# HKUST-SING/herald

Hardware: AMD Instinct MI355X
Metric: embedding rows/s (lookup+grad) (higher is better)
Workload: dtype f32

## Files before the change

herald_amd/_build.py:

```python
import os
import shutil
import subprocess
import sys

ROOT = os.path.dirname(os.path.dirname(os.path.abspath(__file__)))
PKG = os.path.join(ROOT, "herald_amd")
CSRC = os.path.join(PKG, "csrc")
OBJ = os.path.join(PKG, "_build")
LIB = os.path.join(PKG, "libherald_amd.so")

HIPCC = os.environ.get("HIPCC", "/opt/rocm/bin/hipcc")
HIP_FLAGS = [
    "--offload-arch=gfx950", "-O3", "-std=c++17", "-fPIC",
    "-ffp-contract=off",
    "-fno-gpu-rdc", "-Wall", "-Wno-unused-function",
    "-I", os.path.join(ROOT, "include"),
]


def _run(cmd, **kw):
    r = subprocess.run(cmd, stdout=subprocess.PIPE, stderr=subprocess.STDOUT, text=True, **kw)
    if r.returncode != 0:
        sys.stderr.write(" ".join(cmd) + "\n" + r.stdout + "\n")
        raise RuntimeError("build step failed: %s" % " ".join(cmd[:3]))
    return r.stdout


def _newer(src_list, target):
    if not os.path.exists(target):
        return True
    t = os.path.getmtime(target)
    return any(os.path.getmtime(s) > t for s in src_list)


def hip_sources():
    return sorted(os.path.join(CSRC, f) for f in os.listdir(CSRC) if f.endswith(".hip"))


def build_lib(force=False, verbose=False):
    os.makedirs(OBJ, exist_ok=True)
    headers = [os.path.join(CSRC, f) for f in os.listdir(CSRC) if f.endswith(".h")]
    headers.append(os.path.join(ROOT, "include", "herald_amd.h"))
    objs = []
    procs = []
    for src in hip_sources():
        obj = os.path.join(OBJ, os.path.basename(src)[:-4] + ".o")
        objs.append(obj)
        if force or _newer([src] + headers, obj):
            cmd = [HIPCC] + HIP_FLAGS + ["-c", src, "-o", obj]
            if verbose:
                print(" ".join(cmd))
            procs.append((cmd, subprocess.Popen(cmd, stdout=subprocess.PIPE,
                                                stderr=subprocess.STDOUT, text=True)))
    for cmd, p in procs:
        out, _ = p.communicate()
        if p.returncode != 0:
            sys.stderr.write(" ".join(cmd) + "\n" + out + "\n")
            raise RuntimeError("hipcc failed on %s" % cmd[-3])
        if verbose and out.strip():
            print(out)
    if force or procs or _newer(objs, LIB):
        _run([HIPCC, "--offload-arch=gfx950", "-shared", "-fPIC", "-fno-gpu-rdc", "-o", LIB] + objs)
    return LIB


PS_LIB = os.path.join(PKG, "libherald_ps.so")


def build_ps_shim(force=False):
    src = os.path.join(CSRC, "libps_shim.cpp")
    deps = [src, os.path.join(ROOT, "include", "herald_ps.h"), os.path.join(ROOT, "include", "herald_amd.h"), LIB]
    if force or _newer(deps, PS_LIB):
        _run(["g++", "-O2", "-std=c++17", "-shared", "-fPIC", "-Wall", src, "-o", PS_LIB, "-L", PKG, "-lherald_amd",
              "-Wl,-rpath,$ORIGIN"])
    return PS_LIB


def build_plugins(force=False):
    import sysconfig
    import pybind11
    out_dir = os.path.join(PKG, "plugins")
    os.makedirs(out_dir, exist_ok=True)
    suffix = sysconfig.get_config_var("EXT_SUFFIX")
    inc = ["-I", pybind11.get_include(), "-I", sysconfig.get_paths()["include"], "-I", "/opt/rocm/include"]
    outs = []
    procs = []
    for name in ("hetu_cache", "laia_cache"):
        src = os.path.join(CSRC, "py_%s.cpp" % name)
        out = os.path.join(out_dir, name + suffix)
        outs.append(out)
        if force or _newer([src, os.path.join(ROOT, "include", "herald_amd.h"), LIB], out):
            cmd = ["g++", "-O2", "-std=c++17", "-shared", "-fPIC", "-w", "-D__HIP_PLATFORM_AMD__"] + inc + \
                  [src, "-o", out, "-L", PKG, "-lherald_amd", "-L", "/opt/rocm/lib", "-lamdhip64",
                   "-Wl,-rpath,$ORIGIN/..", "-Wl,-rpath,/opt/rocm/lib", "-pthread"]
            procs.append((cmd, subprocess.Popen(cmd, stdout=subprocess.PIPE, stderr=subprocess.STDOUT, text=True)))
    for cmd, p in procs:
        o, _ = p.communicate()
        if p.returncode != 0:
            sys.stderr.write(" ".join(cmd) + "\n" + o + "\n")
            raise RuntimeError("plugin build failed")
    return outs


def build_oracle(force=False):
    src = os.path.join(ROOT, "oracle", "oracle.c")
    out_dir = os.path.join(ROOT, "oracle", "_build")
    out = os.path.join(out_dir, "liboracle.so")
    if not os.path.exists(src):
        return None
    os.makedirs(out_dir, exist_ok=True)
    if force or _newer([src], out):
        _run(["gcc", "-O3", "-fopenmp", "-ffp-contract=off", "-fPIC", "-shared", "-std=c11",
              "-Wall", "-o", out, src, "-lm"])
    return out


def build_ref(force=False):
    script = os.path.join(ROOT, "oracle", "build_ref.sh")
    if not (os.path.isdir("/root/reference") and os.path.exists(script)):
        return None
    _run(["bash", script])
    return os.path.join(ROOT, "oracle", "_ref")


def build_all(force=False, verbose=False):
    lib = build_lib(force=force, verbose=verbose)
    build_ps_shim(force=force)
    build_plugins(force=force)
    build_oracle(force=force)
    build_ref(force=force)
    return lib


if __name__ == "__main__":
    build_all(force="--force" in sys.argv, verbose=True)
    print("built", LIB)
```

herald_amd/_lib.py:

```python
import ctypes
import os
import re

_PKG = os.path.dirname(os.path.abspath(__file__))
LIB_PATH = os.path.join(_PKG, "libherald_amd.so")
HEADER_PATH = os.path.join(os.path.dirname(_PKG), "include", "herald_amd.h")

_lib = None


class HeraldAmdError(RuntimeError):
    pass


class DLContext(ctypes.Structure):
    _fields_ = [("device_id", ctypes.c_int), ("device_type", ctypes.c_int)]


class DLArray(ctypes.Structure):
    _fields_ = [("data", ctypes.c_void_p), ("ctx", DLContext), ("ndim", ctypes.c_int),
                ("shape", ctypes.POINTER(ctypes.c_int64)), ("stride", ctypes.POINTER(ctypes.c_int64))]


class DLStream(ctypes.Structure):
    _fields_ = [("device_id", ctypes.c_int), ("handle", ctypes.c_void_p)]


class CacheRemote(ctypes.Structure):
    _fields_ = [("req_keys", ctypes.c_void_p), ("req_versions", ctypes.c_void_p), ("inbox_pull", ctypes.c_void_p),
                ("inbox_idx", ctypes.c_void_p), ("inbox_versions", ctypes.c_void_p), ("inbox_rows", ctypes.c_void_p),
                ("out_keys", ctypes.c_void_p), ("out_updates", ctypes.c_void_p), ("out_rows", ctypes.c_void_p),
                ("out_capacity", ctypes.c_int64), ("max_batch", ctypes.c_int64)]


class PlanView(ctypes.Structure):
    _fields_ = [("n", ctypes.c_int64), ("n_unique", ctypes.c_void_p), ("keys", ctypes.c_void_p),
                ("sorted", ctypes.c_void_p), ("perm", ctypes.c_void_p), ("inverse", ctypes.c_void_p),
                ("uniq", ctypes.c_void_p), ("counts", ctypes.c_void_p), ("seg", ctypes.c_void_p),
                ("upos", ctypes.c_void_p)]


def declared_symbols(header=None):
    text = open(header or HEADER_PATH).read()
    text = re.sub(r"/\*.*?\*/", "", text, flags=re.S)
    text = re.sub(r"\(\s*\*\s*\w+\s*\)\s*\([^;{}]*\)\s*;", ";", text)
    names = re.findall(r"\b([A-Za-z_][A-Za-z0-9_]*)\s*\([^;{}]*\)\s*;", text)
    return sorted(set(n for n in names if n not in ("defined", "int", "void", "float")))


PS_LIB_PATH = os.path.join(_PKG, "libherald_ps.so")
PS_HEADER_PATH = os.path.join(os.path.dirname(_PKG), "include", "herald_ps.h")


def load(build_if_missing=True):
    global _lib
    if _lib is not None:
        return _lib
    try:
        import torch
    except ImportError:
        pass
    if not os.path.exists(LIB_PATH):
        if not build_if_missing:
            raise HeraldAmdError("libherald_amd.so is not built (%s)" % LIB_PATH)
        from . import _build
        _build.build_lib()
    try:
        L = ctypes.CDLL(LIB_PATH, mode=ctypes.RTLD_GLOBAL)
    except OSError as e:
        raise HeraldAmdError("cannot load %s: %s" % (LIB_PATH, e))
    _declare(L)
    _lib = L
    return L


class ShardSlot(ctypes.Structure):
    _fields_ = [("world", ctypes.c_int32), ("rank", ctypes.c_int32), ("rcap", ctypes.c_int64), ("n", ctypes.c_int64),
                ("plan_ws", ctypes.c_void_p), ("keys_fixed", ctypes.c_void_p), ("meta_dev", ctypes.c_void_p),
                ("posmap", ctypes.c_void_p), ("rowmap", ctypes.c_void_p), ("counts_host", ctypes.c_void_p),
                ("owner_plan_ws", ctypes.c_void_p)]


def check(rc, what=""):
    if rc != 0:
        msg = load().ha_last_error().decode("utf-8", "replace")
        raise HeraldAmdError("%s failed: %s" % (what or "herald_amd call", msg))


def _declare(L):
    c = ctypes
    vp, i64, f32, sz = c.c_void_p, c.c_int64, c.c_float, c.c_size_t
    L.ha_version.restype = c.c_char_p
    L.ha_last_error.restype = c.c_char_p
    L.ha_device_count.restype = c.c_int
    L.ha_plan_bytes.restype = sz
    L.ha_plan_bytes.argtypes = [i64]
    L.ha_plan_view_of.argtypes = [vp, i64, c.POINTER(PlanView)]
    L.ha_plan_radix_stamps.argtypes = [vp, i64, vp, vp]
    L.ha_pend_bytes.restype = sz
    L.ha_pend_bytes.argtypes = []
    L.ha_plan_handoff_timeout.restype = vp
    L.ha_plan_handoff_timeout.argtypes = [vp]
    L.ha_step_tab_bytes.restype = sz
    L.ha_step_tab_bytes.argtypes = []
    L.ha_step_max_ids.restype = i64
    L.ha_step_max_ids.argtypes = []
    L.ha_qstep_max_ids.restype = i64
    L.ha_qstep_max_ids.argtypes = []
    L.ha_qstep_init.restype = c.c_int
    L.ha_qstep_init.argtypes = []
    L.ha_event_create.restype = vp
    L.ha_event_create.argtypes = []
    L.ha_host_unmap.restype = c.c_int
    L.ha_host_unmap.argtypes = [vp]
    L.ha_qbig_max_ids.restype = i64
    L.ha_qbig_max_ids.argtypes = []
    L.ha_xchg_create.restype = vp
    L.ha_xchg_create.argtypes = [vp, c.c_int, c.c_int]
    L.ha_qbig_plan_bytes.restype = sz
    L.ha_qbig_plan_bytes.argtypes = [i64]
    L.ha_qbig_buckets.restype = c.c_int
    L.ha_qbig_buckets.argtypes = [i64]
    L.ha_qstep_queue_bytes.restype = sz
    L.ha_qstep_queue_bytes.argtypes = [i64, i64]
    L.ha_qstep_queue_header.restype = vp
    L.ha_qstep_queue_header.argtypes = [vp]
    sigs = {
        "ha_gather_f32ids": [vp, i64, i64, vp, i64, vp, vp],
        "ha_gather_u64ids": [vp, i64, i64, vp, i64, vp, vp],
        "ha_gather_u32keys": [vp, i64, i64, vp, i64, vp, vp],
        "ha_scatter_rows_f32ids": [vp, vp, i64, i64, vp, i64, vp],
        "ha_scale_f32": [vp, i64, f32, vp],
        "ha_plan_build_f32ids": [vp, i64, vp, vp],
        "ha_plan_build_u64ids": [vp, i64, vp, vp],
        "ha_plan_build_u32keys": [vp, i64, vp, c.c_int, vp],
        "ha_plan_sort_f32ids": [vp, i64, vp, vp],
        "ha_plan_sort_u32keys": [vp, i64, vp, c.c_int, vp],
        "ha_plan_sort_u64ids": [vp, i64, vp, vp],
        "ha_plan_finish": [vp, i64, vp],
        "ha_plan_build_f32ids_lim": [vp, i64, vp, c.c_uint64, vp],
        "ha_plan_sort_f32ids_lim": [vp, i64, vp, c.c_uint64, vp],
        "ha_plan_build_u64ids_lim": [vp, i64, vp, c.c_uint64, vp],
        "ha_plan_sort_u64ids_lim": [vp, i64, vp, c.c_uint64, vp],
        "ha_plan_export_f32": [vp, i64, vp, vp, vp],
        "ha_dedup_reduce": [vp, i64, vp, i64, vp, vp],
        "ha_apply_mapped": [vp, i64, i64, vp, i64, vp, f32, vp, vp, vp, vp],
        "ha_apply_mapped2": [vp, i64, vp, i64, vp, i64, vp, f32, vp, vp, vp, vp],
        "ha_shard_bucket": [vp, i64, vp, c.c_int, vp, vp, vp],
        "ha_shard_route_f32ids": [vp, i64, vp, vp, c.c_int, vp, vp, vp],
        "ha_shard_route_u64ids": [vp, i64, vp, vp, c.c_int, vp, vp, vp],
        "ha_shard_route_pack_f32ids": [vp, i64, vp, vp, c.c_int, i64, vp, vp, vp],
        "ha_shard_route_pack_u64ids": [vp, i64, vp, vp, c.c_int, i64, vp, vp, vp],
        "ha_shard_route_unpack": [vp, c.c_int, i64, vp, vp, vp],
        "ha_shard_frames_route_f32ids": [vp, i64, vp, vp, c.c_int, i64, i64, vp, vp, vp, vp],
        "ha_shard_frames_route_u64ids": [vp, i64, vp, vp, c.c_int, i64, i64, vp, vp, vp, vp],
        "ha_shard_frames_pack": [vp, i64, vp, c.c_int, i64, i64, vp, vp, vp, vp],
        "ha_shard_frames_unpack": [vp, c.c_int, i64, i64, vp, vp, vp],
        "ha_set_tolerance_mode": [c.c_int],
        "ha_get_tolerance_mode": [],
        "ha_shard_frames_serve_push": [vp, i64, i64, vp, c.c_int, i64, vp, vp, vp],
        "ha_shard_frames_pack_batch": [vp, vp, c.c_int, vp, c.c_int, i64, i64, vp, vp, vp, vp],
        "ha_shard_frames_unpack_batch": [vp, c.c_int, c.c_int, i64, i64, vp, vp, vp],
        "ha_shard_frames_pack_batch_sized": [vp, vp, c.c_int, vp, c.c_int, c.c_int, i64, i64, vp, vp, vp, vp, vp, vp],
        "ha_shard_frames_unpack_batch_sized": [vp, c.c_int, c.c_int, i64, i64, vp, vp, vp, vp],
        "ha_shard_sized_serve_pull": [vp, i64, i64, vp, c.c_int, c.c_int, i64, vp, vp, vp],
        "ha_gather2_u32map": [vp, i64, vp, i64, i64, vp, i64, vp, vp],
        "ha_shard_sized_serve_push": [vp, i64, i64, vp, c.c_int, c.c_int, i64, vp, i64, vp, vp, vp],
        "ha_push_apply_scaled_finished": [vp, i64, i64, vp, i64, vp, f32, vp],
        "ha_qbig_plan_batch_f32ids": [vp, vp, vp, i64, i64, vp],
        "ha_qbig_plan_batch_u64ids": [vp, vp, vp, i64, i64, vp],
        "ha_qbig_queue_batch": [i64, i64, vp, vp, vp, vp, vp, i64, i64, vp, vp, vp],
        "ha_qbig_apply": [vp, i64, i64, vp, i64, vp, f32, vp, i64, vp, vp, i64, i64, c.c_uint32, vp, vp, vp],
        "ha_event_destroy": [vp],
        "ha_event_record": [vp, vp],
        "ha_stream_wait_event": [vp, vp],
        "ha_qqueue_batch_epochs": [i64, i64, vp, vp, vp, vp, vp, i64, i64, vp, vp, vp],
        "ha_shard_step_pull": [vp, i64, i64, vp, vp, vp, vp, i64, vp, vp],
        "ha_shard_step_push": [vp, i64, i64, vp, vp, vp, i64, vp, vp, f32, vp],
        "ha_shard_step": [vp, i64, i64, vp, vp, vp, vp, i64, vp, i64, vp, vp, vp, f32, vp],
        "ha_shard_steps": [vp, i64, i64, i64, vp, vp, vp, vp, i64, vp, i64, vp, vp, vp, f32, vp],
        "ha_qapply_steps_sync": [vp, i64, i64, f32, i64, i64, vp, vp, vp, vp, vp, vp, vp, vp, vp, vp, vp, vp],
        "ha_qapply_steps_counts": [vp, i64, i64, f32, i64, i64, vp, vp, vp, vp, vp, vp, vp, vp, vp, vp, vp, vp, vp],
        "ha_qapply_sync": [vp, i64, i64, vp, i64, vp, f32, vp, i64, vp, vp, i64, i64, c.c_uint32, vp, vp, vp],
        "ha_xchg_available": [],
        "ha_xchg_unique_id": [vp],
        "ha_xchg_destroy": [vp],
        "ha_xchg_bytes": [vp, vp, vp, vp, vp, vp],
        "ha_xchg_rows": [vp, vp, vp, vp, vp, i64, vp],
        "ha_qbig_plan_view": [vp, i64, vp, vp, vp, vp, vp, vp, vp],
        "ha_plan_build_batch_f32ids_lim": [vp, vp, vp, c.c_int, c.c_uint64, vp],
        "ha_plan_sort_batch_f32ids_lim": [vp, vp, vp, c.c_int, c.c_uint64, vp],
        "ha_plan_sort_batch_u64ids_lim": [vp, vp, vp, c.c_int, c.c_uint64, vp],
        "ha_plan_build_batch_u64ids_lim": [vp, vp, vp, c.c_int, c.c_uint64, vp],
        "ha_shard_frames_serve_pull": [vp, i64, i64, vp, c.c_int, i64, i64, vp, vp, vp, vp],
        "ha_shard_serve_push": [vp, i64, i64, vp, i64, vp, vp, vp],
        "ha_dedup_reduce_scaled": [vp, i64, vp, i64, f32, vp, vp],
        "ha_debug_apply_timeline": [vp, i64, i64, vp, i64, vp, f32, vp, vp],
        "ha_sgd_apply": [vp, i64, i64, vp, i64, vp, f32, vp],
        "ha_sgd_apply_finished": [vp, i64, i64, vp, i64, vp, f32, vp],
        "ha_push_apply": [vp, i64, i64, vp, i64, vp, vp],
        "ha_sgd_sparse_update_f32ids": [vp, i64, i64, vp, i64, vp, f32, vp],
        "ha_lookup_sort_f32ids": [vp, i64, i64, vp, i64, vp, vp, vp],
        "ha_lookup_sort_u64ids": [vp, i64, i64, vp, i64, vp, vp, vp],
        "ha_sgd_apply_finish": [vp, i64, i64, vp, i64, vp, f32, vp],
        "ha_push_apply_finish": [vp, i64, i64, vp, i64, vp, vp],
        "ha_sgd_apply_finish_prefetch_f32ids": [vp, i64, i64, vp, i64, vp, f32, vp, i64, vp],
        "ha_sparse_opt_fused_f32ids": [c.c_int, vp, i64, i64, vp, i64, vp, vp, vp, vp, vp, vp],
        "ha_pend_reset": [vp, vp],
        "ha_lookup_sort_pend_f32ids": [vp, i64, i64, vp, i64, vp, vp, vp, vp],
        "ha_lookup_sort_pend_u64ids": [vp, i64, i64, vp, i64, vp, vp, vp, vp],
        "ha_sgd_push_pull_f32ids": [vp, i64, i64, vp, i64, vp, f32, vp, vp, i64, vp, vp, vp, vp],
        "ha_sgd_push_pull_u64ids": [vp, i64, i64, vp, i64, vp, f32, vp, vp, i64, vp, vp, vp, vp],
        "ha_step_tab_reset": [vp, vp],
        "ha_step_f32ids": [vp, i64, i64, vp, i64, vp, f32, vp, vp, i64, vp, vp, vp, i64, vp, vp, i64, vp, vp, vp],
        "ha_step_u64ids": [vp, i64, i64, vp, i64, vp, f32, vp, vp, i64, vp, vp, vp, i64, vp, vp, i64, vp, vp, vp],
        "ha_qstep_f32ids": [vp, i64, i64, vp, i64, vp, f32, vp, i64, vp, vp, vp, i64, vp, i64, vp, i64, vp, vp],
        "ha_qstep_u64ids": [vp, i64, i64, vp, i64, vp, f32, vp, i64, vp, vp, vp, i64, vp, i64, vp, i64, vp, vp],
        "ha_qprep_f32ids": [i64, i64, vp, i64, vp, vp, i64, vp, i64, vp, i64, vp],
        "ha_qprep_u64ids": [i64, i64, vp, i64, vp, vp, i64, vp, i64, vp, i64, vp],
        "ha_qplan_batch_f32ids": [vp, vp, vp, i64, vp],
        "ha_qplan_batch_u64ids": [vp, vp, vp, i64, vp],
        "ha_qqueue_batch": [i64, i64, vp, vp, vp, vp, vp, i64, i64, vp],
        "ha_stream_gate": [vp, vp],
        "ha_debug_occupy": [i64, i64, i64, i64, vp],
        "ha_qapply": [vp, i64, i64, vp, i64, vp, f32, vp, i64, vp, vp, i64, vp],
        "ha_qapply_sized": [vp, i64, i64, vp, i64, vp, f32, vp, i64, vp, vp, i64, i64, vp],
        "ha_qapply_steps": [vp, i64, i64, f32, i64, i64, vp, vp, vp, vp, vp, vp, vp, vp, vp],
        "ha_qqueue_batch_counts": [i64, i64, vp, vp, vp, vp, vp, i64, i64, vp, vp],
        "ha_debug_qprep_f32ids": [i64, i64, vp, i64, vp, vp, i64, vp, i64, vp, i64, vp, vp],
        "ha_debug_qapply": [vp, i64, i64, vp, i64, vp, f32, vp, i64, vp, vp, i64, vp, vp],
        "ha_debug_step_fwd_timeline": [vp, i64, i64, vp, i64, vp, f32, vp, vp, i64, vp, vp, vp, i64, vp, vp, i64, vp,
                                       vp, vp, vp],
    }
    for name, args in sigs.items():
        fn = getattr(L, name)
        fn.argtypes = args
        fn.restype = c.c_int
    L.ha_cache_create.restype = vp
    L.ha_cache_create.argtypes = [c.c_int, i64, i64, i64, i64]
    L.ha_cache_destroy.restype = None
    L.ha_cache_destroy.argtypes = [vp]
    for name in ("ha_cache_data", "ha_cache_grad"):
        getattr(L, name).restype = vp
        getattr(L, name).argtypes = [vp]
    for name in ("ha_cache_limit", "ha_cache_width", "ha_cache_fused_updates"):
        getattr(L, name).restype = i64
        getattr(L, name).argtypes = [vp]
    cache_sigs = {
        "ha_cache_set_bounds": [vp, i64, i64],
        "ha_cache_set_bypass": [vp, c.c_int],
        "ha_cache_bind_store": [vp, vp, vp, i64, i64],
        "ha_cache_lookup": [vp, vp, c.c_int, i64, vp, vp],
        "ha_cache_sort_ahead": [vp, vp, c.c_int, i64, vp],
        "ha_cache_lookup_presorted": [vp, vp, c.c_int, i64, vp, vp],
        "ha_cache_sort_ahead_batch": [vp, vp, c.c_int, vp, c.c_int, vp],
        "ha_cache_plan_block": [vp, vp, c.c_int, vp, c.c_int, vp, vp],
        "ha_cache_plan_block_push_keys": [vp, vp, c.c_int, vp, vp, c.c_int, vp, c.c_int, vp, vp],
        "ha_cache_lookup_planned": [vp, i64, vp, vp],
        "ha_cache_update_planned": [vp, i64, vp, vp],
        "ha_cache_plan_pending": [vp],
        "ha_cache_run_planned_pairs": [vp, c.c_int, vp, vp, vp, vp],
        "ha_cache_plan_block_push_pull": [vp, vp, c.c_int, vp, c.c_int, vp, vp],
        "ha_cache_push_pull_planned": [vp, i64, vp, i64, vp, vp],
        "ha_cache_run_planned_push_pulls": [vp, c.c_int, vp, vp, vp, vp, vp],
        "ha_cache_update": [vp, vp, c.c_int, i64, vp, vp],
        "ha_cache_update_same_keys": [vp, i64, vp, vp],
        "ha_cache_update_with_push_keys": [vp, vp, c.c_int, i64, vp, c.c_int, i64, vp, vp],
        "ha_cache_push_pull": [vp, vp, c.c_int, i64, vp, vp, c.c_int, i64, vp, vp],
        "ha_cache_perf": [vp, vp, vp],
        "ha_cache_state": [vp, vp, vp],
        "ha_cache_phase_times": [vp, vp, vp],
        "ha_cache_set_timing": [vp, c.c_int],
        "ha_cache_stage_times": [vp, vp],
        "ha_cache_snapshot": [vp, i64, vp, vp, vp, vp, vp, vp, vp],
        "ha_cache_set_line": [vp, i64, i64, vp, vp],
        "ha_cache_set_remote": [vp],
        "ha_cache_remote_buffers": [vp, vp],
        "ha_cache_lookup_begin": [vp, vp, c.c_int, i64, vp, vp],
        "ha_cache_lookup_finish": [vp, i64, vp, vp],
        "ha_cache_outbox_count": [vp, vp, vp],
        "ha_cache_outbox_pad": [vp, i64],
        "ha_store_count_valid": [vp, i64, i64, vp, vp],
        "ha_cache_push_pull_begin": [vp, vp, c.c_int, i64, vp, c.c_int, i64, vp, vp, vp],
        "ha_cache_push_pull_finish": [vp, vp, vp],
        "ha_store_serve_sync": [vp, vp, i64, i64, vp, vp, i64, i64, vp, vp, vp, vp, vp, vp, vp],
        "ha_store_add_versions": [vp, i64, vp, vp, i64, vp],
        "ha_store_push_distinct": [vp, vp, i64, i64, vp, vp, vp, i64, vp],
    }
    for name, args in cache_sigs.items():
        fn = getattr(L, name)
        fn.argtypes = args
        fn.restype = c.c_int
    L.ha_laia_create.restype = vp
    L.ha_laia_create.argtypes = [vp, i64, i64, i64, i64, i64, i64]
    L.ha_laia_destroy.restype = None
    L.ha_laia_destroy.argtypes = [vp]
    L.ha_laia_next.restype = c.c_int
    L.ha_laia_next.argtypes = [vp, i64, i64, vp, vp, i64, vp]
    L.ha_laia_hint_next.restype = c.c_int
    L.ha_laia_hint_next.argtypes = [vp, i64]
    L.ha_laia_next_for_rank.restype = c.c_int
    L.ha_laia_next_for_rank.argtypes = [vp, i64, i64, i64, vp, vp, i64, vp]
    L.ha_laia_snapshot_keys.restype = i64
    L.ha_laia_snapshot_keys.argtypes = [vp, i64, vp, i64]
    L.ha_laia_next_topk.restype = c.c_int
    L.ha_laia_next_topk.argtypes = [vp, i64, i64, vp, i64, i64, vp, vp, i64, vp]
    L.ha_laia_counters.restype = c.c_int
    L.ha_laia_counters.argtypes = [vp, vp]
    L.ha_laia_timing.restype = c.c_int
    L.ha_laia_timing.argtypes = [vp, vp]
    L.ha_laia_timing_device.restype = c.c_int
    L.ha_laia_timing_device.argtypes = [vp, vp]
    L.ha_laia_on_device.restype = c.c_int
    L.ha_laia_on_device.argtypes = [vp]
    L.ha_shm_ring_open.restype = vp
    L.ha_shm_ring_open.argtypes = [c.c_char_p, c.c_int, i64]
    L.ha_shm_ring_close.restype = None
    L.ha_shm_ring_close.argtypes = [vp]
    L.ha_shm_ring_send.restype = c.c_int
    L.ha_shm_ring_send.argtypes = [vp, vp, i64]
    L.ha_shm_ring_recv.restype = i64
    L.ha_shm_ring_recv.argtypes = [vp, vp, i64, vp]
    L.ha_shm_ring_pending_words.restype = i64
    L.ha_shm_ring_pending_words.argtypes = [vp]
    A, S = c.POINTER(DLArray), c.POINTER(DLStream)
    dl = {
        "DLGpuEmbeddingLookUp": [A, A, A, S],
        "DLGpuEmbeddingLookUp_Gradient": [A, A, A, S],
        "IndexedSlicesOneSideAdd": [A, A, A, S],
        "DeduplicateIndexedSlices": [A, A, A, S],
        "IndexedSlices2Dense": [A, A, A, S],
        "SGDOptimizerSparseUpdate": [A, A, A, f32, S],
        "AdaGradOptimizerSparseUpdate": [A, A, A, A, f32, f32, S],
        "AdamOptimizerSparseUpdate": [A, A, A, A, A, f32, f32, f32, f32, f32, f32, S],
        "AdamWOptimizerSparseUpdate": [A, A, A, A, A, f32, f32, f32, f32, f32, f32, f32, S],
        "AddL2RegularizationSparse": [A, A, A, f32, S],
# ... 10 lines not shown
```

herald_amd/csrc/qstep.hip:

```cpp
#include <hip/hip_ext.h>

#include "plan_dev.h"
#include "gather_dev.h"

namespace ha {

constexpr int kQMax = 7168;
#ifndef QV_GOLD
#define QV_GOLD 1
#endif
#ifndef QV_WG
#define QV_WG (QV_GOLD ? 1024 : 256)
#endif
#ifndef QV_COOPSLOTS
#define QV_COOPSLOTS (QV_GOLD ? 64 : 256)
#endif
constexpr int kQWg = QV_WG;
constexpr int kQWpw = kQWg / 64;
constexpr int kQCoopSlots = QV_COOPSLOTS;
constexpr int kQWorkerMax = 448 * 16 / kQWpw;
constexpr int kQSmallC = 3, kQSmallM = 16, kQMediumC = 15, kQLongC = 64;
enum QKind { kQS = 0, kQM = 1, kQL = 2, kQZ = 3, kQG = 4, kQNone = 15 };

struct QHeader {
    uint32_t n_wave, n_coop;
    uint32_t n_long, n_medium, n_small;
    uint32_t n_copy, n_copy_medium, n_copy_small;
    uint32_t overflow_wave, overflow_copy;
    uint32_t epoch_wave, epoch_copy, done;
    uint32_t verdict;
    uint32_t reserved[50];
};
static_assert(sizeof(QHeader) == 256, "queue header is one 256-byte line");
struct QEntry {
    uint32_t w[8];
};
constexpr uint32_t kQOccMask = 0x1FFFFFu;
__host__ __device__ __forceinline__ uint2 q_occ_pack(uint32_t o0, uint32_t o1, uint32_t o2) {
    const unsigned long long v = static_cast<unsigned long long>(o0 & kQOccMask) |
                                 (static_cast<unsigned long long>(o1 & kQOccMask) << 21) |
                                 (static_cast<unsigned long long>(o2 & kQOccMask) << 42);
    return uint2{static_cast<uint32_t>(v), static_cast<uint32_t>(v >> 32)};
}
static_assert(sizeof(QEntry) == 32, "queue items are 32 bytes");

struct QLayout {
    QHeader *hdr;
    QEntry *coop, *wave, *copy;
    float *part;
    uint32_t *pcnt;
    uint32_t cap_coop, cap_wave, cap_copy;
    size_t bytes;
};
constexpr uint32_t kQChunk = 256;
__host__ __device__ __forceinline__ uint32_t q_nchunk(uint32_t c) {
    return (QV_GOLD && c > kQChunk) ? (c + kQChunk - 1u) / kQChunk : 1u;
}
static inline int ceil_div(int64_t a, int64_t b) { return static_cast<int>((a + b - 1) / b); }
static inline QLayout queue_layout(void *ws, int64_t n_cap, int64_t width) {
    QLayout q;
    char *b = static_cast<char *>(ws);
    q.cap_coop = static_cast<uint32_t>(ceil_div(width, 32) * (ceil_div(n_cap, kQLongC) + 1));
    q.cap_wave = static_cast<uint32_t>(ceil_div(width, 512) * 2 * n_cap + 64);
    q.cap_copy = static_cast<uint32_t>(ceil_div(width, 512) * n_cap + 64);
    q.hdr = reinterpret_cast<QHeader *>(b);
    q.coop = reinterpret_cast<QEntry *>(b ? b + sizeof(QHeader) : nullptr);
    q.wave = q.coop ? q.coop + q.cap_coop : nullptr;
    q.copy = q.wave ? q.wave + q.cap_wave : nullptr;
    const size_t items = sizeof(QHeader) + (static_cast<size_t>(q.cap_coop) + q.cap_wave + q.cap_copy) * sizeof(QEntry);
    q.part = reinterpret_cast<float *>(b ? b + items : nullptr);
    q.pcnt = reinterpret_cast<uint32_t *>(b ? b + items + static_cast<size_t>(q.cap_coop) * 256 : nullptr);
    q.bytes = items + static_cast<size_t>(q.cap_coop) * (256 + 4);
    return q;
}

struct QPlan {
    PlanHeader *hdr;
    uint32_t *keys, *sorted, *uniq;
    int32_t *perm, *inverse, *counts, *seg, *upos;
    uint32_t *occ;
    int n;
};
static inline QPlan qplan(void *ws, int64_t n) {
    QPlan q;
    memset(&q, 0, sizeof(q));
    if (ws == nullptr || n <= 0)
        return q;
    PlanPtrs p = plan_layout(ws, n);
    q.hdr = p.hdr; q.keys = p.keys; q.sorted = p.sorted; q.uniq = p.uniq;
    q.perm = p.perm; q.inverse = p.inverse; q.counts = p.counts; q.seg = p.seg; q.upos = p.upos;
    q.occ = p.keys_alt;
    q.n = static_cast<int>(n);
    return q;
}

struct QArgs {
    float *table;
    uint64_t rows;
    int width;
    const QHeader *qh;
    const QEntry *qcoop, *qwave, *qcopy;
    float *qpart;
    uint32_t *qpcnt;
    uint32_t cap_coop, cap_wave, cap_copy;
    const int32_t *perm_a;
    int n_a;
    const float *grads;
    float lr;
    const int32_t *perm_g;
    int n_g;
    float *out;
    int ncoop, nworker;
    uint32_t epoch;
    uint32_t *err;
    unsigned long long *dbg;
};

__device__ __forceinline__ void q_phase(unsigned long long *ph, int k) {
    if (ph != nullptr && threadIdx.x == 0)
        ph[k] = __builtin_amdgcn_s_memrealtime();
}

template <int NW>
__device__ __forceinline__ uint32_t qscan_n(uint32_t v, uint32_t *s_w, uint32_t *total, int w) {
    const int lane = lane_id();
    uint32_t x = v;
#pragma unroll
    for (int o = 1; o < 64; o <<= 1) {
        const uint32_t y = __shfl_up(x, o, 64);
        if (lane >= o)
            x += y;
    }
    __syncthreads();
    if (lane == 63)
        s_w[w] = x;
    __syncthreads();
    const uint32_t mine = s_w[lane & (NW - 1)];
    uint32_t woff = 0, tot = 0;
#pragma unroll
    for (int k = 0; k < NW; ++k) {
        const uint32_t t = static_cast<uint32_t>(__builtin_amdgcn_readlane(static_cast<int>(mine), k));
        woff += k < w ? t : 0u;
        tot += t;
    }
    *total = tot;
    return woff + x - v;
}

constexpr int kQTabBits = 13, kQTabSize = 1 << kQTabBits;
constexpr uint32_t kQTabEmpty = 0xFFFFFFFFu;
constexpr int kGroupedFlagWord = 12;
constexpr int kOrderFlagWord = 13;
__device__ __forceinline__ uint32_t q_hash(uint32_t key, int bits = kQTabBits) {
    return (key * 0x9E3779B1u) >> (32 - bits);
}
static inline size_t qsort_lds_bytes(int n) {
    const size_t npad = (static_cast<size_t>(n) + 1023) & ~static_cast<size_t>(1023);
    return kQTabSize * 4 + 3 * npad * 2 + 8 + 32 * 4;
}
constexpr int kQSubThreads = 256, kQSubTabBits = 12, kQSubMax = 7 * kQSubThreads;
constexpr size_t kQSubPlanLds = (size_t(1) << kQSubTabBits) * 4 + 3 * size_t(kQSubMax) * 2 + 8 + 32 * 4 + 120;
static_assert(kQSubPlanLds % 128 == 0, "the groups' LDS regions stay aligned");

template <typename IdT, bool RANK_ATOMIC, bool BUCKET = false, int NT = 1024, int TBITS = kQTabBits>
__device__ __forceinline__ void qsort_finish_body(const IdT *__restrict__ ids, const QPlan &p, uint32_t *lds,
                                                  unsigned long long *ph = nullptr,
                                                  const uint32_t *__restrict__ pos_map = nullptr) {
    constexpr int TS = 1 << TBITS, SPT = TS / NT;
    const int n = p.n;
    const int tid = static_cast<int>(threadIdx.x) & (NT - 1), lane = lane_id(), w = tid >> 6;
    const int npad = (n + NT - 1) & ~(NT - 1);
    const int P = npad / NT;
    uint32_t *s_tab = lds;
    uint16_t *s_lab = reinterpret_cast<uint16_t *>(lds + TS);
    uint16_t *s_cnt = s_lab + npad;
    uint16_t *s_rank = s_cnt + npad + 4;
    uint32_t *s_w = reinterpret_cast<uint32_t *>(s_rank + npad);
    q_phase(ph, 0);
    uint32_t key[7];
#pragma unroll
    for (int k = 0; k < 7; ++k)
        key[k] = to_key<IdT>(ids[max(min(tid + k * NT, n - 1), 0)]);
    for (int i = tid; i < TS; i += NT)
        s_tab[i] = kQTabEmpty;
    for (int i = tid; i < npad / 2 + 2; i += NT)
        reinterpret_cast<uint32_t *>(s_cnt)[i] = 0;
    __syncthreads();
    q_phase(ph, 1);
    {
        uint32_t h[7], seen[7];
#pragma unroll
        for (int k = 0; k < 7; ++k) {
            h[k] = q_hash(key[k], TBITS);
            seen[k] = key[k];
            if (k < P && tid + k * NT < n) {
                if (BUCKET && k > 0 && s_tab[h[k]] == key[k])
                    continue;
                seen[k] = kQTabEmpty;
                if (__hip_atomic_compare_exchange_strong(s_tab + h[k], &seen[k], key[k], __ATOMIC_RELAXED,
                                                         __ATOMIC_RELAXED, __HIP_MEMORY_SCOPE_WORKGROUP))
                    seen[k] = key[k];
            }
        }
#pragma unroll
        for (int k = 0; k < 7; ++k) {
            const int i = tid + k * NT;
            if (k < P && i < n) {
                while (seen[k] != key[k]) {
                    h[k] = (h[k] + 1) & (TS - 1);
                    seen[k] = kQTabEmpty;
                    if (__hip_atomic_compare_exchange_strong(s_tab + h[k], &seen[k], key[k], __ATOMIC_RELAXED,
                                                             __ATOMIC_RELAXED, __HIP_MEMORY_SCOPE_WORKGROUP))
                        seen[k] = key[k];
                }
                s_lab[i] = static_cast<uint16_t>(h[k]);
            }
        }
    }
    __syncthreads();
    q_phase(ph, 2);
    uint32_t U;
    {
        uint32_t kk[SPT], occ = 0;
#pragma unroll
        for (int j = 0; j < SPT; ++j) {
            kk[j] = s_tab[tid * SPT + j];
            occ += kk[j] != kQTabEmpty;
        }
        uint32_t g = qscan_n<NT / 64>(occ, s_w, &U, w);
#pragma unroll
        for (int j = 0; j < SPT; ++j) {
            if (kk[j] != kQTabEmpty) {
                p.uniq[g] = kk[j];
                s_tab[tid * SPT + j] = g;
                ++g;
            }
        }
    }
    __syncthreads();
    q_phase(ph, 3);
    uint32_t lab[7];
#pragma unroll
    for (int k = 0; k < 7; ++k) {
        const int i = tid + k * NT;
        lab[k] = 0;
        if (k < P && i < n) {
            lab[k] = s_tab[s_lab[i]];
            s_lab[i] = static_cast<uint16_t>(lab[k]);
        }
    }
    __syncthreads();
    q_phase(ph, 4);
    if (w == 0) {
        uint32_t *cnt32 = reinterpret_cast<uint32_t *>(s_cnt);
        const uint32_t spare = static_cast<uint32_t>(npad);
        uint32_t nx[8];
#pragma unroll
        for (int r = 0; r < 8; ++r)
            nx[r] = s_lab[min(r * 64 + lane, npad - 1)];
        for (int r0 = 0; r0 < npad; r0 += 8 * 64) {
            uint32_t lb[8], rk[8];
#pragma unroll
            for (int r = 0; r < 8; ++r) {
                const int i = r0 + r * 64 + lane;
                lb[r] = i < n ? nx[r] : spare;
            }
// ... 77 lines not shown
        }
    }
    if (tid == 0) {
        p.hdr->n_unique = U;
        p.hdr->reserved[kGroupedFlagWord] = 1;
        p.hdr->reserved[kOrderFlagWord] = 0;
        p.seg[U] = n;
    }
    __syncthreads();
    q_phase(ph, 6);
    {
        uint32_t q[7];
#pragma unroll
        for (int k = 0; k < 7; ++k) {
            const int i = tid + k * NT;
            q[k] = (k < P && i < n) ? static_cast<uint32_t>(s_cnt[lab[k]]) + s_rank[i] : 0u;
        }
        __syncthreads();
        uint16_t *s_perm = s_lab, *s_gq = s_rank;
        uint32_t *s_key = s_tab;
#pragma unroll
        for (int k = 0; k < 7; ++k) {
            const int i = tid + k * NT;
            if (k < P && i < n) {
                s_perm[q[k]] = static_cast<uint16_t>(i);
                s_gq[q[k]] = static_cast<uint16_t>(lab[k]);
                s_key[i] = key[k];
            }
        }
        __syncthreads();
        bool disorder = false;
        for (int qq = tid; qq < n; qq += NT) {
            const uint32_t i = s_perm[qq];
            if (BUCKET) {
                p.perm[qq] = static_cast<int32_t>(pos_map[i]);
            } else {
                p.perm[qq] = static_cast<int32_t>(i);
                p.sorted[qq] = s_key[i];
                p.upos[qq] = static_cast<int32_t>(s_gq[qq]);
            }
            disorder |= qq > 0 && s_gq[qq] == s_gq[qq - 1] && i <= s_perm[qq - 1];
        }
        if (disorder)
            p.hdr->reserved[kOrderFlagWord] = 1;
        for (uint32_t g = tid; g < U; g += NT) {
            const int st = s_cnt[g];
            uint32_t o0 = s_perm[min(st, n - 1)], o1 = s_perm[min(st + 1, n - 1)], o2 = s_perm[min(st + 2, n - 1)];
            if (BUCKET) {
                o0 = pos_map[o0];
                o1 = pos_map[o1];
                o2 = pos_map[o2];
            }
            reinterpret_cast<uint2 *>(p.occ)[g] = q_occ_pack(o0, o1, o2);
        }
    }
    q_phase(ph, 7);
}

static inline size_t qjoin_lds_bytes(int n_a, int n_g) {
    return kQTabSize * 4 + static_cast<size_t>(n_a > n_g ? n_a : n_g) * 4 + 32 * 4;
}
static inline size_t qjoin_lds_resident_bytes(int n_g) {
    return kQTabSize * 4 + static_cast<size_t>(n_g) * 8 + 32 * 4;
}

__device__ __forceinline__ int q_kind(uint32_t c, uint32_t m, bool in_table) {
    if (!in_table)
        return m > 0 ? kQZ : kQNone;
    if (c >= static_cast<uint32_t>(kQLongC))
        return kQG;
    if (c > static_cast<uint32_t>(kQMediumC))
        return kQL;
    if (c > static_cast<uint32_t>(kQSmallC) || m > static_cast<uint32_t>(kQSmallM))
        return kQM;
    return kQS;
}
__device__ __forceinline__ int q_slice(int kind) {
    return kind == kQL ? 32 : kind == kQG ? (QV_GOLD ? 64 : 32) : kind == kQM ? 128 : 512;
}

__device__ __forceinline__ void q_st_item(QEntry *dst, uint4 lo, uint4 hi) {
    float4v a, b;
    __builtin_memcpy(&a, &lo, 16);
    __builtin_memcpy(&b, &hi, 16);
    st4_sc1(reinterpret_cast<float *>(dst), a);
    st4_sc1(reinterpret_cast<float *>(dst) + 4, b);
}
__device__ __forceinline__ void q_emit_words(QEntry *dst, int kind, uint32_t key, uint32_t c, uint32_t st, uint32_t m,
                                             uint32_t fs, int width, uint32_t o01, uint32_t o23, uint32_t *pcnt = nullptr) {
    const int slice = q_slice(kind);
    if (kind == kQZ)
        c = 0;
    int j = 0;
    const uint32_t nch = kind == kQG ? q_nchunk(c) : 1u;
    if (nch > 1u) {
        for (int col0 = 0; col0 < width; col0 += slice) {
            __hip_atomic_store(pcnt + j, 0u, __ATOMIC_RELAXED, __HIP_MEMORY_SCOPE_AGENT);
            for (uint32_t ch = 0; ch < nch; ++ch, ++j) {
                uint4 lo, hi;
                lo.x = static_cast<uint32_t>(kind) | (static_cast<uint32_t>(col0 / 4) << 4);
                lo.y = key;
                lo.z = c;
                lo.w = st;
                hi.x = m;
                hi.y = fs;
                hi.z = ch | (nch << 16);
                hi.w = 0;
                q_st_item(dst + j, lo, hi);
            }
        }
        return;
    }
    if (kind == kQG)
        o01 = 0;
    for (int col0 = 0; col0 < width; col0 += slice, ++j) {
        const int cols = min(slice, width - col0);
        uint4 lo, hi;
        lo.x = static_cast<uint32_t>(kind) | (static_cast<uint32_t>(col0 / 4) << 4);
        lo.y = key;
        lo.z = c;
        (void)cols;
        lo.w = st;
        hi.x = m;
        hi.y = fs;
        hi.z = o01;
        hi.w = o23;
        q_st_item(dst + j, lo, hi);
    }
}
struct QCount {
    uint32_t g, l, m, s;
};
__device__ __forceinline__ QCount q_count(QCount t, int kind, uint32_t per512, uint32_t per128, uint32_t per32, uint32_t c) {
    t.g += kind == kQG ? (QV_GOLD ? (per32 + 1u) / 2u : per32) * q_nchunk(c) : 0u;
    t.l += kind == kQL ? per32 : 0u;
    t.m += kind == kQM ? per128 : 0u;
    t.s += (kind == kQS || kind == kQZ) ? per512 : 0u;
    return t;
}

struct QJoin {
    QPlan pa, pg;
    uint64_t rows;
    int width, Ua, Ug, Ub;
    bool cs_res;
    uint32_t *s_tab, *s_bk, *s_cs, *s_w;
    QHeader *bqh;
    QEntry *bcoop, *bwave, *bcopy;
    uint32_t *bpcnt;
    uint32_t bcap_coop, bcap_wave, bcap_copy, per512, per128, per32;
    uint32_t st_base, fs_base;
    uint32_t tid, nt;
    int tbits;
};

__device__ __forceinline__ uint32_t qjoin_probe(const QJoin &j, uint32_t key) {
    uint32_t h = q_hash(key, j.tbits);
    const uint32_t mask = (1u << j.tbits) - 1u;
    for (;;) {
        const uint32_t e = j.s_tab[h];
        if (e == kQTabEmpty || j.s_bk[e] == key)
            return e;
        h = (h + 1) & mask;
    }
}
__device__ __forceinline__ uint32_t qjoin_dest(const QJoin &j, uint32_t e) {
    if (e == kQTabEmpty)
        return 0u;
    return j.cs_res ? j.s_cs[e] : (static_cast<uint32_t>(j.pg.counts[e]) | (static_cast<uint32_t>(j.pg.seg[e]) << 16));
}
__device__ __forceinline__ QCount qjoin_emit_one(const QJoin &j, QCount b, QEntry *wave, uint32_t cap_wave, uint32_t key,
                                                 uint32_t c, uint32_t st, uint32_t m, uint32_t fs, uint32_t o01, uint32_t o2) {
    const int kind = q_kind(c, m, key < j.rows);
    if (kind == kQNone)
        return b;
    const uint32_t at = kind == kQG ? b.g : kind == kQL ? b.l : kind == kQM ? b.m : b.s;
    const QCount nb = q_count(b, kind, j.per512, j.per128, j.per32, c);
    const uint32_t cnt = (nb.g - b.g) + (nb.l - b.l) + (nb.m - b.m) + (nb.s - b.s);
    if (at + cnt <= (kind == kQG ? j.bcap_coop : cap_wave))
        q_emit_words((kind == kQG ? j.bcoop : wave) + at, kind, key, c, st + j.st_base, m, fs + j.fs_base, j.width, o01, o2,
                     kind == kQG ? j.bpcnt + at : nullptr);
    return nb;
}

template <int R0, int R1>
__device__ __forceinline__ QCount qjoin_count_groups(const QJoin &j, QCount t) {
    const uint32_t tid = j.tid, last = static_cast<uint32_t>(max(j.Ua, 1) - 1);
    uint32_t ka[R1 - R0], c[R1 - R0];
#pragma unroll
    for (int r = R0; r < R1; ++r) {
        const uint32_t x = min(static_cast<uint32_t>(r) * j.nt + tid, last);
        ka[r - R0] = j.pa.uniq[x];
        c[r - R0] = static_cast<uint32_t>(j.pa.counts[x]);
    }
#pragma unroll
    for (int r = R0; r < R1; ++r) {
        if (static_cast<int>(static_cast<uint32_t>(r) * j.nt + tid) < j.Ua) {
            const uint32_t mf = qjoin_dest(j, qjoin_probe(j, ka[r - R0]));
            t = q_count(t, q_kind(c[r - R0], mf & 0xFFFFu, ka[r - R0] < j.rows), j.per512, j.per128, j.per32, c[r - R0]);
        }
    }
    return t;
}
template <int R0, int R1>
__device__ __forceinline__ QCount qjoin_emit_groups(const QJoin &j, QCount b) {
    const uint32_t tid = j.tid, last = static_cast<uint32_t>(max(j.Ua, 1) - 1);
    uint32_t ka[R1 - R0], cst[R1 - R0], o01[R1 - R0], o2[R1 - R0];
#pragma unroll
    for (int r = R0; r < R1; ++r) {
        const uint32_t x = min(static_cast<uint32_t>(r) * j.nt + tid, last);
        const uint2 oc = reinterpret_cast<const uint2 *>(j.pa.occ)[x];
        ka[r - R0] = j.pa.uniq[x];
        cst[r - R0] = static_cast<uint32_t>(j.pa.counts[x]) | (static_cast<uint32_t>(j.pa.seg[x]) << 16);
        o01[r - R0] = oc.x;
        o2[r - R0] = oc.y;
    }
#pragma unroll
    for (int r = R0; r < R1; ++r) {
        if (static_cast<int>(static_cast<uint32_t>(r) * j.nt + tid) < j.Ua) {
            const uint32_t mf = qjoin_dest(j, qjoin_probe(j, ka[r - R0]));
            b = qjoin_emit_one(j, b, j.bwave, j.bcap_wave, ka[r - R0], cst[r - R0] & 0xFFFFu, cst[r - R0] >> 16,
                               mf & 0xFFFFu, mf >> 16, o01[r - R0], o2[r - R0]);
        }
    }
    return b;
}

template <int R0, int R1>
__device__ __forceinline__ QCount qjoin_count_copies(const QJoin &j, QCount t) {
    const uint32_t tid = j.tid, last = static_cast<uint32_t>(max(j.Ug, 1) - 1);
    uint32_t kg[R1 - R0], m[R1 - R0];
#pragma unroll
    for (int r = R0; r < R1; ++r) {
        const uint32_t y = min(static_cast<uint32_t>(r) * j.nt + tid, last);
        kg[r - R0] = j.pg.uniq[y];
        m[r - R0] = static_cast<uint32_t>(j.pg.counts[y]);
    }
#pragma unroll
    for (int r = R0; r < R1; ++r)
        if (static_cast<int>(static_cast<uint32_t>(r) * j.nt + tid) < j.Ug && qjoin_probe(j, kg[r - R0]) == kQTabEmpty)
            t = q_count(t, q_kind(0u, m[r - R0], kg[r - R0] < j.rows), j.per512, j.per128, j.per32, 0u);
    return t;
}
template <int R0, int R1>
__device__ __forceinline__ QCount qjoin_emit_copies(const QJoin &j, QCount b) {
    const uint32_t tid = j.tid, last = static_cast<uint32_t>(max(j.Ug, 1) - 1);
    uint32_t kg[R1 - R0], mfs[R1 - R0];
#pragma unroll
    for (int r = R0; r < R1; ++r) {
        const uint32_t y = min(static_cast<uint32_t>(r) * j.nt + tid, last);
        kg[r - R0] = j.pg.uniq[y];
        mfs[r - R0] = static_cast<uint32_t>(j.pg.counts[y]) | (static_cast<uint32_t>(j.pg.seg[y]) << 16);
    }
#pragma unroll
    for (int r = R0; r < R1; ++r)
        if (static_cast<int>(static_cast<uint32_t>(r) * j.nt + tid) < j.Ug && qjoin_probe(j, kg[r - R0]) == kQTabEmpty)
            b = qjoin_emit_one(j, b, j.bcopy, j.bcap_copy, kg[r - R0], 0u, 0u, mfs[r - R0] & 0xFFFFu, mfs[r - R0] >> 16,
                               0u, 0u);
    return b;
}

template <bool WIDE = false, int NT = 1024, int TBITS = kQTabBits>
__device__ __forceinline__ void qjoin_body(const QPlan pa, const QPlan pg, const uint64_t rows, const int width,
                                           QHeader *bqh, QEntry *bcoop, QEntry *bwave, QEntry *bcopy,
                                           const uint32_t bcap_coop, const uint32_t bcap_wave, const uint32_t bcap_copy,
                                           uint32_t *lds, uint32_t lds_bytes, const int part,
                                           unsigned long long *ph = nullptr, uint32_t *mirror = nullptr,
                                           const uint32_t st_base = 0, const uint32_t fs_base = 0,
                                           const uint32_t epoch = 0, const uint32_t wide_parts = 0, const bool signal = true) {
    constexpr int TS = 1 << TBITS;
    const int tid = static_cast<int>(threadIdx.x) & (NT - 1), w = tid >> 6;
    q_phase(ph, 0);
    QJoin j;
    j.tid = static_cast<uint32_t>(tid);
    j.nt = NT;
    j.tbits = TBITS;
    j.pa = pa;
    j.pg = pg;
    j.st_base = st_base;
    j.fs_base = fs_base;
    j.rows = rows;
    j.width = width;
    j.Ua = uniform(pa.n > 0 ? static_cast<int>(pa.hdr->n_unique) : 0);
    j.Ug = uniform(pg.n > 0 ? static_cast<int>(pg.hdr->n_unique) : 0);
    j.Ub = part == 0 ? j.Ug : j.Ua;
    j.cs_res = part == 0 && static_cast<uint32_t>(TS * 4 + j.Ug * 8 + 32 * 4) <= lds_bytes;
    j.s_tab = lds;
    j.s_bk = lds + TS;
    j.s_cs = j.s_bk + j.Ub;
    j.s_w = j.s_bk + (j.cs_res ? 2 * j.Ub : j.Ub);
    j.bqh = bqh;
    j.bcoop = bcoop;
    j.bwave = bwave;
    j.bcopy = bcopy;
    j.bcap_coop = bcap_coop;
    j.bpcnt = reinterpret_cast<uint32_t *>(reinterpret_cast<char *>(bcoop + (static_cast<size_t>(bcap_coop) + bcap_wave + bcap_copy)) +
                                           static_cast<size_t>(bcap_coop) * 256);
    j.bcap_wave = bcap_wave;
    j.bcap_copy = bcap_copy;
    j.per512 = (width + 511) / 512;
    j.per128 = (width + 127) / 128;
    j.per32 = (width + 31) / 32;
    const uint32_t *bkeys = part == 0 ? pg.uniq : pa.uniq;
    for (int i = tid; i < TS; i += NT)
        j.s_tab[i] = kQTabEmpty;
    for (int y = tid; y < j.Ub; y += NT) {
        j.s_bk[y] = bkeys[y];
        if (j.cs_res)
            j.s_cs[y] = static_cast<uint32_t>(pg.counts[y]) | (static_cast<uint32_t>(pg.seg[y]) << 16);
    }
    __syncthreads();
    q_phase(ph, 1);
    for (int y = tid; y < j.Ub; y += NT) {
        uint32_t h = q_hash(j.s_bk[y], TBITS);
        for (;;) {
            uint32_t seen = kQTabEmpty;
            if (__hip_atomic_compare_exchange_strong(j.s_tab + h, &seen, static_cast<uint32_t>(y), __ATOMIC_RELAXED,
                                                     __ATOMIC_RELAXED, __HIP_MEMORY_SCOPE_WORKGROUP))
                break;
            h = (h + 1) & (TS - 1);
        }
    }
    __syncthreads();
    q_phase(ph, 2);
    QCount t{0u, 0u, 0u, 0u};
    if (part == 0) {
        if (j.Ua > 0)
            t = qjoin_count_groups<0, 4>(j, t);
        if (j.Ua > 4 * NT)
            t = qjoin_count_groups<4, 8>(j, t);
        q_phase(ph, 3);
        uint32_t nL, nM, nS, nG;
        QCount b;
        b.l = qscan_n<NT / 64>(t.l, j.s_w, &nL, w);
        b.m = qscan_n<NT / 64>(t.m, j.s_w, &nM, w) + nL;
        b.s = qscan_n<NT / 64>(t.s, j.s_w, &nS, w) + nL + nM;
        b.g = qscan_n<NT / 64>(t.g, j.s_w, &nG, w);
        if (WIDE) {
            __syncthreads();
            if (tid == 0) {
                const uint32_t tot = nL + nM + nS;
                const uint32_t bw = tot ? atomicAdd(&bqh->n_wave, tot) : 0u;
                const uint32_t bc = nG ? atomicAdd(&bqh->n_coop, nG) : 0u;
                if (nL) atomicAdd(&bqh->n_long, nL);
                if (nM) atomicAdd(&bqh->n_medium, nM);
                if (nS) atomicAdd(&bqh->n_small, nS);
                uint32_t over = (bw + tot > bcap_wave || bc + nG > bcap_coop) ? 1u : 0u;
                if ((pa.n > 0 && pa.hdr->reserved[kOrderFlagWord] != 0) || (pg.n > 0 && pg.hdr->reserved[kOrderFlagWord] != 0))
                    over |= 2u;
                if (over) {
                    atomicOr(&bqh->overflow_wave, over);
                    if (mirror)
                        mirror[3] = over;
                }
                j.s_w[20] = bw;
                j.s_w[21] = bc;
            }
            __syncthreads();
            const uint32_t bw = j.s_w[20], bc = j.s_w[21];
            b.l += bw;
            b.m += bw;
            b.s += bw;
            b.g += bc;
        }
        if (!WIDE && tid == 0) {
            bqh->n_wave = min(nL + nM + nS, bcap_wave);
            bqh->n_coop = min(nG, bcap_coop);
            bqh->n_long = nL;
            bqh->n_medium = nM;
            bqh->n_small = nS;
            uint32_t over = (nL + nM + nS > bcap_wave || nG > bcap_coop) ? 1u : 0u;
            if ((pa.n > 0 && pa.hdr->reserved[kOrderFlagWord] != 0) || (pg.n > 0 && pg.hdr->reserved[kOrderFlagWord] != 0))
                over |= 2u;
            bqh->overflow_wave = over;
            if (mirror) {
                mirror[0] = min(nL + nM + nS, bcap_wave) + 1u;
                mirror[1] = min(nG, bcap_coop) + 1u;
                if (over)
                    mirror[3] = over;
            }
        }
        q_phase(ph, 4);
        if (j.Ua > 0)
            b = qjoin_emit_groups<0, 3>(j, b);
        if (j.Ua > 3 * NT)
            b = qjoin_emit_groups<3, 5>(j, b);
        if (j.Ua > 5 * NT)
            b = qjoin_emit_groups<5, 8>(j, b);
    } else {
        if (j.Ug > 0)
            t = qjoin_count_copies<0, 4>(j, t);
        if (j.Ug > 4 * NT)
            t = qjoin_count_copies<4, 8>(j, t);
        q_phase(ph, 3);
        uint32_t nM, nS;
        QCount b{0u, 0u, 0u, 0u};
        b.m = qscan_n<NT / 64>(t.m, j.s_w, &nM, w);
        b.s = qscan_n<NT / 64>(t.s, j.s_w, &nS, w) + nM;
        if (WIDE) {
            __syncthreads();
            if (tid == 0) {
                const uint32_t tot = nM + nS;
                const uint32_t bw = tot ? atomicAdd(&bqh->n_copy, tot) : 0u;
                if (nM) atomicAdd(&bqh->n_copy_medium, nM);
                if (nS) atomicAdd(&bqh->n_copy_small, nS);
                if (bw + tot > bcap_copy) {
                    atomicOr(&bqh->overflow_copy, 1u);
                    if (mirror)
                        mirror[3] = 1u;
                }
                j.s_w[20] = bw;
            }
            __syncthreads();
            const uint32_t bw = j.s_w[20];
            b.m += bw;
            b.s += bw;
        }
        if (!WIDE && tid == 0) {
            bqh->n_copy = min(nM + nS, bcap_copy);
            bqh->n_copy_medium = nM;
            bqh->n_copy_small = nS;
            bqh->overflow_copy = nM + nS > bcap_copy ? 1u : 0u;
            if (mirror) {
                mirror[2] = min(nM + nS, bcap_copy) + 1u;
                if (nM + nS > bcap_copy)
                    mirror[3] = 1u;
            }
        }
        q_phase(ph, 4);
        if (j.Ug > 0)
            b = qjoin_emit_copies<0, 4>(j, b);
        if (j.Ug > 4 * NT)
            b = qjoin_emit_copies<4, 8>(j, b);
    }
    q_phase(ph, 5);
    asm volatile("s_waitcnt vmcnt(0) lgkmcnt(0)" ::: "memory");
    __syncthreads();
    if (tid == 0) {
        if (!WIDE) {
            if (part == 0) {
                __hip_atomic_store(&bqh->n_wave, bqh->n_wave, __ATOMIC_RELAXED, __HIP_MEMORY_SCOPE_AGENT);
                __hip_atomic_store(&bqh->n_coop, bqh->n_coop, __ATOMIC_RELAXED, __HIP_MEMORY_SCOPE_AGENT);
            } else {
                __hip_atomic_store(&bqh->n_copy, bqh->n_copy, __ATOMIC_RELAXED, __HIP_MEMORY_SCOPE_AGENT);
            }
            asm volatile("s_waitcnt vmcnt(0) lgkmcnt(0)" ::: "memory");
            __hip_atomic_store(part == 0 ? &bqh->epoch_wave : &bqh->epoch_copy, epoch, __ATOMIC_RELAXED, __HIP_MEMORY_SCOPE_AGENT);
        } else if (signal &&
                   __hip_atomic_fetch_add(&bqh->done, 1u, __ATOMIC_RELAXED, __HIP_MEMORY_SCOPE_AGENT) + 1u == wide_parts) {
            __hip_atomic_store(&bqh->epoch_wave, epoch, __ATOMIC_RELAXED, __HIP_MEMORY_SCOPE_AGENT);
            __hip_atomic_store(&bqh->epoch_copy, epoch, __ATOMIC_RELAXED, __HIP_MEMORY_SCOPE_AGENT);
            if (mirror) {
                const uint32_t nw = __hip_atomic_load(&bqh->n_wave, __ATOMIC_RELAXED, __HIP_MEMORY_SCOPE_AGENT);
                const uint32_t nc = __hip_atomic_load(&bqh->n_coop, __ATOMIC_RELAXED, __HIP_MEMORY_SCOPE_AGENT);
                const uint32_t np = __hip_atomic_load(&bqh->n_copy, __ATOMIC_RELAXED, __HIP_MEMORY_SCOPE_AGENT);
                mirror[1] = min(nc, bcap_coop) + 1u;
                mirror[2] = min(np, bcap_copy) + 1u;
                __threadfence_system();
                mirror[0] = min(nw, bcap_wave) + 1u;
            }
        }
    }
}

typedef float float2v_ __attribute__((ext_vector_type(2)));

__device__ __forceinline__ float4v sgd4(float4v acc, float4v g, float lr) {
    float4v r;
#pragma unroll
    for (int k = 0; k < 4; ++k)
        r[k] = __fsub_rn(acc[k], __fmul_rn(lr, g[k]));
    return r;
}
__device__ __forceinline__ float4v acc4(float4v p, float4v g, float lr) {
    float4v r;
#pragma unroll
    for (int k = 0; k < 4; ++k)
        r[k] = __fadd_rn(p[k], __fmul_rn(lr, g[k]));
    return r;
}
__device__ __forceinline__ float4v add4(float4v x, float4v y) {
    float4v r;
#pragma unroll
    for (int k = 0; k < 4; ++k)
        r[k] = __fadd_rn(x[k], y[k]);
    return r;
}
__device__ __forceinline__ float4v sub4(float4v x, float4v y) {
    float4v r;
#pragma unroll
    for (int k = 0; k < 4; ++k)
        r[k] = __fsub_rn(x[k], y[k]);
    return r;
}
__device__ __forceinline__ float4v shfl_xor4(float4v v, int mask) {
    float4v r;
#pragma unroll
    for (int k = 0; k < 4; ++k)
        r[k] = __shfl_xor(v[k], mask, 64);
    return r;
}

#ifndef QV_ROW_NT
#define QV_ROW_NT 1
#endif
#ifndef QV_OUT_NT
#define QV_OUT_NT 1
#endif
#ifndef QV_GRAD_NT
#define QV_GRAD_NT 0
#endif
#ifndef QV_INTERLEAVE
#define QV_INTERLEAVE 1
#endif
#ifndef QV_ROWLD_NT
#define QV_ROWLD_NT 0
#endif
template <typename V>
__device__ __forceinline__ V q_ld_row(const float *p) {
#if QV_ROWLD_NT
    return __builtin_nontemporal_load(reinterpret_cast<const V *>(p));
#else
    return *reinterpret_cast<const V *>(p);
#endif
}
template <typename V>
__device__ __forceinline__ void q_st_row(float *p, V v) {
#if QV_ROW_NT
    __builtin_nontemporal_store(v, reinterpret_cast<V *>(p));
#else
    *reinterpret_cast<V *>(p) = v;
#endif
}
template <typename V>
__device__ __forceinline__ void q_st_out(float *p, V v) {
#if QV_OUT_NT
    __builtin_nontemporal_store(v, reinterpret_cast<V *>(p));
#else
    *reinterpret_cast<V *>(p) = v;
#endif
}
template <typename V>
__device__ __forceinline__ V q_ld_grad(const float *p) {
#if QV_GRAD_NT
    return __builtin_nontemporal_load(reinterpret_cast<const V *>(p));
#else
    return *reinterpret_cast<const V *>(p);
#endif
}

struct QItem {
    int kind, col0, cols;
    uint32_t key, c, st, m, fs, o01, o23;
};
__device__ __forceinline__ QItem q_load(const QEntry *e, int width) {
    const uint4 lo = reinterpret_cast<const uint4 *>(e)[0], hi = reinterpret_cast<const uint4 *>(e)[1];
    QItem it;
    it.kind = static_cast<int>(uniform(lo.x & 15u));
    it.col0 = static_cast<int>(uniform(lo.x >> 4)) * 4;
    it.key = uniform(lo.y);
    it.c = uniform(lo.z);
    it.cols = min(q_slice(it.kind), width - it.col0);
    it.st = uniform(lo.w);
    it.m = uniform(hi.x);
    it.fs = uniform(hi.y);
    it.o01 = uniform(hi.z);
    it.o23 = uniform(hi.w);
    return it;
}

__device__ __forceinline__ void q_small(const QArgs &a, const QItem &it) {
    const int lane = lane_id();
    const int width = a.width;
    const int ca = it.col0 + 4 * lane, cb = ca + 256;
    const bool a0 = 4 * lane < it.cols, a1 = 256 + 4 * lane < it.cols;
    const int la = a0 ? ca : it.col0, lb = a1 ? cb : it.col0;
    float *row = a.table + static_cast<uint64_t>(it.kind == kQZ ? 0u : it.key) * static_cast<uint64_t>(width);
    float4v r0{0.f, 0.f, 0.f, 0.f}, r1{0.f, 0.f, 0.f, 0.f};
    if (it.kind != kQZ) {
        r0 = q_ld_row<float4v>(row + la);
        r1 = q_ld_row<float4v>(row + lb);
    }
    int dv = 0;
    if (it.m > 0)
        dv = a.perm_g[it.fs + min(static_cast<uint32_t>(lane), it.m - 1u)];
    float4v g0[kQSmallC], g1[kQSmallC];
#pragma unroll
    for (int t = 0; t < kQSmallC; ++t) {
        if (static_cast<uint32_t>(t) < it.c) {
            const uint32_t o = t == 0 ? (it.o01 & kQOccMask)
                                      : t == 1 ? (((it.o01 >> 21) | (it.o23 << 11)) & kQOccMask) : ((it.o23 >> 10) & kQOccMask);
            const float *src = a.grads + static_cast<uint64_t>(o) * static_cast<uint64_t>(width);
            g0[t] = q_ld_grad<float4v>(src + la);
            g1[t] = q_ld_grad<float4v>(src + lb);
        }
    }
#pragma unroll
// ... 164 lines not shown
    float4v cur = q_ld_row<float4v>(row + col);
    int dv = 0;
    if (it.m > 0)
        dv = a.perm_g[it.fs + min(static_cast<uint32_t>(64 * (lane >> 2) + 4 * w + (lane & 3)), it.m - 1u)];
    float4v p{0.f, 0.f, 0.f, 0.f};
    for (uint32_t base = c_lo; base < c_hi; base += 256) {
        const uint32_t mine = base + 16u * static_cast<uint32_t>(w);
        if (mine >= c_hi)
            break;
        const int pidx = a.perm_a[it.st + min(mine + static_cast<uint32_t>(lane & 15), c_hi - 1u)];
        float4v g[4];
#pragma unroll
        for (int t = 0; t < 4; ++t) {
            const uint32_t o = static_cast<uint32_t>(__shfl(pidx, 4 * t + r, 64));
            g[t] = q_ld_grad<float4v>(a.grads + static_cast<uint64_t>(o) * static_cast<uint64_t>(width) + col);
        }
#pragma unroll
        for (int t = 0; t < 4; ++t) {
            const float4v q = acc4(p, g[t], a.lr);
            const bool valid = mine + static_cast<uint32_t>(4 * t + r) < c_hi;
            p = valid ? q : p;
        }
    }
    p = add4(p, shfl_xor4(p, 16));
    p = add4(p, shfl_xor4(p, 32));
    if (lane < 16)
        *reinterpret_cast<float4v *>(s_part + w * 64 + 4 * c4) = p;
    __syncthreads();
    const float *sp = s_part + (4 * r) * 64 + 4 * c4;
    float4v total = add4(add4(*reinterpret_cast<const float4v *>(sp), *reinterpret_cast<const float4v *>(sp + 64)),
                         add4(*reinterpret_cast<const float4v *>(sp + 128), *reinterpret_cast<const float4v *>(sp + 192)));
    total = add4(total, shfl_xor4(total, 16));
    total = add4(total, shfl_xor4(total, 32));
    if (nch > 1u) {
        const uint32_t first = e - ch;
        if (w == 0 && r == 0)
            st4_sc1(a.qpart + static_cast<size_t>(e) * 64 + 4 * c4, total);
        asm volatile("s_waitcnt vmcnt(0) lgkmcnt(0)" ::: "memory");
        __syncthreads();
        uint32_t *s_flag = reinterpret_cast<uint32_t *>(s_part);
        if (threadIdx.x == 0)
            *s_flag = __hip_atomic_fetch_add(a.qpcnt + first, 1u, __ATOMIC_RELAXED, __HIP_MEMORY_SCOPE_AGENT);
        __syncthreads();
        const bool last = *s_flag + 1u == nch;
        __syncthreads();
        if (!last)
            return;
        const float *pp = a.qpart + static_cast<size_t>(first) * 64 + 4 * c4;
        float4v tot{0.f, 0.f, 0.f, 0.f};
        for (uint32_t j0 = 0; j0 < nch; j0 += 4) {
            float4v q0 = ld4_sc1_async(pp + static_cast<size_t>(min(j0, nch - 1u)) * 64);
            float4v q1 = ld4_sc1_async(pp + static_cast<size_t>(min(j0 + 1u, nch - 1u)) * 64);
            float4v q2 = ld4_sc1_async(pp + static_cast<size_t>(min(j0 + 2u, nch - 1u)) * 64);
            float4v q3 = ld4_sc1_async(pp + static_cast<size_t>(min(j0 + 3u, nch - 1u)) * 64);
            wait_loads(q0, q1, q2, q3);
            tot = j0 == 0 ? q0 : add4(tot, q0);
            if (j0 + 1u < nch) tot = add4(tot, q1);
            if (j0 + 2u < nch) tot = add4(tot, q2);
            if (j0 + 3u < nch) tot = add4(tot, q3);
        }
        total = tot;
    }
    const float4v nv = sub4(cur, total);
    if (w == 0 && r == 0 && act)
        q_st_row(row + col, nv);
    for (uint32_t k0 = 0; k0 * 64u < it.m; k0 += 16) {
        if (k0 > 0)
            dv = a.perm_g[it.fs + min(64u * (k0 + static_cast<uint32_t>(lane >> 2)) + static_cast<uint32_t>(4 * w + (lane & 3)),
                                      it.m - 1u)];
        const uint32_t rounds = min(16u, (it.m - 64u * k0 + 63u) / 64u);
        for (uint32_t k = 0; k < rounds; ++k) {
            const uint32_t j = 64u * (k0 + k) + static_cast<uint32_t>(4 * w + r);
            const uint32_t d = static_cast<uint32_t>(__shfl(dv, static_cast<int>(4 * k) + r, 64));
            if (j < it.m && act)
                q_st_out(a.out + static_cast<uint64_t>(d) * static_cast<uint64_t>(width) + col, nv);
        }
    }
    __syncthreads();
}

#endif

__device__ __forceinline__ void q_coop(const QArgs &a, const QItem &it, float *s_part) {
    const int lane = lane_id(), w = uniform(static_cast<int>(threadIdx.x >> 6));
    const int width = a.width;
    const int r = lane >> 3, c4 = lane & 7;
    const bool act = 4 * c4 < it.cols;
    const int col = it.col0 + (act ? 4 * c4 : 0);
    float *row = a.table + static_cast<uint64_t>(it.key) * static_cast<uint64_t>(width);
    const float4v cur = q_ld_row<float4v>(row + col);
    constexpr uint32_t kDW = 8u * kQWpw, kBlk = 64u * kQWpw;
    int dv = 0;
    if (it.m > 0)
        dv = a.perm_g[it.fs + min(kDW * static_cast<uint32_t>(lane >> 3) + static_cast<uint32_t>(8 * w + (lane & 7)), it.m - 1u)];
    float4v p{0.f, 0.f, 0.f, 0.f};
    for (uint32_t base = 0; base < it.c; base += kBlk) {
        const uint32_t mine = base + 64u * static_cast<uint32_t>(w);
        if (mine >= it.c)
            break;
        const int pidx = a.perm_a[it.st + min(mine + static_cast<uint32_t>(lane), it.c - 1u)];
        float4v g[8];
#pragma unroll
        for (int t = 0; t < 8; ++t) {
            const uint32_t o = static_cast<uint32_t>(__shfl(pidx, 8 * t + r, 64));
            g[t] = q_ld_grad<float4v>(a.grads + static_cast<uint64_t>(o) * static_cast<uint64_t>(width) + col);
        }
#pragma unroll
        for (int t = 0; t < 8; ++t) {
            const float4v q = acc4(p, g[t], a.lr);
            const bool valid = mine + static_cast<uint32_t>(8 * t + r) < it.c;
            p = valid ? q : p;
        }
    }
    p = add4(p, shfl_xor4(p, 8));
    p = add4(p, shfl_xor4(p, 16));
    p = add4(p, shfl_xor4(p, 32));
    if (lane < 8)
        *reinterpret_cast<float4v *>(s_part + w * 32 + 4 * c4) = p;
    __syncthreads();
    const float *sp = s_part + 4 * c4;
    float4v total = add4(add4(*reinterpret_cast<const float4v *>(sp), *reinterpret_cast<const float4v *>(sp + 32)),
                         add4(*reinterpret_cast<const float4v *>(sp + 64), *reinterpret_cast<const float4v *>(sp + 96)));
#pragma unroll
    for (int q = 1; q < kQWpw / 4; ++q)
        total = add4(total, add4(add4(*reinterpret_cast<const float4v *>(sp + 128 * q), *reinterpret_cast<const float4v *>(sp + 128 * q + 32)),
                                 add4(*reinterpret_cast<const float4v *>(sp + 128 * q + 64), *reinterpret_cast<const float4v *>(sp + 128 * q + 96))));
    const float4v nv = sub4(cur, total);
    if (w == 0 && r == 0 && act)
        q_st_row(row + col, nv);
    for (uint32_t k0 = 0; k0 * kDW < it.m; k0 += 8) {
        if (k0 > 0)
            dv = a.perm_g[it.fs + min(kDW * (k0 + static_cast<uint32_t>(lane >> 3)) + static_cast<uint32_t>(8 * w + (lane & 7)),
                                      it.m - 1u)];
        const uint32_t rounds = min(8u, (it.m - kDW * k0 + kDW - 1u) / kDW);
        for (uint32_t k = 0; k < rounds; ++k) {
            const uint32_t j = kDW * (k0 + k) + static_cast<uint32_t>(8 * w + r);
            const uint32_t d = static_cast<uint32_t>(__shfl(dv, static_cast<int>(8 * k) + r, 64));
            if (j < it.m && act)
                q_st_out(a.out + static_cast<uint64_t>(d) * static_cast<uint64_t>(width) + col, nv);
        }
    }
    __syncthreads();
}

static_assert(kQWg == 256 || kQWg == 512 || kQWg == 1024, "workgroups of 4, 8 or 16 waves");
static_assert(!QV_GOLD || kQWg == 1024, "the sixteen-wave G item needs 1024-thread workgroups");
__global__ __launch_bounds__(kQWg, 8) void qapply_kernel(const QArgs a) {
    extern __shared__ __attribute__((aligned(16))) uint32_t s_dyn[];
    const unsigned long long t0 = a.dbg ? __builtin_amdgcn_s_memrealtime() : 0ull;
    int role, kind = -1;
    int b = blockIdx.x;
    if (a.epoch != 0u) {
        const uint32_t fail = ~a.epoch;
        bool ready = a.qh->epoch_wave == a.epoch && a.qh->epoch_copy == a.epoch &&
                     a.qh->verdict != fail;
        if (blockIdx.x == 0) {
            const unsigned long long t_poll = __builtin_amdgcn_s_memrealtime();
            for (int spin = 0; !ready && spin < (1 << 22); ++spin) {
                const uint32_t e0 = __hip_atomic_load(&a.qh->epoch_wave, __ATOMIC_ACQUIRE, __HIP_MEMORY_SCOPE_AGENT);
                const uint32_t e1 = __hip_atomic_load(&a.qh->epoch_copy, __ATOMIC_ACQUIRE, __HIP_MEMORY_SCOPE_AGENT);
                ready = uniform(static_cast<uint32_t>(e0 == a.epoch && e1 == a.epoch)) != 0u;
                if (ready || __builtin_amdgcn_s_memrealtime() - t_poll > 200000000ull)
                    break;
                __builtin_amdgcn_s_sleep(64);
            }
            if (threadIdx.x == 0) {
                __hip_atomic_store(const_cast<uint32_t *>(&a.qh->verdict), ready ? a.epoch : fail, __ATOMIC_RELAXED,
                                   __HIP_MEMORY_SCOPE_AGENT);
                if (!ready && a.err != nullptr)
                    __hip_atomic_store(a.err, 8u, __ATOMIC_RELAXED, __HIP_MEMORY_SCOPE_SYSTEM);
            }
        } else if (!ready) {
            const unsigned long long t_poll = __builtin_amdgcn_s_memrealtime();
            uint32_t vd = 0u;
            for (int spin = 0; spin < (1 << 23); ++spin) {
                vd = uniform(__hip_atomic_load(&a.qh->verdict, __ATOMIC_ACQUIRE, __HIP_MEMORY_SCOPE_AGENT));
                if (vd == a.epoch || vd == fail || __builtin_amdgcn_s_memrealtime() - t_poll > 400000000ull)
                    break;
                __builtin_amdgcn_s_sleep(64);
            }
            ready = vd == a.epoch;
            if (!ready && vd != fail && a.err != nullptr && threadIdx.x == 0)
                __hip_atomic_store(a.err, 8u, __ATOMIC_RELAXED, __HIP_MEMORY_SCOPE_SYSTEM);
        }
        if (!ready)
            return;
    }
    const bool coop = b < a.ncoop;
    if (coop) {
        role = 0;
        const uint32_t n = min(a.qh->n_coop, a.cap_coop);
        for (uint32_t e = static_cast<uint32_t>(b); e < n; e += static_cast<uint32_t>(a.ncoop)) {
            const QItem it = q_load(a.qcoop + e, a.width);
#if QV_GOLD
            q_coop_r3(a, it, reinterpret_cast<float *>(s_dyn), e);
#else
            q_coop(a, it, reinterpret_cast<float *>(s_dyn));
#endif
            kind = it.kind;
        }
    } else {
        b -= a.ncoop;
        role = 3;
        const uint32_t n0 = min(a.qh->n_wave, a.cap_wave), n = n0 + min(a.qh->n_copy, a.cap_copy);
        const uint32_t stride = static_cast<uint32_t>(a.nworker) * static_cast<uint32_t>(kQWpw);
        const uint32_t wv = uniform(static_cast<uint32_t>(threadIdx.x >> 6));
        if (a.width <= 128) {
            const uint32_t n1 = n - n0, both = 2u * (n0 < n1 ? n0 : n1), npair = (n + 1u) / 2u;
            for (uint32_t pe = static_cast<uint32_t>(b) * static_cast<uint32_t>(kQWpw) + wv; pe < npair; pe += stride) {
                const QEntry *src[2];
#pragma unroll
                for (int h = 0; h < 2; ++h) {
                    const uint32_t e = 2u * pe + static_cast<uint32_t>(h);
                    src[h] = e >= n ? nullptr
                                    : e < both ? ((e & 1u) ? a.qcopy + (e >> 1) : a.qwave + (e >> 1))
                                               : (n0 > n1 ? a.qwave + (e - n1) : a.qcopy + (e - n0));
                }
                const uint32_t ka = uniform(src[0]->w[0] & 15u), kb = src[1] ? uniform(src[1]->w[0] & 15u) : 15u;
                const bool sa = ka == static_cast<uint32_t>(kQS), sb = kb == static_cast<uint32_t>(kQS);
                if (sa && sb) {
                    q_small_pair(a, src[0], src[1]);
                    kind = kQS;
                    continue;
                }
#pragma unroll
                for (int h = 0; h < 2; ++h) {
                    if (src[h] == nullptr)
                        continue;
                    const QItem it = q_load(src[h], a.width);
                    kind = it.kind;
                    if (it.kind == kQL)
                        q_long(a, it);
                    else if (it.kind == kQM)
                        q_medium(a, it);
                    else
                        q_small(a, it);
                }
            }
        } else
        for (uint32_t e = static_cast<uint32_t>(b) * static_cast<uint32_t>(kQWpw) + wv; e < n; e += stride) {
#if QV_INTERLEAVE
            const uint32_t n1 = n - n0, both = 2u * (n0 < n1 ? n0 : n1);
            const QEntry *src;
            if (e < both)
                src = (e & 1u) ? a.qcopy + (e >> 1) : a.qwave + (e >> 1);
            else
                src = n0 > n1 ? a.qwave + (e - n1) : a.qcopy + (e - n0);
            const QItem it = q_load(src, a.width);
#else
            const QItem it = q_load(e < n0 ? a.qwave + e : a.qcopy + (e - n0), a.width);
#endif
            kind = it.kind;
            if (it.kind == kQL)
                q_long(a, it);
            else if (it.kind == kQM)
                q_medium(a, it);
            else
                q_small(a, it);
        }
    }
    if (a.dbg) {
        __builtin_amdgcn_s_waitcnt(0);
        const unsigned long long t1 = __builtin_amdgcn_s_memrealtime();
        if (lane_id() == 0) {
            unsigned xcc;
            asm volatile("s_getreg_b32 %0, hwreg(HW_REG_XCC_ID)" : "=s"(xcc));
            unsigned long long *d = a.dbg + (static_cast<size_t>(blockIdx.x) * kQWpw + (threadIdx.x >> 6)) * 4;
            d[0] = t0;
            d[1] = t1;
            d[2] = static_cast<unsigned long long>(role) | (static_cast<unsigned long long>(xcc & 0xF) << 8);
            unsigned long long rec = static_cast<unsigned long long>(static_cast<unsigned>(kind)) & 0xFFull;
            if (kind >= 0) {
                const QEntry *src = nullptr;
                if (role == 0) {
                    src = a.qcoop + blockIdx.x;
                } else if (a.width > 128) {
                    const uint32_t n0 = min(a.qh->n_wave, a.cap_wave), n = n0 + min(a.qh->n_copy, a.cap_copy);
                    const uint32_t e = static_cast<uint32_t>(b) * static_cast<uint32_t>(kQWpw) + static_cast<uint32_t>(threadIdx.x >> 6);
                    const uint32_t n1 = n - n0, both = 2u * (n0 < n1 ? n0 : n1);
                    if (e < n)
                        src = e < both ? ((e & 1u) ? a.qcopy + (e >> 1) : a.qwave + (e >> 1))
                                       : (n0 > n1 ? a.qwave + (e - n1) : a.qcopy + (e - n0));
                }
                if (src != nullptr)
                    rec = (src->w[0] & 15u) | (static_cast<unsigned long long>(src->w[2] & 0xFFFFFu) << 8) |
                          (static_cast<unsigned long long>(src->w[4] & 0xFFFFFu) << 28) |
                          (static_cast<unsigned long long>((src->w[0] >> 4) & 0xFFFFu) << 48);
            }
            d[3] = rec;
        }
    }
}

constexpr int kQBatch = 16;
struct QPlanBatch {
    int count;
    const void *ids[kQBatch];
    QPlan plan[kQBatch];
    unsigned long long *ph;
};
template <typename IdT, bool RANK_ATOMIC>
__global__ __launch_bounds__(1024, 4) void qplan_kernel(const QPlanBatch b) {
    extern __shared__ __attribute__((aligned(16))) uint32_t s_dyn[];
    const int i = blockIdx.x;
    qsort_finish_body<IdT, RANK_ATOMIC>(static_cast<const IdT *>(b.ids[i]), b.plan[i], s_dyn, i == 0 ? b.ph : nullptr);
}

constexpr int kQJoinBatch = 8;
struct QJoinBatch {
    int count, width;
    uint64_t rows;
    uint32_t lds_bytes, cap_coop, cap_wave, cap_copy;
    QPlan pa[kQJoinBatch], pg[kQJoinBatch];
    QHeader *qh[kQJoinBatch];
    QEntry *coop[kQJoinBatch], *wave[kQJoinBatch], *copy[kQJoinBatch];
    uint32_t *mirror[kQJoinBatch];
    uint32_t epoch[kQJoinBatch];
    unsigned long long *ph;
};
__global__ __launch_bounds__(1024, 4) void qqueue_kernel(const QJoinBatch b) {
    extern __shared__ __attribute__((aligned(16))) uint32_t s_dyn[];
    const int i = blockIdx.x >> 1, part = blockIdx.x & 1;
    qjoin_body(b.pa[i], b.pg[i], b.rows, b.width, b.qh[i], b.coop[i], b.wave[i], b.copy[i], b.cap_coop, b.cap_wave,
               b.cap_copy, s_dyn, b.lds_bytes, part, (i == 0 && b.ph) ? b.ph + 8 * part : nullptr, b.mirror[i], 0u, 0u,
               b.epoch[i]);
}

__global__ __launch_bounds__(1024) void q_lds_order_check_kernel(uint32_t *bad) {
    __shared__ uint32_t cnt[16][256];
    __shared__ uint32_t ref[16][512];
    const int w = threadIdx.x >> 6, lane = lane_id();
    for (int i = threadIdx.x; i < 16 * 256; i += 1024)
        (&cnt[0][0])[i] = 0;
    for (int i = threadIdx.x; i < 16 * 512; i += 1024)
        (&ref[0][0])[i] = 0;
    __syncthreads();
    uint32_t s = 12345u + 977u * threadIdx.x, wrong = 0;
    for (int r = 0; r < 7; ++r) {
        s = s * 1664525u + 1013904223u;
        const uint32_t x = s >> 16;
        const int mode = w & 3;
        const uint32_t d = mode == 0 ? 7u : mode == 1 ? (x & 1u) * 255u + 3u : mode == 2 ? (x & 15u) * 3u : (x & 511u);
        const uint32_t sh = (d & 1u) * 16u;
        const uint32_t old = (__hip_atomic_fetch_add(&cnt[w][d >> 1], 1u << sh, __ATOMIC_RELAXED,
                                                     __HIP_MEMORY_SCOPE_WORKGROUP) >> sh) & 0xFFFFu;
        uint32_t want = 0;
        for (int l = 0; l < 64; ++l) {
            if (lane == l) {
                want = ref[w][d];
                ref[w][d] = want + 1;
            }
        }
        wrong += old != want;
    }
    if (wrong)
        atomicAdd(bad, wrong);
}

static int lds_atomics_lane_ordered() {
    static std::atomic<int> state[256];
    int d = 0;
    if (hipGetDevice(&d) != hipSuccess || d < 0 || d >= 256)
        return 0;
    int st = state[d].load(std::memory_order_acquire);
    if (st == 0) {
        st = 2;
        const char *env = getenv("HA_QSTEP_BALLOT");
        uint32_t *bad = nullptr, host = 1;
        if (!(env && env[0] == '1') && hipMalloc(reinterpret_cast<void **>(&bad), 4) == hipSuccess) {
            if (hipMemset(bad, 0, 4) == hipSuccess) {
                hipLaunchKernelGGL(q_lds_order_check_kernel, dim3(8), dim3(1024), 0, nullptr, bad);
                if (hipGetLastError() == hipSuccess &&
                    hipMemcpy(&host, bad, 4, hipMemcpyDeviceToHost) == hipSuccess && host == 0)
                    st = 1;
            }
            (void)hipFree(bad);
        }
        state[d].store(st, std::memory_order_release);
    }
    return st == 1;
}

template <typename IdT>
static int qplan_batch(const IdT *const *ids, const int64_t *n, void *const *plans, int64_t count, hipStream_t stream,
                       unsigned long long *ph = nullptr) {
    HA_REQUIRE(count >= 0 && (count == 0 || (ids && n && plans)), "ha_qplan_batch: null pointer");
    static DeviceOnce lds_allowed;
    if (lds_allowed.run([]() -> int {
            HA_ALLOW_LDS((qplan_kernel<IdT, true>), 160 * 1024);
            HA_ALLOW_LDS((qplan_kernel<IdT, false>), 160 * 1024);
            return 0;
        }))
        return -1;
    const bool ordered = lds_atomics_lane_ordered() != 0;
    for (int64_t k0 = 0; k0 < count; k0 += kQBatch) {
        QPlanBatch b;
        memset(&b, 0, sizeof(b));
        b.ph = k0 == 0 ? ph : nullptr;
        size_t lds = 0;
        for (int64_t k = k0; k < count && b.count < kQBatch; ++k) {
            HA_REQUIRE(n[k] >= 0 && n[k] <= kQMax, "ha_qplan_batch: at most %d ids per batch", kQMax);
            if (n[k] == 0)
                continue;
            HA_REQUIRE(ids[k] && plans[k], "ha_qplan_batch: null pointer (batch %lld)", (long long)k);
            b.ids[b.count] = ids[k];
            b.plan[b.count] = qplan(plans[k], n[k]);
            lds = lds > qsort_lds_bytes(static_cast<int>(n[k])) ? lds : qsort_lds_bytes(static_cast<int>(n[k]));
            ++b.count;
        }
        if (b.count == 0)
            continue;
        if (ordered)
            hipLaunchKernelGGL((qplan_kernel<IdT, true>), dim3(b.count), dim3(1024), lds, stream, b);
        else
            hipLaunchKernelGGL((qplan_kernel<IdT, false>), dim3(b.count), dim3(1024), lds, stream, b);
        HA_LAUNCH_CHECK();
    }
    return 0;
}

static int qqueue_batch(int64_t rows, int64_t width, void *const *plans_a, const int64_t *n_a, void *const *plans_g,
                        const int64_t *n_g, void *const *queues, int64_t queue_n_cap, int64_t count,
                        hipStream_t stream, unsigned long long *ph = nullptr, uint32_t *const *counts_host = nullptr,
                        const uint32_t *epochs = nullptr) {
    HA_REQUIRE(rows >= 0 && rows <= 0xFFFFFFFEll && width >= 4 && width % 4 == 0 && width <= (1 << 20),
               "ha_qqueue_batch: rows of a multiple of 4 floats");
    HA_REQUIRE(count >= 0 && (count == 0 || (plans_a && n_a && plans_g && n_g && queues)), "ha_qqueue_batch: null pointer");
    HA_REQUIRE(count == 0 || (queue_n_cap >= 1 && queue_n_cap <= kQMax), "ha_qqueue_batch: bad queue capacity");
    static DeviceOnce lds_allowed;
    if (lds_allowed.run([]() -> int {
            HA_ALLOW_LDS(qqueue_kernel, 160 * 1024);
            return 0;
        }))
        return -1;
    for (int64_t k0 = 0; k0 < count; k0 += kQJoinBatch) {
        QJoinBatch b;
        memset(&b, 0, sizeof(b));
        b.rows = static_cast<uint64_t>(rows);
        b.width = static_cast<int>(width);
        b.ph = k0 == 0 ? ph : nullptr;
        size_t lds = 0;
        for (int64_t k = k0; k < count && b.count < kQJoinBatch; ++k) {
            HA_REQUIRE(n_a[k] >= 0 && n_g[k] >= 0 && n_a[k] <= queue_n_cap && n_g[k] <= queue_n_cap,
                       "ha_qqueue_batch: a batch is larger than the queues were sized for");
            if (n_a[k] == 0 && n_g[k] == 0)
                continue;
            HA_REQUIRE(queues[k] && (n_a[k] == 0 || plans_a[k]) && (n_g[k] == 0 || plans_g[k]),
                       "ha_qqueue_batch: null pointer (step %lld)", (long long)k);
            const int i = b.count++;
            b.pa[i] = qplan(plans_a[k], n_a[k]);
            b.pg[i] = qplan(plans_g[k], n_g[k]);
            const QLayout q = queue_layout(queues[k], queue_n_cap, width);
            b.qh[i] = q.hdr;
            b.mirror[i] = counts_host ? counts_host[k] : nullptr;
            b.epoch[i] = epochs ? epochs[k] : 0u;
            b.coop[i] = q.coop;
            b.wave[i] = q.wave;
            b.copy[i] = q.copy;
            b.cap_coop = q.cap_coop;
            b.cap_wave = q.cap_wave;
            b.cap_copy = q.cap_copy;
            const size_t need = qjoin_lds_bytes(b.pa[i].n, b.pg[i].n), res = qjoin_lds_resident_bytes(b.pg[i].n);
            lds = lds > need ? lds : need;
            lds = lds > res ? lds : res;
        }
        if (b.count == 0)
            continue;
        b.lds_bytes = static_cast<uint32_t>(lds);
        hipLaunchKernelGGL(qqueue_kernel, dim3(2 * b.count), dim3(1024), lds, stream, b);
        HA_LAUNCH_CHECK();
    }
    return 0;
}

static int qapply_lists(float *table, int64_t rows, int64_t width, const int32_t *perm_cur, int64_t n_cur, const float *grads,
                        float lr, const int32_t *perm_next, int64_t n_next, float *next_out, const void *queue_cur,
                        int64_t queue_n_cap, int64_t n_max, hipStream_t stream, unsigned long long *dbg = nullptr,
                        int64_t wave_items = -1, uint32_t epoch = 0, uint32_t *err = nullptr, hipEvent_t done = nullptr,
                        int64_t coop_items = -1);

static int qapply(float *table, int64_t rows, int64_t width, void *plan_cur, int64_t n_cur, const float *grads, float lr,
                  void *plan_next, int64_t n_next, float *next_out, const void *queue_cur, int64_t queue_n_cap,
                  hipStream_t stream, unsigned long long *dbg = nullptr, int64_t wave_items = -1, uint32_t epoch = 0,
                  uint32_t *err = nullptr, hipEvent_t done = nullptr) {
    HA_REQUIRE(n_cur >= 0 && n_next >= 0 && (n_cur == 0 || plan_cur) && (n_next == 0 || plan_next),
               "ha_qapply: a batch needs its plan");
    return qapply_lists(table, rows, width, n_cur > 0 ? plan_layout(plan_cur, n_cur).perm : nullptr, n_cur, grads, lr,
                        n_next > 0 ? plan_layout(plan_next, n_next).perm : nullptr, n_next, next_out, queue_cur, queue_n_cap,
                        kQMax, stream, dbg, wave_items, epoch, err, done);
}

static int qapply_lists(float *table, int64_t rows, int64_t width, const int32_t *perm_cur, int64_t n_cur, const float *grads,
                        float lr, const int32_t *perm_next, int64_t n_next, float *next_out, const void *queue_cur,
                        int64_t queue_n_cap, int64_t n_max, hipStream_t stream, unsigned long long *dbg,
                        int64_t wave_items, uint32_t epoch, uint32_t *err, hipEvent_t done, int64_t coop_items) {
    HA_REQUIRE(table != nullptr && rows >= 0 && rows <= 0xFFFFFFFEll && width >= 4 && width % 4 == 0 &&
                   width <= (1 << 20) && reinterpret_cast<uintptr_t>(table) % 16 == 0,
               "ha_qapply: the table must be 16-byte aligned with rows of a multiple of 4 floats");
    HA_REQUIRE(n_cur >= 0 && n_next >= 0 && n_cur <= n_max && n_next <= n_max && queue_n_cap >= 1 &&
                   queue_n_cap <= n_max && n_cur <= queue_n_cap && n_next <= queue_n_cap,
               "ha_qapply: at most %lld ids per batch and no more than the queue was sized for", (long long)n_max);
    HA_REQUIRE(n_cur == 0 || (perm_cur && grads && reinterpret_cast<uintptr_t>(grads) % 16 == 0),
               "ha_qapply: current batch needs its plan and 16-byte aligned gradients");
    HA_REQUIRE(n_next == 0 || (perm_next && next_out && reinterpret_cast<uintptr_t>(next_out) % 16 == 0),
               "ha_qapply: next batch needs its plan and a 16-byte aligned output");
    if (n_cur == 0 && n_next == 0) {
        if (done != nullptr)
            HA_CHECK_HIP(hipEventRecord(done, stream));
        return 0;
    }
    HA_REQUIRE(queue_cur != nullptr, "ha_qapply: the queue of this step is missing");
    QArgs a;
    memset(&a, 0, sizeof(a));
    a.epoch = epoch;
    a.err = err;
    a.table = table;
    a.rows = static_cast<uint64_t>(rows);
    a.width = static_cast<int>(width);
    a.lr = lr;
    a.dbg = dbg;
    const QLayout q = queue_layout(const_cast<void *>(queue_cur), queue_n_cap, width);
    a.qh = q.hdr;
    a.qcoop = q.coop;
    a.qwave = q.wave;
    a.qcopy = q.copy;
    a.qpart = q.part;
    a.qpcnt = q.pcnt;
    a.cap_coop = q.cap_coop;
    a.cap_wave = q.cap_wave;
    a.cap_copy = q.cap_copy;
    a.perm_a = perm_cur;
    a.n_a = static_cast<int>(n_cur);
    a.grads = grads;
    a.perm_g = perm_next;
    a.n_g = static_cast<int>(n_next);
    a.out = next_out;
    a.ncoop = n_cur >= kQLongC ? kQCoopSlots : 0;
    if (coop_items >= 0) {
        const int64_t most = 4096 / kQWpw;
        a.ncoop = static_cast<int>(coop_items < most ? coop_items : most);
    }
    const int64_t bound = static_cast<int64_t>(ceil_div(width, 512)) * (n_cur + n_next);
    a.nworker = static_cast<int>(bound / kQWpw + 1 < kQWorkerMax ? bound / kQWpw + 1 : kQWorkerMax);
    if (wave_items >= 0 && wave_items / kQWpw + 1 < a.nworker)
        a.nworker = static_cast<int>(wave_items / kQWpw + 1);
    if (done != nullptr)
        hipExtLaunchKernelGGL(qapply_kernel, dim3(static_cast<unsigned>(a.ncoop + a.nworker)), dim3(kQWg), kQWpw * 64 * 4, stream,
                              nullptr, done, 0, a);
    else
        hipLaunchKernelGGL(qapply_kernel, dim3(static_cast<unsigned>(a.ncoop + a.nworker)), dim3(kQWg), kQWpw * 64 * 4, stream, a);
    HA_LAUNCH_CHECK();
    return 0;
}


constexpr int kQBigTile = 4096;
constexpr int kQBigBucketsMax = 128;
constexpr int64_t kQBigMax = 1 << 17;
constexpr int kQBigTilesMax = static_cast<int>(kQBigMax / kQBigTile);

static inline int qbig_buckets(int64_t n_cap) {
    int p = 4;
    while (p < kQBigBucketsMax && static_cast<int64_t>(p) * 1024 < n_cap)
        p *= 2;
    return p;
}
__device__ __forceinline__ uint32_t qbig_bucket(uint32_t key, int logp) {
    return (key * 0x85EBCA6Bu) >> (32 - logp);
}

struct QBigRef {
    const void *ids;
    int n;
    uint32_t *meta;
    uint32_t *boff;
    uint32_t *thist;
    uint32_t *bkeys, *bpos;
    int32_t *gperm;
    uint32_t *uniq;
    int32_t *counts;
    int32_t *seg;
    uint32_t *occ;
    PlanHeader *bhdr;
    PlanHeader *dummy;
};
static inline size_t qbig_layout(void *ws, int64_t n_cap, QBigRef *r) {
    char *b = static_cast<char *>(ws);
    size_t off = 0;
    auto take = [&](size_t bytes) {
        char *q = b ? b + off : nullptr;
        off += align_up(bytes, 256);
        return q;
    };
    const int P = qbig_buckets(n_cap);
    const size_t n4 = static_cast<size_t>(n_cap) * 4;
    QBigRef t;
    memset(&t, 0, sizeof(t));
    t.meta = reinterpret_cast<uint32_t *>(take(256));
    t.boff = reinterpret_cast<uint32_t *>(take((P + 1) * 4));
    t.thist = reinterpret_cast<uint32_t *>(take(static_cast<size_t>(kQBigTilesMax) * P * 4));
    t.bkeys = reinterpret_cast<uint32_t *>(take(n4));
    t.bpos = reinterpret_cast<uint32_t *>(take(n4));
    t.gperm = reinterpret_cast<int32_t *>(take(n4));
    t.uniq = reinterpret_cast<uint32_t *>(take(n4));
    t.counts = reinterpret_cast<int32_t *>(take(n4));
    t.seg = reinterpret_cast<int32_t *>(take(n4 + (P + 1) * 4));
    t.occ = reinterpret_cast<uint32_t *>(take(2 * n4));
    t.bhdr = reinterpret_cast<PlanHeader *>(take(static_cast<size_t>(P) * sizeof(PlanHeader)));
    t.dummy = reinterpret_cast<PlanHeader *>(take(2 * sizeof(PlanHeader)));
    if (r)
        *r = t;
    return off;
}

struct QBigBatch {
    int count, P, logp;
    QBigRef r[kQBatch];
};

template <typename IdT>
__global__ __launch_bounds__(1024) void qbpart_hist_kernel(const QBigBatch b) {
    __shared__ uint32_t s_h[kQBigBucketsMax];
    const QBigRef &r = b.r[blockIdx.y];
    const int n = r.n, base = static_cast<int>(blockIdx.x) * kQBigTile;
    if (base >= n)
        return;
    if (threadIdx.x < kQBigBucketsMax)
        s_h[threadIdx.x] = 0;
    __syncthreads();
    const IdT *ids = static_cast<const IdT *>(r.ids);
#pragma unroll
    for (int k = 0; k < kQBigTile / 1024; ++k) {
        const int i = base + k * 1024 + static_cast<int>(threadIdx.x);
        if (i < n)
            atomicAdd(&s_h[qbig_bucket(to_key<IdT>(ids[i]), b.logp)], 1u);
    }
    __syncthreads();
    if (static_cast<int>(threadIdx.x) < b.P)
        r.thist[blockIdx.x * b.P + threadIdx.x] = s_h[threadIdx.x];
}

template <typename IdT>
__global__ __launch_bounds__(1024) void qbpart_scatter_kernel(const QBigBatch b) {
    __shared__ uint32_t s_base[kQBigBucketsMax], s_tot[kQBigBucketsMax];
    __shared__ uint32_t s_cnt[(kQBigTile / 64) * kQBigBucketsMax];
    const QBigRef &r = b.r[blockIdx.y];
    const int n = r.n, P = b.P, t = static_cast<int>(blockIdx.x), tid = static_cast<int>(threadIdx.x);
    const int T = (n + kQBigTile - 1) / kQBigTile;
    if (n == 0) {
        if (t == 0 && tid <= P) {
            r.boff[tid] = 0;
            if (tid == 0)
                r.meta[0] = 0;
        }
        return;
    }
    if (t >= T)
        return;
    uint32_t before = 0;
    if (tid < P) {
        uint32_t tot = 0;
        for (int q = 0; q < T; ++q) {
            const uint32_t v = r.thist[q * P + tid];
            tot += v;
            before += q < t ? v : 0u;
        }
        s_tot[tid] = tot;
// ... 269 lines not shown
            if (n_a[k] > 0)
                qbig_layout(ws_a[k], n_cap, &b.a[i]);
            if (n_g[k] > 0)
                qbig_layout(ws_g[k], n_cap, &b.g[i]);
            b.a[i].n = static_cast<int>(n_a[k]);
            b.g[i].n = static_cast<int>(n_g[k]);
            const QLayout q = queue_layout(queues[k], n_cap, width);
            b.qh[i] = q.hdr;
            z.qh[z.count++] = q.hdr;
            b.mirror[i] = counts_host ? counts_host[k] : nullptr;
            b.epoch[i] = epochs ? epochs[k] : 0u;
            b.coop[i] = q.coop;
            b.wave[i] = q.wave;
            b.copy[i] = q.copy;
            b.cap_coop = q.cap_coop;
            b.cap_wave = q.cap_wave;
            b.cap_copy = q.cap_copy;
        }
        if (b.count == 0)
            continue;
        const size_t need = qjoin_lds_bytes(kQMax, kQMax), res = qjoin_lds_resident_bytes(kQMax);
        const size_t lds1 = need > res ? need : res;
        b.lds_bytes = static_cast<uint32_t>(lds1);
        hipLaunchKernelGGL(qbzero_kernel, dim3(z.count), dim3(64), 0, stream, z);
        HA_LAUNCH_CHECK();
        hipLaunchKernelGGL(qbqueue_kernel<true>, dim3(2 * (P / 4), b.count), dim3(1024), 4 * kQSubJoinLds, stream, b);
        hipLaunchKernelGGL(qbqueue_kernel<false>, dim3(2 * (P / 4), b.count), dim3(1024), lds1, stream, b);
        HA_LAUNCH_CHECK();
    }
    return 0;
}

}

using namespace ha;

extern "C" int64_t ha_qstep_max_ids(void) { return kQMax; }

extern "C" int ha_qstep_init(void) {
    const float *ids = nullptr;
    const uint64_t *ids64 = nullptr;
    if (qplan_batch<float>(&ids, nullptr, nullptr, 0, nullptr) || qplan_batch<uint64_t>(&ids64, nullptr, nullptr, 0, nullptr) ||
        qqueue_batch(0, 4, nullptr, nullptr, nullptr, nullptr, nullptr, 1, 0, nullptr))
        return -1;
    return lds_atomics_lane_ordered();
}

extern "C" size_t ha_qstep_queue_bytes(int64_t n_cap, int64_t width) {
    if (n_cap < 1 || width < 4)
        return 0;
    return queue_layout(nullptr, n_cap, width).bytes;
}

extern "C" int ha_qplan_batch_f32ids(const float *const *ids, const int64_t *n, void *const *plans, int64_t count,
                                     ha_stream_t stream) {
    return qplan_batch<float>(ids, n, plans, count, as_stream(stream));
}
extern "C" int ha_qplan_batch_u64ids(const uint64_t *const *ids, const int64_t *n, void *const *plans, int64_t count,
                                     ha_stream_t stream) {
    return qplan_batch<uint64_t>(ids, n, plans, count, as_stream(stream));
}
extern "C" int ha_qqueue_batch(int64_t rows, int64_t width, void *const *plans_a, const int64_t *n_a,
                               void *const *plans_g, const int64_t *n_g, void *const *queues, int64_t queue_n_cap,
                               int64_t count, ha_stream_t stream) {
    return qqueue_batch(rows, width, plans_a, n_a, plans_g, n_g, queues, queue_n_cap, count, as_stream(stream));
}
extern "C" int ha_qapply(float *table, int64_t rows, int64_t width, void *plan_cur, int64_t n_cur, const float *grads,
                         float lr, void *plan_next, int64_t n_next, float *next_out, const void *queue_cur,
                         int64_t queue_n_cap, ha_stream_t stream) {
    return qapply(table, rows, width, plan_cur, n_cur, grads, lr, plan_next, n_next, next_out, queue_cur, queue_n_cap,
                  as_stream(stream));
}
extern "C" int ha_qapply_sized(float *table, int64_t rows, int64_t width, void *plan_cur, int64_t n_cur, const float *grads,
                               float lr, void *plan_next, int64_t n_next, float *next_out, const void *queue_cur,
                               int64_t queue_n_cap, int64_t wave_items, ha_stream_t stream) {
    return qapply(table, rows, width, plan_cur, n_cur, grads, lr, plan_next, n_next, next_out, queue_cur, queue_n_cap,
                  as_stream(stream), nullptr, wave_items);
}
extern "C" int ha_qapply_steps(float *table, int64_t rows, int64_t width, float lr, int64_t queue_n_cap, int64_t count,
                               void *const *plan_cur, const int64_t *n_cur, const float *const *grads,
                               void *const *plan_next, const int64_t *n_next, float *const *next_out,
                               const void *const *queue_cur, const int64_t *wave_items, ha_stream_t stream) {
    HA_REQUIRE(count >= 0 && (count == 0 || (plan_cur && n_cur && grads && plan_next && n_next && next_out && queue_cur)),
               "ha_qapply_steps: null pointer");
    for (int64_t k = 0; k < count; ++k)
        if (qapply(table, rows, width, plan_cur[k], n_cur[k], grads[k], lr, plan_next[k], n_next[k], next_out[k],
                   queue_cur[k], queue_n_cap, as_stream(stream), nullptr, wave_items ? wave_items[k] : -1))
            return -1;
    return 0;
}

extern "C" void *ha_event_create(void) {
    hipEvent_t e = nullptr;
    if (hipEventCreateWithFlags(&e, hipEventDisableTiming) != hipSuccess)
        return nullptr;
    return e;
}
extern "C" int ha_event_destroy(void *event) {
    if (event)
        HA_CHECK_HIP(hipEventDestroy(static_cast<hipEvent_t>(event)));
    return 0;
}
extern "C" int ha_event_record(void *event, ha_stream_t stream) {
    HA_REQUIRE(event != nullptr, "ha_event_record: null event");
    HA_CHECK_HIP(hipEventRecord(static_cast<hipEvent_t>(event), as_stream(stream)));
    return 0;
}
extern "C" int ha_stream_wait_event(ha_stream_t stream, void *event) {
    HA_REQUIRE(event != nullptr, "ha_stream_wait_event: null event");
    HA_CHECK_HIP(hipStreamWaitEvent(as_stream(stream), static_cast<hipEvent_t>(event), 0));
    return 0;
}
extern "C" int ha_qqueue_batch_epochs(int64_t rows, int64_t width, void *const *plans_a, const int64_t *n_a,
                                      void *const *plans_g, const int64_t *n_g, void *const *queues, int64_t queue_n_cap,
                                      int64_t count, uint32_t *const *counts_host, const uint32_t *epochs,
                                      ha_stream_t stream) {
    return qqueue_batch(rows, width, plans_a, n_a, plans_g, n_g, queues, queue_n_cap, count, as_stream(stream), nullptr,
                        counts_host, epochs);
}
extern "C" int ha_qapply_steps_sync(float *table, int64_t rows, int64_t width, float lr, int64_t queue_n_cap, int64_t count,
                                    void *const *plan_cur, const int64_t *n_cur, const float *const *grads,
                                    void *const *plan_next, const int64_t *n_next, float *const *next_out,
                                    const void *const *queue_cur, const int64_t *wave_items, const uint32_t *epochs,
                                    uint32_t *err, void *done_event, ha_stream_t stream) {
    HA_REQUIRE(count >= 0 && (count == 0 || (plan_cur && n_cur && grads && plan_next && n_next && next_out && queue_cur)),
               "ha_qapply_steps_sync: null pointer");
    for (int64_t k = 0; k < count; ++k)
        if (qapply(table, rows, width, plan_cur[k], n_cur[k], grads[k], lr, plan_next[k], n_next[k], next_out[k],
                   queue_cur[k], queue_n_cap, as_stream(stream), nullptr, wave_items ? wave_items[k] : -1,
                   epochs ? epochs[k] : 0u, err, k + 1 == count ? static_cast<hipEvent_t>(done_event) : nullptr))
            return -1;
    if (count == 0 && done_event)
        HA_CHECK_HIP(hipEventRecord(static_cast<hipEvent_t>(done_event), as_stream(stream)));
    return 0;
}
extern "C" int ha_qapply_steps_counts(float *table, int64_t rows, int64_t width, float lr, int64_t queue_n_cap, int64_t count,
                                      void *const *plan_cur, const int64_t *n_cur, const float *const *grads,
                                      void *const *plan_next, const int64_t *n_next, float *const *next_out,
                                      const void *const *queue_cur, const int64_t *wave_items,
                                      const uint32_t *const *counts_host, const uint32_t *epochs, uint32_t *err,
                                      void *done_event, ha_stream_t stream) {
    (void)counts_host;
    return ha_qapply_steps_sync(table, rows, width, lr, queue_n_cap, count, plan_cur, n_cur, grads, plan_next, n_next, next_out,
                                queue_cur, wave_items, epochs, err, done_event, stream);
}
extern "C" int ha_qapply_sync(float *table, int64_t rows, int64_t width, void *plan_cur, int64_t n_cur, const float *grads,
                              float lr, void *plan_next, int64_t n_next, float *next_out, const void *queue_cur,
                              int64_t queue_n_cap, int64_t wave_items, uint32_t epoch, uint32_t *err, void *done_event,
                              ha_stream_t stream) {
    return qapply(table, rows, width, plan_cur, n_cur, grads, lr, plan_next, n_next, next_out, queue_cur, queue_n_cap,
                  as_stream(stream), nullptr, wave_items, epoch, err, static_cast<hipEvent_t>(done_event));
}

extern "C" int ha_qqueue_batch_counts(int64_t rows, int64_t width, void *const *plans_a, const int64_t *n_a,
                                      void *const *plans_g, const int64_t *n_g, void *const *queues, int64_t queue_n_cap,
                                      int64_t count, uint32_t *const *counts_host, ha_stream_t stream) {
    return qqueue_batch(rows, width, plans_a, n_a, plans_g, n_g, queues, queue_n_cap, count, as_stream(stream), nullptr,
                        counts_host);
}

template <typename IdT>
static int qprep_one(int64_t rows, int64_t width, const IdT *ahead_ids, int64_t n_ahead, void *plan_ahead, void *plan_a,
                     int64_t n_a, void *plan_g, int64_t n_g, void *queue_build, int64_t queue_n_cap, hipStream_t s) {
    if (n_ahead > 0 && qplan_batch<IdT>(&ahead_ids, &n_ahead, &plan_ahead, 1, s))
        return -1;
    if (n_a > 0 || n_g > 0)
        return qqueue_batch(rows, width, &plan_a, &n_a, &plan_g, &n_g, &queue_build, queue_n_cap, 1, s);
    return 0;
}
extern "C" int ha_qprep_f32ids(int64_t rows, int64_t width, const float *ahead_ids, int64_t n_ahead, void *plan_ahead,
                               void *plan_a, int64_t n_a, void *plan_g, int64_t n_g, void *queue_build,
                               int64_t queue_n_cap, ha_stream_t stream) {
    return qprep_one<float>(rows, width, ahead_ids, n_ahead, plan_ahead, plan_a, n_a, plan_g, n_g, queue_build,
                            queue_n_cap, as_stream(stream));
}
extern "C" int ha_qprep_u64ids(int64_t rows, int64_t width, const uint64_t *ahead_ids, int64_t n_ahead, void *plan_ahead,
                               void *plan_a, int64_t n_a, void *plan_g, int64_t n_g, void *queue_build,
                               int64_t queue_n_cap, ha_stream_t stream) {
    return qprep_one<uint64_t>(rows, width, ahead_ids, n_ahead, plan_ahead, plan_a, n_a, plan_g, n_g, queue_build,
                               queue_n_cap, as_stream(stream));
}
extern "C" int ha_qstep_f32ids(float *table, int64_t rows, int64_t width, void *plan_cur, int64_t n_cur,
                               const float *grads, float lr, void *plan_next, int64_t n_next, float *next_out,
                               const void *queue_cur, void *plan_b1, int64_t n_b1, void *queue_build,
                               int64_t queue_n_cap, const float *ahead_ids, int64_t n_ahead, void *plan_ahead,
                               ha_stream_t stream) {
    if (qprep_one<float>(rows, width, ahead_ids, n_ahead, plan_ahead, plan_next, n_next, plan_b1, n_b1, queue_build,
                         queue_n_cap, as_stream(stream)))
        return -1;
    return qapply(table, rows, width, plan_cur, n_cur, grads, lr, plan_next, n_next, next_out, queue_cur, queue_n_cap,
                  as_stream(stream));
}
extern "C" int ha_qstep_u64ids(float *table, int64_t rows, int64_t width, void *plan_cur, int64_t n_cur,
                               const float *grads, float lr, void *plan_next, int64_t n_next, float *next_out,
                               const void *queue_cur, void *plan_b1, int64_t n_b1, void *queue_build,
                               int64_t queue_n_cap, const uint64_t *ahead_ids, int64_t n_ahead, void *plan_ahead,
                               ha_stream_t stream) {
    if (qprep_one<uint64_t>(rows, width, ahead_ids, n_ahead, plan_ahead, plan_next, n_next, plan_b1, n_b1, queue_build,
                            queue_n_cap, as_stream(stream)))
        return -1;
    return qapply(table, rows, width, plan_cur, n_cur, grads, lr, plan_next, n_next, next_out, queue_cur, queue_n_cap,
                  as_stream(stream));
}

extern "C" int64_t ha_qbig_max_ids(void) { return kQBigMax; }
extern "C" size_t ha_qbig_plan_bytes(int64_t n_cap) {
    if (n_cap < 1 || n_cap > kQBigMax)
        return 0;
    return qbig_layout(nullptr, n_cap, nullptr);
}
extern "C" int ha_qbig_buckets(int64_t n_cap) { return n_cap >= 1 && n_cap <= kQBigMax ? qbig_buckets(n_cap) : 0; }
extern "C" int ha_qbig_plan_batch_f32ids(const float *const *ids, const int64_t *n, void *const *ws, int64_t n_cap,
                                         int64_t count, ha_stream_t stream) {
    return qbig_plan_batch<float>(ids, n, ws, n_cap, count, as_stream(stream));
}
extern "C" int ha_qbig_plan_batch_u64ids(const uint64_t *const *ids, const int64_t *n, void *const *ws, int64_t n_cap,
                                         int64_t count, ha_stream_t stream) {
    return qbig_plan_batch<uint64_t>(ids, n, ws, n_cap, count, as_stream(stream));
}
extern "C" int ha_qbig_queue_batch(int64_t rows, int64_t width, void *const *ws_a, const int64_t *n_a, void *const *ws_g,
                                   const int64_t *n_g, void *const *queues, int64_t n_cap, int64_t count,
                                   uint32_t *const *counts_host, const uint32_t *epochs, ha_stream_t stream) {
    return qbig_queue_batch(rows, width, ws_a, n_a, ws_g, n_g, queues, n_cap, count, counts_host, epochs, as_stream(stream));
}
extern "C" int ha_qbig_apply(float *table, int64_t rows, int64_t width, void *ws_cur, int64_t n_cur, const float *grads,
                             float lr, void *ws_next, int64_t n_next, float *next_out, const void *queue_cur, int64_t n_cap,
                             int64_t coop_items, uint32_t epoch, uint32_t *err, void *done_event, ha_stream_t stream) {
    HA_REQUIRE(n_cap >= 1 && n_cap <= kQBigMax && (n_cur == 0 || ws_cur) && (n_next == 0 || ws_next), "ha_qbig_apply: bad arguments");
    QBigRef a, g;
    memset(&a, 0, sizeof(a));
    memset(&g, 0, sizeof(g));
    if (n_cur > 0)
        qbig_layout(ws_cur, n_cap, &a);
    if (n_next > 0)
        qbig_layout(ws_next, n_cap, &g);
    return qapply_lists(table, rows, width, a.gperm, n_cur, grads, lr, g.gperm, n_next, next_out, queue_cur, n_cap, kQBigMax,
                        as_stream(stream), nullptr, -1, epoch, err, static_cast<hipEvent_t>(done_event), coop_items);
}
extern "C" int ha_qbig_plan_view(void *ws, int64_t n_cap, void **boff, void **bhdr, void **uniq, void **counts, void **seg,
                                 void **gperm, void **meta) {
    HA_REQUIRE(ws && n_cap >= 1 && n_cap <= kQBigMax, "ha_qbig_plan_view: bad arguments");
    QBigRef r;
    qbig_layout(ws, n_cap, &r);
    if (boff) *boff = r.boff;
    if (bhdr) *bhdr = r.bhdr;
    if (uniq) *uniq = r.uniq;
    if (counts) *counts = r.counts;
    if (seg) *seg = r.seg;
    if (gperm) *gperm = r.gperm;
    if (meta) *meta = r.meta;
    return 0;
}

extern "C" int ha_debug_qapply(float *table, int64_t rows, int64_t width, void *plan_cur, int64_t n_cur,
                               const float *grads, float lr, void *plan_next, int64_t n_next, float *next_out,
                               const void *queue_cur, int64_t queue_n_cap, unsigned long long *dbg, ha_stream_t stream) {
    HA_REQUIRE(dbg != nullptr, "qapply timeline: null debug buffer");
    return qapply(table, rows, width, plan_cur, n_cur, grads, lr, plan_next, n_next, next_out, queue_cur, queue_n_cap,
                  as_stream(stream), dbg);
}
extern "C" int ha_debug_qprep_f32ids(int64_t rows, int64_t width, const float *ahead_ids, int64_t n_ahead,
                                     void *plan_ahead, void *plan_a, int64_t n_a, void *plan_g, int64_t n_g,
                                     void *queue_build, int64_t queue_n_cap, unsigned long long *ph, ha_stream_t stream) {
    HA_REQUIRE(ph != nullptr, "qprep phases: null debug buffer");
    if (n_ahead > 0 && qplan_batch<float>(&ahead_ids, &n_ahead, &plan_ahead, 1, as_stream(stream), ph))
        return -1;
    if (n_a > 0 || n_g > 0)
        return qqueue_batch(rows, width, &plan_a, &n_a, &plan_g, &n_g, &queue_build, queue_n_cap, 1, as_stream(stream),
                            ph + 16);
    return 0;
}

extern "C" const uint32_t *ha_qstep_queue_header(const void *queue) {
    return reinterpret_cast<const uint32_t *>(queue);
}
```

herald_amd/ops.py:

```python
import ctypes
import os

import numpy as np

import torch

from . import _lib
from ._lib import DLArray, DLContext, DLStream, PlanView, check


def _stream_ptr(stream=None):
    if stream is None:
        return ctypes.c_void_p(torch._C._cuda_getCurrentRawStream(torch.cuda.current_device()))
    if isinstance(stream, int):
        return ctypes.c_void_p(stream)
    return ctypes.c_void_p(stream.cuda_stream)


def _ptr(t):
    return ctypes.c_void_p(t.data_ptr())


def _raw_stream(stream=None):
    p = _stream_ptr(stream).value
# ... 523 lines not shown
        L = _lib.load()
        ptr = [ctypes.c_void_p() for _ in range(7)]
        check(L.ha_qbig_plan_view(_ptr(self.ws), self.capacity, *[ctypes.byref(p) for p in ptr]), "ha_qbig_plan_view")
        torch.cuda.synchronize(self.device)
        base = self.ws.data_ptr()

        def arr(p, count, dtype):
            off = p.value - base
            return self.ws[off:off + count * dtype.itemsize].view(dtype).cpu().numpy()
        P, n = self.buckets, self.n
        boff = arr(ptr[0], P + 1, torch.int32).astype(np.int64)
        hdr = arr(ptr[1], P * 32, torch.int64).reshape(P, 32)
        uniq = arr(ptr[2], max(n, 1), torch.int32).astype(np.int64) & 0xFFFFFFFF
        counts = arr(ptr[3], max(n, 1), torch.int32).astype(np.int64)
        gperm = arr(ptr[5], max(n, 1), torch.int32).astype(np.int64)
        meta = arr(ptr[6], 1, torch.int32)
        keys, cnts, lists = [], [], []
        for p in range(P):
            U = int(hdr[p, 0])
            o = int(boff[p])
            keys.append(uniq[o:o + U])
            cnts.append(counts[o:o + U])
            lists.append(gperm[o:int(boff[p + 1])])
        return {"overflow": int(meta[0]), "bucket_sizes": np.diff(boff), "uniq": np.concatenate(keys) if keys else uniq[:0],
                "counts": np.concatenate(cnts) if cnts else counts[:0], "perm": np.concatenate(lists) if lists else gperm[:0]}


def qstep_max_ids():
    return int(_lib.load().ha_qstep_max_ids())


class SortAheadPipeline:

    NBLOCKS = 3

    def __init__(self, table, max_ids, lr, block=8, key_limit=None, device=None, finish_ahead=None):
        _require(table, torch.float32, "table")
        self.table, self.lr, self.block = table, float(lr), int(block)
        self.device = table.device if device is None else torch.device(device)
        self.key_limit = int(table.shape[0]) if key_limit is None else int(key_limit)
        self.finish_ahead = bool(finish_ahead)
        self.plans = [[IndexPlan(max_ids, self.device) for _ in range(self.block)] for _ in range(self.NBLOCKS)]
        self.side = torch.cuda.Stream(device=self.device)
        self._sorted = [torch.cuda.Event() for _ in range(self.NBLOCKS)]
        self._freed = [None] * self.NBLOCKS
        self._first = [0] * self.NBLOCKS
        self._count = [0] * self.NBLOCKS
        self._next_block = 0
        self._waited = -1

    def prepare_block(self, ids_list):
        if not 0 < len(ids_list) <= self.block:
            raise ValueError("a block holds 1..%d batches" % self.block)
        b = self._next_block
        slot = b % self.NBLOCKS
        self.side.wait_stream(torch.cuda.current_stream(self.device))
        with torch.cuda.stream(self.side):
            if self._freed[slot] is not None:
                self.side.wait_event(self._freed[slot])
            for i, ids in enumerate(ids_list):
                if self.finish_ahead:
                    self.plans[slot][i].build(ids, stream=self.side, key_limit=self.key_limit)
                else:
                    self.plans[slot][i].sort(ids, stream=self.side, key_limit=self.key_limit)
            self._sorted[slot].record(self.side)
        self._first[slot] = (self._first[(b - 1) % self.NBLOCKS] + self._count[(b - 1) % self.NBLOCKS]) if b else 0
        self._count[slot] = len(ids_list)
        self._next_block = b + 1
        return b

    def _plan(self, k, stream):
        for b in range(max(self._next_block - self.NBLOCKS, 0), self._next_block):
            slot = b % self.NBLOCKS
            if self._first[slot] <= k < self._first[slot] + self._count[slot]:
                if b > self._waited:
                    (stream or torch.cuda.current_stream(self.device)).wait_event(self._sorted[slot])
                    self._waited = b
                return slot, k - self._first[slot]
        raise ValueError("step %d is not in a prepared block" % k)

    def lookup(self, k, ids, out=None, stream=None):
        self._plan(k, stream)
        return embedding_lookup(self.table, ids, out=out, stream=stream)

    def apply(self, k, grads, stream=None):
        slot, i = self._plan(k, stream)
        if self.finish_ahead:
            sgd_apply(self.table, self.plans[slot][i], grads, self.lr, stream=stream, finished=True)
            self.plans[slot][i].produced_on(self.side)
        else:
            sgd_apply_finish(self.table, self.plans[slot][i], grads, self.lr, stream=stream)
        if i == self._count[slot] - 1:
            ev = torch.cuda.Event()
            ev.record(stream or torch.cuda.current_stream(self.device))
            self._freed[slot] = ev
        return self.plans[slot][i]


class QueueStepPipeline:

    def __init__(self, table, capacity, lr, device=None, block=8, overlap=True, sync="events", min_flags_block=8):
        L = _lib.load()
        _require(table, torch.float32, "table")
        self.table, self.lr = table, float(lr)
        self.device = table.device if device is None else torch.device(device)
        self.wide = capacity > qstep_max_ids()
        if capacity > qbig_max_ids():
            raise ValueError("ha_qstep_* takes at most %d ids per batch (got capacity %d): use SortAheadPipeline / "
                             "lookup_sort + sgd_apply_finish" % (qbig_max_ids(), capacity))
        if table.shape[1] % 4 != 0:
            raise ValueError("ha_qstep_* needs rows of a multiple of 4 floats")
        with torch.cuda.device(self.device):
            if L.ha_qstep_init() < 0:
                check(-1, "ha_qstep_init")
        self.capacity = max(int(capacity), 1)
        self.overlap = bool(overlap)
        if sync not in ("events", "flags"):
            raise ValueError("sync must be 'events' or 'flags'")
        self.sync = sync if self.overlap else "events"
        if self.sync == "flags" and int(block) < int(min_flags_block):
            self.sync = "events"
        self._done_ev, self._cev_pool = {}, []
        self._cev_busy = []
        self.block = int(block) if self.overlap else 1
        if not 1 <= self.block <= 64:
            raise ValueError("block must be 1..64")
        self.LOOKAHEAD = 3 * self.block
        self.NPLAN, self.NQUEUE = 4 * self.block, 2 * self.block
        self.ROTATION = 4 * self.block
        self.plans = [(WidePlan if self.wide else IndexPlan)(self.capacity, self.device) for _ in range(self.NPLAN)]
        self.queue_bytes = int(L.ha_qstep_queue_bytes(self.capacity, table.shape[1]))
        self.queues = torch.zeros(self.NQUEUE * self.queue_bytes, dtype=torch.uint8, device=self.device)
        torch.cuda.current_stream(self.device).synchronize()
        side_prio = 0
        if os.environ.get("HA_QSIDE_PRIO") in ("low", "high"):
            try:
                lo_hi = torch.cuda.Stream.priority_range()
                side_prio = max(lo_hi) if os.environ["HA_QSIDE_PRIO"] == "low" else min(lo_hi)
            except Exception:
                side_prio = 0
        self.side = torch.cuda.Stream(device=self.device, priority=side_prio) if self.overlap else None
        self.COUNTS = 8192
        self.counts = torch.zeros((self.COUNTS, 4), dtype=torch.int32).pin_memory()
        self._counts_np = self.counts.numpy()
        self._counts_c = (ctypes.c_int32 * (self.COUNTS * 4)).from_address(self.counts.data_ptr())
        self._counts_base = self.counts.data_ptr()
        self._L = L
        self._plan_ptr = [p.ws.data_ptr() for p in self.plans]
        self._queue_ptr = [self.queues.data_ptr() + q * self.queue_bytes for q in range(self.NQUEUE)]
        self._ev_pool = []
        self._last_items = 0
        self.fallbacks, self._fb_plan, self._wide_ids = 0, None, {}
        self._enq_last = None
        self.reset()

    def close(self):
        for ev in list(self._done_ev.values()) + self._cev_pool + [e for e, _ in self._cev_busy]:
            self._L.ha_event_destroy(ev)
        self._done_ev, self._cev_pool, self._cev_busy = {}, [], []

    def __del__(self):
        try:
            self.close()
        except Exception:
            pass

    def reset(self, stream=None):
        if self._done_ev:
            if self.side is not None:
                marker = self._event() if hasattr(self, "_ev_pool") else torch.cuda.Event()
                marker.record(self.side)
                self._cev_busy.extend((e, marker) for e in self._done_ev.values())
            else:
                self._cev_pool.extend(self._done_ev.values())
        self._done_ev = {}
        self.c, self.n, self.shape, self.ids = None, {}, {}, {}
        self._enq_last, self._covered = None, -(1 << 60)
        self._ev_side = {}
        self._held = {}
        return self

    def plan_of(self, b):
        return self.plans[b % self.NPLAN]

    def _queue(self, c):
        return self.queues.data_ptr() + (c % self.NQUEUE) * self.queue_bytes

    def queue_header(self, c):
        off = (c % self.NQUEUE) * self.queue_bytes
        torch.cuda.synchronize(self.device)
        h = self.queues[off:off + 40].view(torch.int32).cpu().tolist()
        d = dict(zip(("wave_items", "workgroup_items", "long", "medium", "small", "copy_items"), h))
        d["overflow"] = int(h[8] != 0 or h[9] != 0)
        return d

    def overflowed(self):
        return bool((self._counts_np[:, 3] & ~4).any())

    def _raise_if_failed(self, steps):
        cc, ring = self._counts_c, self.COUNTS
        for j in steps:
            f = cc[4 * (j % ring) + 3]
            if f & ~4:
                raise RuntimeError("QueueStepPipeline: step %d failed on the device (flags %d: 1 = queue overflow, 2 = an "
                                   "occurrence list out of position order, 8 = an apply launch gave up waiting -- its queue was "
                                   "never completed, or an item it depends on never finished; the table is partly updated)"
                                   % (j, f))

    def prepare_block(self, b, ids_of, stream=None, ph=None):
        L = self._L
        rows, width = self.table.shape
        main = stream if stream is not None else torch.cuda.current_stream(self.device)
        B = self.block
        s = self.side if self.overlap else main
        sp = _stream_ptr(s)
        vp, i64 = ctypes.c_void_p, ctypes.c_int64
        flags = self.sync == "flags"
        self._raise_if_failed(range(max((b - 2) * B, 0), max((b - 1) * B, 0)))
        if self.overlap and flags:
            cev = self._done_ev.pop(b - 1, None)
            if cev is not None:
                check(L.ha_stream_wait_event(sp, cev), "ha_stream_wait_event")
                marker = self._event()
                marker.record(s)
                self._cev_busy.append((cev, marker))
                self._covered = b * B - 1
            elif self._enq_last is not None and self._enq_last > self._covered:
                ev = self._event()
                ev.record(main)
                s.wait_event(ev)
                self._ev_pool.append(ev)
                self._covered = self._enq_last
        elif self.overlap:
            ev = self._event()
            ev.record(main)
            s.wait_event(ev)
        sel = {"f32ids": [], "u64ids": []}
        held = []
        for j in range((b + 2) * B, (b + 3) * B):
            t = ids_of(j)
            if t is None:
                continue
            m = t.numel()
            if m == 0:
                continue
            if m > self.capacity:
                raise ValueError("plan capacity %d < %d ids" % (self.capacity, m))
            if not t.is_cuda or not t.is_contiguous():
                raise ValueError("ids must be contiguous device tensors")
            sel[_ids_kind(t)].append((j, t, m))
            held.append(t)
            self.n[j] = m
            if self.wide:
                self._wide_ids[j] = t
                self._wide_ids.pop(j - 5 * B, None)
        for kind, lst in sel.items():
            if not lst:
                continue
            cnt = len(lst)
            ids_arr = (vp * cnt)(*[t.data_ptr() for _, t, _ in lst])
            n_arr = (i64 * cnt)(*[m for _, _, m in lst])
            pl_arr = (vp * cnt)(*[self._plan_ptr[j % self.NPLAN] for j, _, _ in lst])
            if ph is not None and kind == "f32ids":
                j0, t0, m0 = lst[0]
                check(L.ha_debug_qprep_f32ids(rows, width, _ptr(t0), m0, _ptr(self.plan_of(j0).ws), None, 0,
                                              None, 0, None, self.capacity, _ptr(ph), sp), "ha_debug_qprep")
            if self.wide:
                check(getattr(L, "ha_qbig_plan_batch_" + kind)(ids_arr, n_arr, pl_arr, self.capacity, cnt, sp),
                      "ha_qbig_plan_batch")
            else:
                check(getattr(L, "ha_qplan_batch_" + kind)(ids_arr, n_arr, pl_arr, cnt, sp), "ha_qplan_batch")
            for j, _, m in lst:
                pl = self.plans[j % self.NPLAN]
                pl.n = m
                pl._view = None
                pl._produced_on = sp.value if sp.value is not None else 0
        self._held[b] = held
        self._held.pop(b - 2, None)
        nget = self.n.get
        steps = [j for j in range((b + 1) * B, (b + 2) * B) if nget(j, 0) or nget(j + 1, 0)]
        if steps:
            cnt = len(steps)
            pp, NP, NQ = self._plan_ptr, self.NPLAN, self.NQUEUE
            pa = (vp * cnt)(*[pp[j % NP] if nget(j, 0) else None for j in steps])
            na = (i64 * cnt)(*[nget(j, 0) for j in steps])
            pg = (vp * cnt)(*[pp[(j + 1) % NP] if nget(j + 1, 0) else None for j in steps])
            ng = (i64 * cnt)(*[nget(j + 1, 0) for j in steps])
            qs = (vp * cnt)(*[self._queue_ptr[j % NQ] for j in steps])
            if ph is not None:
                check(L.ha_debug_qprep_f32ids(rows, width, None, 0, None, pa[0], na[0], pg[0], ng[0], qs[0], self.capacity,
                                              _ptr(ph), sp), "ha_debug_qprep")
            base, ring, cc = self._counts_base, self.COUNTS, self._counts_c
            for j in steps:
                at = 4 * (j % ring)
                cc[at] = 0
                cc[at + 2] = 0
                cc[at + 3] &= ~4
            cs = (vp * cnt)(*[base + 16 * (j % ring) for j in steps])
            eps = (ctypes.c_uint32 * cnt)(*[self._epoch(j) for j in steps])
            if self.wide:
                check(L.ha_qbig_queue_batch(rows, width, pa, na, pg, ng, qs, self.capacity, cnt, cs, eps, sp),
                      "ha_qbig_queue_batch")
            else:
                check(L.ha_qqueue_batch_epochs(rows, width, pa, na, pg, ng, qs, self.capacity, cnt, cs, eps, sp),
                      "ha_qqueue_batch")
        if self.overlap and not flags:
            ev = self._event()
            ev.record(s)
            self._ev_side[b] = ev
            ready = self._ev_side.pop(b - 1, None)
            if ready is not None:
                main.wait_event(ready)
                self._ev_pool.append(ready)

    def _event(self):
        return self._ev_pool.pop() if self._ev_pool else torch.cuda.Event()

    @staticmethod
    def _epoch(j):
        return (j + (1 << 24)) & 0xFFFFFFFF

    def _block_done_event(self, c):
        if self.sync != "flags" or (c + 1) % self.block != 0:
            return None
        if not self._cev_pool and self._cev_busy and self._cev_busy[0][1].query():
            old_ev, marker = self._cev_busy.pop(0)
            self._ev_pool.append(marker)
            self._cev_pool.append(old_ev)
        ev = self._cev_pool.pop() if self._cev_pool else ctypes.c_void_p(self._L.ha_event_create())
        if not ev:
            raise RuntimeError("ha_event_create failed")
        old = self._done_ev.pop(c // self.block, None)
        if old is not None:
            self._cev_pool.append(old)
        self._done_ev[c // self.block] = ev
        return ev

    def _err_ptr(self, c):
        return ctypes.c_void_p(self._counts_base + 16 * (c % self.COUNTS) + 12)

    def wave_items(self, c):
        at = 4 * (c % self.COUNTS)
        if self._counts_c[at + 3]:
            raise RuntimeError("ha_qqueue_batch: the work queue of step %d is unusable (flags %d: 1 = overflow, 2 = an "
                               "occurrence list out of position order, 4 = a hash bucket of a wide batch holds more than "
                               "%d ids)" % (c, self._counts_c[at + 3], qstep_max_ids()))
        if os.environ.get("HA_QHINT") == "0":
            return -1
        w, cp = self._counts_c[at], self._counts_c[at + 2]
        return w + cp - 2 if w > 0 and cp > 0 else -1

    def apply(self, c, grads, out, stream=None, dbg=None, n_cur=None, n_next=None):
        L = self._L
        t = self.table
        rows, width = t.shape
        n_cur = self.n.get(c, 0) if n_cur is None else int(n_cur)
        n_next = self.n.get(c + 1, 0) if n_next is None else int(n_next)
        if n_cur:
            _require(grads, torch.float32, "grads")
            if grads.numel() != n_cur * width:
                raise ValueError("grads must hold %d x %d values" % (n_cur, width))
        if n_next:
            _require(out, torch.float32, "out")
            if out.numel() != n_next * width:
                raise ValueError("out must hold %d x %d values" % (n_next, width))
        flags = self.sync == "flags" and dbg is None
        capturing = flags and torch.cuda.is_current_stream_capturing()
        if capturing:
            raise RuntimeError("QueueStepPipeline(sync='flags'): steps cannot be captured into a hipGraph (use sync='events')")
        done = self._block_done_event(c) if flags else None
        self._enq_last = c if self._enq_last is None else max(self._enq_last, c)
        if not (n_cur or n_next):
            if done is not None:
                check(L.ha_event_record(done, _stream_ptr(stream)), "ha_event_record")
            return
        args = [_ptr(t), rows, width, _ptr(self.plan_of(c).ws) if n_cur else None, n_cur,
                _ptr(grads) if n_cur else None, ctypes.c_float(self.lr),
                _ptr(self.plan_of(c + 1).ws) if n_next else None, n_next, _ptr(out) if n_next else None,
                self._queue(c), self.capacity]
        if self.wide:
            flag, coop = self._wide_built(c)
            if flag & 4:
                self._wide_fallback(c, grads, out, stream, n_cur, n_next, done)
                return
            if flag:
                self.wave_items(c)
            check(L.ha_qbig_apply(*args, coop, self._epoch(c) if flags else 0, self._err_ptr(c) if flags else None, done,
                                  _stream_ptr(stream)), "ha_qbig_apply")
        elif flags:
            check(L.ha_qapply_sync(*args, self.wave_items(c), self._epoch(c), self._err_ptr(c), done, _stream_ptr(stream)),
                  "ha_qapply_sync")
        elif dbg is None:
            check(L.ha_qapply_sized(*args, self.wave_items(c), _stream_ptr(stream)), "ha_qapply")
        else:
            check(L.ha_debug_qapply(*args, _ptr(dbg), _stream_ptr(stream)), "ha_debug_qapply")

    def _wide_built(self, c, timeout=20.0):
        import time
        at = 4 * (c % self.COUNTS)
        cc = self._counts_c
        if cc[at] == 0:
            t0 = time.perf_counter()
            while cc[at] == 0:
                if time.perf_counter() - t0 > timeout:
                    raise RuntimeError("QueueStepPipeline: the queue of step %d was not built within %.0f s (was its block "
                                       "prepared?)" % (c, timeout))
        return cc[at + 3], max(cc[at + 1] - 1, 0)

    def _wide_fallback(self, c, grads, out, stream, n_cur, n_next, done):
        self.fallbacks += 1
        if n_cur:
            if self._fb_plan is None:
                self._fb_plan = IndexPlan(self.capacity, self.device)
            self._fb_plan.build(self._wide_ids[c], stream=stream)
            sgd_apply(self.table, self._fb_plan, grads.reshape(n_cur, -1), self.lr, stream=stream, finished=True)
        if n_next:
            embedding_lookup(self.table, self._wide_ids[c + 1].reshape(-1), out=out.reshape(n_next, -1), stream=stream)
        if done is not None:
            check(self._L.ha_event_record(done, _stream_ptr(stream)), "ha_event_record")

    def apply_call(self, c, grads, out, stream, n_cur, n_next, sized=True):
        if self.sync == "flags":
            raise RuntimeError("apply_call: use apply / apply_steps_call with sync='flags'")
        L = self._L
        t = self.table
        rows, width = t.shape
        hint = ctypes.c_int64(-1)
        args = (ctypes.c_void_p(t.data_ptr()), ctypes.c_int64(rows), ctypes.c_int64(width),
                ctypes.c_void_p(self.plan_of(c).ws.data_ptr() if n_cur else None), ctypes.c_int64(n_cur),
                ctypes.c_void_p(grads.data_ptr() if n_cur else None), ctypes.c_float(self.lr),
                ctypes.c_void_p(self.plan_of(c + 1).ws.data_ptr() if n_next else None), ctypes.c_int64(n_next),
                ctypes.c_void_p(out.data_ptr() if n_next else None), ctypes.c_void_p(self._queue(c)),
                ctypes.c_int64(self.capacity), hint, _stream_ptr(stream))
        fn = L.ha_qapply_sized

        def call(k):
            self._enq_last = k if self._enq_last is None else max(self._enq_last, k)
            if sized:
                hint.value = self.wave_items(k)
            if fn(*args) != 0:
                check(-1, "ha_qapply")
        return call

    def apply_steps_call(self, c0, grads_list, out_list, stream, n, sized=True):
        L = self._L
        t = self.table
        rows, width = t.shape
        cnt = len(grads_list)
        vp, i64 = ctypes.c_void_p, ctypes.c_int64
        pc = (vp * cnt)(*[self.plan_of(c0 + i).ws.data_ptr() for i in range(cnt)])
        pn = (vp * cnt)(*[self.plan_of(c0 + i + 1).ws.data_ptr() for i in range(cnt)])
        ns = (i64 * cnt)(*[n] * cnt)
        gs = (vp * cnt)(*[g.data_ptr() for g in grads_list])
        os_ = (vp * cnt)(*[o.data_ptr() for o in out_list])
        qs = (vp * cnt)(*[self._queue(c0 + i) for i in range(cnt)])
        hints = (i64 * cnt)(*[-1] * cnt)
        head = (vp(t.data_ptr()), i64(rows), i64(width), ctypes.c_float(self.lr), i64(self.capacity), i64(cnt))
        sp = _stream_ptr(stream)
        fn = L.ha_qapply_steps
        counts, ring = self._counts_c, self.COUNTS
        flags = self.sync == "flags"
        eps = (ctypes.c_uint32 * cnt)()
        fn_sync, epoch, last_err = L.ha_qapply_steps_counts, self._epoch, self._err_ptr
        B = self.block
        cs = (vp * cnt)()
        base = self._counts_base
        use_counts = os.environ.get("HA_QCOUNTS", "0") != "0"

        def call(k0):
            if flags and k0 // B != (k0 + cnt - 1) // B:
                raise RuntimeError("apply_steps_call(sync='flags'): steps %d..%d cross a block boundary (block = %d)"
                                   % (k0, k0 + cnt - 1, B))
            self._enq_last = k0 + cnt - 1 if self._enq_last is None else max(self._enq_last, k0 + cnt - 1)
            if sized:
                for i in range(cnt):
                    at = 4 * ((k0 + i) % ring)
                    w, cp = counts[at], counts[at + 2]
                    if counts[at + 3]:
                        raise RuntimeError("ha_qqueue_batch: the work queue of step %d is unusable (flags %d: 1 = overflow, "
                                           "2 = an occurrence list out of position order)" % (k0 + i, counts[at + 3]))
                    if w > 0 and cp > 0:
                        self._last_items = w + cp - 2
                    hints[i] = w + cp - 2 if w > 0 and cp > 0 else (self._last_items * 17) // 16 if self._last_items > 0 else -1
                    cs[i] = base + 4 * at if use_counts else None
            if flags:
                for i in range(cnt):
                    eps[i] = epoch(k0 + i)
                done = self._block_done_event(k0 + cnt - 1)
                if fn_sync(*head, pc, ns, gs, pn, ns, os_, qs, hints, cs if sized else None, eps, last_err(k0 + cnt - 1), done,
                           sp) != 0:
                    check(-1, "ha_qapply_steps_counts")
            elif fn(*head, pc, ns, gs, pn, ns, os_, qs, hints, sp) != 0:
                check(-1, "ha_qapply_steps")
        return call

    def _call(self, c, grads, ahead_ids, out, stream):
        if c % self.block == 0:
            self.prepare_block(c // self.block, lambda j: self.ids.get(j), stream)
            for j in [j for j in self.ids if j < c + 3 * self.block]:
                del self.ids[j]
        if ahead_ids is not None and ahead_ids.numel():
            self.ids[c + self.LOOKAHEAD] = ahead_ids
            self.shape[c + self.LOOKAHEAD] = tuple(ahead_ids.shape)
        n_next = self.n.get(c + 1, 0)
        if n_next and out is None:
            out = torch.empty(tuple(self.shape[c + 1]) + (self.table.shape[1],), dtype=torch.float32,
                              device=self.table.device)
        self.apply(c, grads, out, stream)
        for d in (self.n, self.shape):
            d.pop(c - 1, None)
        self.c = c + 1
        return out if n_next else None

    def start(self, ids, out=None, stream=None):
        ids = list(ids)
        if len(ids) > self.LOOKAHEAD:
            raise ValueError("start takes the first %d batches" % self.LOOKAHEAD)
        ids = ids + [None] * (self.LOOKAHEAD - len(ids))
        self.reset()
        res = None
        for k, b in enumerate(ids):
            c = k - self.LOOKAHEAD
            res = self._call(c, None, b, out if c == -1 else None, stream)
        return res

    def step(self, grads, ahead_ids=None, out=None, stream=None):
        if self.c is None:
            raise RuntimeError("QueueStepPipeline.step before start")
        return self._call(self.c, grads, ahead_ids, out, stream)


def push_apply_finish(table, plan, grads, stream=None):
    _require(table, torch.float32, "table")
    _require(grads, torch.float32, "grads")
    check(_lib.load().ha_push_apply_finish(_ptr(table), table.shape[0], table.shape[1], _ptr(plan.ws),
                                           plan.n, _ptr(grads), _stream_ptr(stream)),
          "ha_push_apply_finish")
    plan.produced_on(stream)
    return table


def dl_call(name, arrays, scalars=(), stream=None):
    L = _lib.load()
    holders = [DLHolder(a) for a in arrays]
    sh = DLStreamHolder(stream)
    args = [h.handle for h in holders] + list(scalars) + [sh.handle]
    check(getattr(L, name)(*args), name)


class IndexedSlices:

    def __init__(self, indices=None, values=None, dense_shape=None, push_indices=None):
        self.indices = indices
        self.values = values
        self.dense_shape = dense_shape
        self.push_indices = push_indices
        self.deduplicated = False

    def get_dense_shape(self):
        assert self.dense_shape is not None
        return self.dense_shape

    def get_sparse_shape(self):
        return tuple(self.values.shape)

    def update(self, indices, values, dense_shape, push_indices=None):
        self.indices = indices
        self.push_indices = push_indices
        self.values = values
        if self.dense_shape is not None:
            assert tuple(self.dense_shape) == tuple(dense_shape)
        else:
            self.dense_shape = dense_shape
        self.deduplicated = False

    def deduplicate(self, stream=None):
        ids = self.indices.reshape(-1)
        n = ids.numel()
        width = self.values.shape[-1]
        plan = IndexPlan(max(n, 1), device=ids.device).build(ids, stream)
        reduced = dedup_reduce(plan, self.values.reshape(n, width), stream=stream)
        uniq_f32, _ = plan.export_f32(stream)
        u = uniq_f32.numel()
        self.indices = uniq_f32
        self.values = reduced[:u]
        if self.push_indices is not None:
            pids = self.push_indices.reshape(-1)
            pplan = IndexPlan(max(pids.numel(), 1), device=pids.device).build(pids, stream)
            self.push_indices, _ = pplan.export_f32(stream)
        self.deduplicated = True
        return self

    def to_dense(self, stream=None):
        dense = torch.zeros(tuple(self.get_dense_shape()), dtype=torch.float32, device=self.values.device)
        dl_call("IndexedSlices2Dense", [self.values.contiguous(), self.indices.contiguous(), dense],
                stream=stream)
        return dense
```

herald_amd/streams.py:

```python
import os

import torch

_PICKED = {}


def _probe(main, side, buf, small, blocks=6, per=12):
    import ctypes
    from . import _lib
    L = _lib.load()
    booked = [torch.cuda.Event() for _ in range(blocks)]
    done = [torch.cuda.Event() for _ in range(blocks)]
    e0, e1 = torch.cuda.Event(enable_timing=True), torch.cuda.Event(enable_timing=True)
    for b in range(blocks):
        with torch.cuda.stream(side):
            if b >= 2:
                side.wait_event(done[b - 2])
            L.ha_debug_occupy(16, 1024, 96 * 1024, 2500, ctypes.c_void_p(side.cuda_stream))
            L.ha_debug_occupy(32, 256, 64, 5000, ctypes.c_void_p(side.cuda_stream))
            small.add_(1)
            booked[b].record(side)
        with torch.cuda.stream(main):
            if b == 2:
                e0.record(main)
            main.wait_event(booked[b])
            for i in range(per):
                buf.fill_(float(i))
            done[b].record(main)
    with torch.cuda.stream(main):
        e1.record(main)
    e1.synchronize()
    side.synchronize()
    return e0.elapsed_time(e1) / ((blocks - 2) * per)


def pick_side_stream(main, priority=0, candidates=4):
    if main is None:
        main = torch.cuda.current_stream()
    dev = main.device
    key = (dev.index, main.cuda_stream, priority)
    if key in _PICKED:
        return _PICKED[key]
    first = torch.cuda.Stream(device=dev, priority=priority)
    if os.environ.get("HA_STREAM_CALIBRATE", "1") == "0" or candidates <= 1:
        _PICKED[key] = first
        return first
    buf = torch.empty(8 << 20, dtype=torch.float32, device=dev)
    small = torch.zeros(1 << 16, device=dev)
    torch.cuda.synchronize(dev)
    cands, times = [first], []
    for i in range(candidates):
        if i:
            cands.append(torch.cuda.Stream(device=dev, priority=priority))
        times.append(_probe(main, cands[i], buf, small))
        if i and times[i] < 1.5 * min(times) and times[0] < 1.5 * min(times):
            break
    best = min(range(len(times)), key=lambda i: times[i])
    pick = cands[0] if times[0] < 1.5 * times[best] else cands[best]
    torch.cuda.synchronize(dev)
    del buf, small
    _PICKED[key] = pick
    return pick
```

include/herald_amd.h:

```cpp
#ifndef HERALD_AMD_H_
#define HERALD_AMD_H_

#include <stddef.h>
#include <stdint.h>

#ifdef __cplusplus
extern "C" {
#endif

typedef enum { kCPU = 1, kGPU = 2 } DLDeviceType;
typedef struct {
    int device_id;
    DLDeviceType device_type;
} DLContext;
typedef struct {
    void *data;
    DLContext ctx;
    int ndim;
    int64_t *shape;
    int64_t *stride;
} DLArray;
typedef struct {
    int device_id;
    void *handle;
// ... 123 lines not shown
                        ha_stream_t stream);
int ha_plan_sort_u64ids(const uint64_t *ids, int64_t n, void *ws,
                        ha_stream_t stream);
int ha_plan_build_batch_f32ids_lim(const float *const *ids, const int64_t *n, void *const *ws, int count,
                                   uint64_t key_limit, ha_stream_t stream);
int ha_plan_build_batch_u64ids_lim(const uint64_t *const *ids, const int64_t *n, void *const *ws, int count,
                                   uint64_t key_limit, ha_stream_t stream);
int ha_plan_sort_batch_f32ids_lim(const float *const *ids, const int64_t *n, void *const *ws, int count,
                                  uint64_t key_limit, ha_stream_t stream);
int ha_plan_sort_batch_u64ids_lim(const uint64_t *const *ids, const int64_t *n, void *const *ws, int count,
                                  uint64_t key_limit, ha_stream_t stream);
int ha_plan_build_f32ids_lim(const float *ids, int64_t n, void *ws, uint64_t key_limit, ha_stream_t stream);
int ha_plan_sort_f32ids_lim(const float *ids, int64_t n, void *ws, uint64_t key_limit, ha_stream_t stream);
int ha_plan_build_u64ids_lim(const uint64_t *ids, int64_t n, void *ws, uint64_t key_limit, ha_stream_t stream);
int ha_plan_sort_u64ids_lim(const uint64_t *ids, int64_t n, void *ws, uint64_t key_limit, ha_stream_t stream);
int ha_plan_finish(void *ws, int64_t n, ha_stream_t stream);
int ha_plan_build_u32keys(const uint32_t *keys, int64_t n, void *ws,
                          int key_bits, ha_stream_t stream);
int ha_plan_export_f32(const void *ws, int64_t n, float *uniq_f32,
                       float *inverse_f32, ha_stream_t stream);

int ha_dedup_reduce(const void *plan_ws, int64_t n, const float *grads,
                    int64_t width, float *reduced, ha_stream_t stream);

int ha_dedup_reduce_scaled(const void *plan_ws, int64_t n, const float *grads,
                           int64_t width, float scale, float *reduced,
                           ha_stream_t stream);

int ha_sgd_apply(float *table, int64_t rows, int64_t width,
                 const void *plan_ws, int64_t n, const float *grads, float lr,
                 ha_stream_t stream);
int ha_sgd_apply_finished(float *table, int64_t rows, int64_t width, void *plan_ws, int64_t n, const float *grads,
                          float lr, ha_stream_t stream);

int ha_push_apply(float *table, int64_t rows, int64_t width,
                  const void *plan_ws, int64_t n, const float *grads,
                  ha_stream_t stream);

int ha_apply_mapped(float *dst, int64_t dst_rows, int64_t width,
                    const void *plan_ws, int64_t n, const float *src, float lr,
                    const int32_t *rowmap, const int32_t *valmap,
                    const uint8_t *dst_init, ha_stream_t stream);
int ha_apply_mapped2(float *dst, int64_t dst_rows, float *dst2, int64_t width,
                     const void *plan_ws, int64_t n, const float *src, float lr,
                     const int32_t *rowmap, const int32_t *rowmap2,
                     const uint8_t *dst_init, ha_stream_t stream);

int ha_sparse_opt_fused_f32ids(int kind, float *param, int64_t rows, int64_t width, const float *ids,
                               int64_t n, const float *grads, float *state1, float *state2,
                               const float *hyper_host, void *plan_ws, ha_stream_t stream);

int ha_lookup_sort_f32ids(const float *table, int64_t rows, int64_t width,
                          const float *ids, int64_t n, float *out,
                          void *plan_ws, ha_stream_t stream);
int ha_lookup_sort_u64ids(const float *table, int64_t rows, int64_t width,
                          const uint64_t *ids, int64_t n, float *out,
                          void *plan_ws, ha_stream_t stream);
int ha_sgd_apply_finish(float *table, int64_t rows, int64_t width,
                        void *plan_ws, int64_t n, const float *grads, float lr,
                        ha_stream_t stream);
int ha_push_apply_finish(float *table, int64_t rows, int64_t width,
                         void *plan_ws, int64_t n, const float *grads,
                         ha_stream_t stream);

size_t ha_pend_bytes(void);
int ha_pend_reset(void *pend, ha_stream_t stream);
int ha_lookup_sort_pend_f32ids(const float *table, int64_t rows, int64_t width,
                               const float *ids, int64_t n, float *out,
                               void *plan_ws, void *pend, ha_stream_t stream);
int ha_lookup_sort_pend_u64ids(const float *table, int64_t rows, int64_t width,
                               const uint64_t *ids, int64_t n, float *out,
                               void *plan_ws, void *pend, ha_stream_t stream);
int ha_sgd_push_pull_f32ids(float *table, int64_t rows, int64_t width,
                            void *plan_cur, int64_t n_cur, const float *grads, float lr,
                            void *pend_cur, const float *next_ids, int64_t n_next,
                            float *next_out, void *plan_next, void *pend_next,
                            ha_stream_t stream);
int ha_sgd_push_pull_u64ids(float *table, int64_t rows, int64_t width,
                            void *plan_cur, int64_t n_cur, const float *grads, float lr,
                            void *pend_cur, const uint64_t *next_ids, int64_t n_next,
                            float *next_out, void *plan_next, void *pend_next,
                            ha_stream_t stream);
int ha_debug_step_timeline(float *table, int64_t rows, int64_t width,
                           void *plan_cur, int64_t n_cur, const float *grads, float lr,
                           void *pend_cur, const float *next_ids, int64_t n_next,
                           float *next_out, void *plan_next, void *pend_next,
                           unsigned long long *dbg, ha_stream_t stream);
int64_t *ha_plan_handoff_timeout(void *plan_ws);

size_t ha_step_tab_bytes(void);
int64_t ha_step_max_ids(void);
int ha_step_tab_reset(void *tab, ha_stream_t stream);
int ha_step_f32ids(float *table, int64_t rows, int64_t width,
                   void *plan_cur, int64_t n_cur, const float *grads, float lr, const void *tab_cur,
                   void *plan_next, int64_t n_next, float *next_out, const void *tab_next,
                   void *plan_fin, int64_t n_fin, void *tab_fin,
                   const float *ahead_ids, int64_t n_ahead, void *plan_ahead,
                   void *tab_clear, ha_stream_t stream);
int ha_step_u64ids(float *table, int64_t rows, int64_t width,
                   void *plan_cur, int64_t n_cur, const float *grads, float lr, const void *tab_cur,
                   void *plan_next, int64_t n_next, float *next_out, const void *tab_next,
                   void *plan_fin, int64_t n_fin, void *tab_fin,
                   const uint64_t *ahead_ids, int64_t n_ahead, void *plan_ahead,
                   void *tab_clear, ha_stream_t stream);
int ha_debug_step_fwd_timeline(float *table, int64_t rows, int64_t width,
                               void *plan_cur, int64_t n_cur, const float *grads, float lr, const void *tab_cur,
                               void *plan_next, int64_t n_next, float *next_out, const void *tab_next,
                               void *plan_fin, int64_t n_fin, void *tab_fin,
                               const float *ahead_ids, int64_t n_ahead, void *plan_ahead,
                               void *tab_clear, unsigned long long *dbg, ha_stream_t stream);

int ha_qstep_init(void);
int64_t ha_qstep_max_ids(void);
size_t ha_qstep_queue_bytes(int64_t n_cap, int64_t width);
int ha_qplan_batch_f32ids(const float *const *ids, const int64_t *n, void *const *plans, int64_t count,
                          ha_stream_t stream);
int ha_qplan_batch_u64ids(const uint64_t *const *ids, const int64_t *n, void *const *plans, int64_t count,
                          ha_stream_t stream);
int ha_qqueue_batch(int64_t rows, int64_t width, void *const *plans_a, const int64_t *n_a, void *const *plans_g,
                    const int64_t *n_g, void *const *queues, int64_t queue_n_cap, int64_t count, ha_stream_t stream);
int ha_qapply(float *table, int64_t rows, int64_t width, void *plan_cur, int64_t n_cur, const float *grads, float lr,
              void *plan_next, int64_t n_next, float *next_out, const void *queue_cur, int64_t queue_n_cap,
              ha_stream_t stream);
int ha_qapply_sized(float *table, int64_t rows, int64_t width, void *plan_cur, int64_t n_cur, const float *grads,
                    float lr, void *plan_next, int64_t n_next, float *next_out, const void *queue_cur,
                    int64_t queue_n_cap, int64_t wave_items, ha_stream_t stream);
int ha_qapply_steps(float *table, int64_t rows, int64_t width, float lr, int64_t queue_n_cap, int64_t count,
                    void *const *plan_cur, const int64_t *n_cur, const float *const *grads, void *const *plan_next,
                    const int64_t *n_next, float *const *next_out, const void *const *queue_cur,
                    const int64_t *wave_items, ha_stream_t stream);
int ha_qqueue_batch_counts(int64_t rows, int64_t width, void *const *plans_a, const int64_t *n_a, void *const *plans_g,
                           const int64_t *n_g, void *const *queues, int64_t queue_n_cap, int64_t count,
                           uint32_t *const *counts_host, ha_stream_t stream);
void *ha_event_create(void);
int ha_event_destroy(void *event);
int ha_event_record(void *event, ha_stream_t stream);
int ha_stream_wait_event(ha_stream_t stream, void *event);
int ha_qqueue_batch_epochs(int64_t rows, int64_t width, void *const *plans_a, const int64_t *n_a, void *const *plans_g,
                           const int64_t *n_g, void *const *queues, int64_t queue_n_cap, int64_t count,
                           uint32_t *const *counts_host, const uint32_t *epochs, ha_stream_t stream);
int ha_qapply_steps_sync(float *table, int64_t rows, int64_t width, float lr, int64_t queue_n_cap, int64_t count,
                         void *const *plan_cur, const int64_t *n_cur, const float *const *grads, void *const *plan_next,
                         const int64_t *n_next, float *const *next_out, const void *const *queue_cur,
                         const int64_t *wave_items, const uint32_t *epochs, uint32_t *err, void *done_event,
                         ha_stream_t stream);
int ha_qapply_sync(float *table, int64_t rows, int64_t width, void *plan_cur, int64_t n_cur, const float *grads, float lr,
                   void *plan_next, int64_t n_next, float *next_out, const void *queue_cur, int64_t queue_n_cap,
                   int64_t wave_items, uint32_t epoch, uint32_t *err, void *done_event, ha_stream_t stream);
int ha_qapply_steps_counts(float *table, int64_t rows, int64_t width, float lr, int64_t queue_n_cap, int64_t count,
                           void *const *plan_cur, const int64_t *n_cur, const float *const *grads, void *const *plan_next,
                           const int64_t *n_next, float *const *next_out, const void *const *queue_cur,
                           const int64_t *wave_items, const uint32_t *const *counts_host, const uint32_t *epochs, uint32_t *err,
                           void *done_event, ha_stream_t stream);

int ha_xchg_available(void);
int ha_xchg_unique_id(void *id128);
void *ha_xchg_create(const void *id128, int world, int rank);
int ha_xchg_destroy(void *xchg);
int ha_xchg_bytes(void *xchg, const void *send, const int64_t *send_bytes, void *recv, const int64_t *recv_bytes,
                  ha_stream_t stream);
int ha_xchg_rows(void *xchg, const float *send, const int64_t *send_rows, float *recv, const int64_t *recv_rows, int64_t width,
                 ha_stream_t stream);

int64_t ha_qbig_max_ids(void);
size_t ha_qbig_plan_bytes(int64_t n_cap);
int ha_qbig_buckets(int64_t n_cap);
int ha_qbig_plan_batch_f32ids(const float *const *ids, const int64_t *n, void *const *ws, int64_t n_cap, int64_t count,
                              ha_stream_t stream);
int ha_qbig_plan_batch_u64ids(const uint64_t *const *ids, const int64_t *n, void *const *ws, int64_t n_cap, int64_t count,
                              ha_stream_t stream);
int ha_qbig_queue_batch(int64_t rows, int64_t width, void *const *ws_a, const int64_t *n_a, void *const *ws_g,
                        const int64_t *n_g, void *const *queues, int64_t n_cap, int64_t count, uint32_t *const *counts_host,
                        const uint32_t *epochs, ha_stream_t stream);
int ha_qbig_apply(float *table, int64_t rows, int64_t width, void *ws_cur, int64_t n_cur, const float *grads, float lr,
                  void *ws_next, int64_t n_next, float *next_out, const void *queue_cur, int64_t n_cap, int64_t coop_items,
                  uint32_t epoch, uint32_t *err, void *done_event, ha_stream_t stream);
int ha_qbig_plan_view(void *ws, int64_t n_cap, void **boff, void **bhdr, void **uniq, void **counts, void **seg, void **gperm,
                      void **meta);

int ha_qprep_f32ids(int64_t rows, int64_t width, const float *ahead_ids, int64_t n_ahead, void *plan_ahead,
                    void *plan_a, int64_t n_a, void *plan_g, int64_t n_g, void *queue_build, int64_t queue_n_cap,
                    ha_stream_t stream);
int ha_qprep_u64ids(int64_t rows, int64_t width, const uint64_t *ahead_ids, int64_t n_ahead, void *plan_ahead,
                    void *plan_a, int64_t n_a, void *plan_g, int64_t n_g, void *queue_build, int64_t queue_n_cap,
                    ha_stream_t stream);
int ha_qstep_f32ids(float *table, int64_t rows, int64_t width,
                    void *plan_cur, int64_t n_cur, const float *grads, float lr,
                    void *plan_next, int64_t n_next, float *next_out, const void *queue_cur,
                    void *plan_b1, int64_t n_b1, void *queue_build, int64_t queue_n_cap,
                    const float *ahead_ids, int64_t n_ahead, void *plan_ahead, ha_stream_t stream);
int ha_qstep_u64ids(float *table, int64_t rows, int64_t width,
                    void *plan_cur, int64_t n_cur, const float *grads, float lr,
                    void *plan_next, int64_t n_next, float *next_out, const void *queue_cur,
                    void *plan_b1, int64_t n_b1, void *queue_build, int64_t queue_n_cap,
                    const uint64_t *ahead_ids, int64_t n_ahead, void *plan_ahead, ha_stream_t stream);
const uint32_t *ha_qstep_queue_header(const void *queue);
int ha_debug_qapply(float *table, int64_t rows, int64_t width, void *plan_cur, int64_t n_cur, const float *grads,
                    float lr, void *plan_next, int64_t n_next, float *next_out, const void *queue_cur,
                    int64_t queue_n_cap, unsigned long long *dbg, ha_stream_t stream);
int ha_debug_qprep_f32ids(int64_t rows, int64_t width, const float *ahead_ids, int64_t n_ahead, void *plan_ahead,
                          void *plan_a, int64_t n_a, void *plan_g, int64_t n_g, void *queue_build, int64_t queue_n_cap,
                          unsigned long long *ph, ha_stream_t stream);

int ha_stream_gate(const uint32_t *flag, ha_stream_t stream);
int ha_debug_occupy(int64_t wgs, int64_t threads, int64_t lds_bytes, int64_t ticks, ha_stream_t stream);

int ha_sgd_apply_finish_prefetch_f32ids(float *table, int64_t rows, int64_t width,
                                        void *plan_ws, int64_t n, const float *grads, float lr,
                                        const float *next_ids, int64_t next_n, ha_stream_t stream);

int ha_shard_bucket(const void *plan_ws, int64_t n, const int64_t *starts_host,
                    int nshard, int32_t *offsets, uint32_t *local_keys,
                    ha_stream_t stream);

int ha_shard_route_f32ids(const float *ids, int64_t n, void *plan_ws,
                          const int64_t *starts_host, int nshard, int64_t *meta,
                          uint32_t *local_keys, ha_stream_t stream);
int ha_shard_route_u64ids(const uint64_t *ids, int64_t n, void *plan_ws,
                          const int64_t *starts_host, int nshard, int64_t *meta,
                          uint32_t *local_keys, ha_stream_t stream);

int ha_shard_route_pack_f32ids(const float *ids, int64_t n, void *plan_ws,
                               const int64_t *starts_host, int nshard, int64_t cap,
                               int64_t *meta, int32_t *send, ha_stream_t stream);
int ha_shard_route_pack_u64ids(const uint64_t *ids, int64_t n, void *plan_ws,
                               const int64_t *starts_host, int nshard, int64_t cap,
                               int64_t *meta, int32_t *send, ha_stream_t stream);
int ha_shard_route_unpack(const int32_t *recv, int nshard, int64_t cap, int64_t *recv_cnt,
                          uint32_t *keys_out, ha_stream_t stream);

int ha_shard_frames_route_f32ids(const float *ids, int64_t n, void *plan_ws, const int64_t *starts_host,
                                 int nshard, int64_t rcap, int64_t frame_stride, int32_t *send, int32_t *rowmap,
                                 int32_t *posmap, ha_stream_t stream);
int ha_shard_frames_route_u64ids(const uint64_t *ids, int64_t n, void *plan_ws, const int64_t *starts_host,
                                 int nshard, int64_t rcap, int64_t frame_stride, int32_t *send, int32_t *rowmap,
                                 int32_t *posmap, ha_stream_t stream);
int ha_shard_frames_pack(const void *plan_ws, int64_t n, const int64_t *starts_host, int nshard, int64_t rcap,
                         int64_t frame_stride, int32_t *send, int32_t *rowmap, int32_t *posmap, ha_stream_t stream);
int ha_shard_frames_unpack(const int32_t *recv, int nshard, int64_t rcap, int64_t frame_stride, uint32_t *keys_fixed,
                           int32_t *state, ha_stream_t stream);
int ha_shard_frames_pack_batch(const void *const *plan_ws, const int64_t *n, int count, const int64_t *starts_host,
                               int nshard, int64_t rcap, int64_t frame_stride, int32_t *send, int32_t *const *rowmap,
                               int32_t *const *posmap, ha_stream_t stream);
int ha_shard_frames_unpack_batch(const int32_t *recv, int count, int nshard, int64_t rcap, int64_t frame_stride,
                                 uint32_t *const *keys_fixed, int32_t *const *state, ha_stream_t stream);
int ha_shard_frames_serve_pull(const float *table, int64_t rows, int64_t width, const int32_t *recv, int nshard,
                               int64_t rcap, int64_t frame_stride, float *rows_out, uint32_t *keys_fixed,
                               int32_t *state, ha_stream_t stream);

int ha_shard_frames_pack_batch_sized(const void *const *plan_ws, const int64_t *n, int count, const int64_t *starts_host,
                                     int nshard, int self, int64_t rcap, int64_t frame_stride, int32_t *send,
                                     int32_t *const *rowmap, int32_t *const *posmap, int32_t *const *meta_dev,
                                     int32_t *const *meta_host, ha_stream_t stream);
int ha_shard_frames_unpack_batch_sized(const int32_t *recv, int count, int nshard, int64_t rcap, int64_t frame_stride,
                                       uint32_t *const *keys_fixed, int32_t *const *meta_dev, int32_t *const *meta_host,
                                       ha_stream_t stream);
int ha_shard_sized_serve_pull(const float *table, int64_t rows, int64_t width, const uint32_t *keys_fixed, int nshard,
                              int self, int64_t rcap, const int32_t *meta_dev, float *rows_out, ha_stream_t stream);
int ha_gather2_u32map(const float *table, int64_t rows, const float *recv, int64_t recv_rows, int64_t width,
                      const uint32_t *map, int64_t n, float *out, ha_stream_t stream);
int ha_shard_sized_serve_push(float *table, int64_t rows, int64_t width, const uint32_t *keys_fixed, int nshard, int self,
                              int64_t rcap, const int32_t *meta_dev, int64_t total, const float *push_buf, void *plan_ws,
                              ha_stream_t stream);
int ha_push_apply_scaled_finished(float *table, int64_t rows, int64_t width, void *plan_ws, int64_t n, const float *grads,
                                  float scale, ha_stream_t stream);

typedef struct ha_shard_slot {
    int32_t world, rank;
    int64_t rcap, n;
    void *plan_ws;
    const uint32_t *keys_fixed;
    const int32_t *meta_dev;
    const uint32_t *posmap;
    const int32_t *rowmap;
    const int32_t *counts_host;
    void *owner_plan_ws;
} ha_shard_slot;
int ha_shard_step_pull(const float *table, int64_t rows, int64_t width, const ha_shard_slot *slot, void *xchg, float *pull_send,
                       float *pull_recv, int64_t pull_rows, float *out, ha_stream_t stream);
int ha_shard_step_push(float *table, int64_t rows, int64_t width, const ha_shard_slot *slot, void *xchg, float *push_buf,
                       int64_t push_rows, const uint8_t *zero_flags, const float *values, float scale, ha_stream_t stream);
int ha_shard_step(float *table, int64_t rows, int64_t width, const ha_shard_slot *slot, void *xchg, float *pull_send,
                  float *pull_recv, int64_t pull_rows, float *push_buf, int64_t push_rows, const uint8_t *zero_flags, float *out,
                  const float *values, float scale, ha_stream_t stream);
int ha_shard_steps(float *table, int64_t rows, int64_t width, int64_t count, const ha_shard_slot *const *slots, void *xchg,
                   float *pull_send, float *pull_recv, int64_t pull_rows, float *push_buf, int64_t push_rows,
                   const uint8_t *zero_flags, float *const *outs, const float *const *values, float scale, ha_stream_t stream);

int ha_shard_serve_push(float *table, int64_t rows, int64_t width, const uint32_t *keys,
                        int64_t n, const float *values, void *plan_ws, ha_stream_t stream);

int ha_shard_frames_serve_push(float *table, int64_t rows, int64_t width, const uint32_t *keys_fixed, int nshard,
                               int64_t rcap, const float *values, void *plan_ws, ha_stream_t stream);

typedef struct ha_cache ha_cache;
ha_cache *ha_cache_create(int policy, int64_t limit, int64_t length,
                          int64_t width, int64_t max_batch);
void ha_cache_destroy(ha_cache *cache);
int ha_cache_set_bounds(ha_cache *cache, int64_t pull_bound, int64_t push_bound);
int ha_cache_set_bypass(ha_cache *cache, int bypass);
int ha_cache_bind_store(ha_cache *cache, float *table, int64_t *versions,
                        int64_t store_rows, int64_t row_start);
int ha_cache_lookup(ha_cache *cache, const void *keys, int key_kind, int64_t n,
                    float *dest, ha_stream_t stream);
int ha_cache_sort_ahead(ha_cache *cache, const void *keys, int key_kind, int64_t n, ha_stream_t stream);
int ha_cache_lookup_presorted(ha_cache *cache, const void *keys, int key_kind, int64_t n,
// ... 149 lines not shown
```

Before: 542.3 million.

## Split apply work into two hash-class chains run on concurrent streams

Rows in the queue builder are partitioned into two classes by a hash of the key, with separate counts and offsets for each class. The apply kernel can then process one class on the main stream and the other on a second chain stream, each with its own verdict, events and error words. A probe selects a chain stream that actually runs alongside the main one, using a host thread and condition variables on the C++ side. This aims to overlap apply work across independent row sets, at the cost of extra scans, header fields, host bookkeeping and stream-selection probing.

```diff
diff --git a/herald_amd/_build.py b/herald_amd/_build.py
--- a/herald_amd/_build.py
+++ b/herald_amd/_build.py
@@ -60,7 +60,7 @@
         if verbose and out.strip():
             print(out)
     if force or procs or _newer(objs, LIB):
-        _run([HIPCC, "--offload-arch=gfx950", "-shared", "-fPIC", "-fno-gpu-rdc", "-o", LIB] + objs)
+        _run([HIPCC, "--offload-arch=gfx950", "-shared", "-fPIC", "-fno-gpu-rdc", "-pthread", "-o", LIB] + objs)
     return LIB
 
 
diff --git a/herald_amd/_lib.py b/herald_amd/_lib.py
--- a/herald_amd/_lib.py
+++ b/herald_amd/_lib.py
@@ -111,6 +111,8 @@
     L.ha_qstep_init.argtypes = []
     L.ha_event_create.restype = vp
     L.ha_event_create.argtypes = []
+    L.ha_qchain_create.restype = vp
+    L.ha_qchain_create.argtypes = []
     L.ha_host_unmap.restype = c.c_int
     L.ha_host_unmap.argtypes = [vp]
     L.ha_qbig_max_ids.restype = i64
@@ -182,6 +184,10 @@
         "ha_qapply_steps_sync": [vp, i64, i64, f32, i64, i64, vp, vp, vp, vp, vp, vp, vp, vp, vp, vp, vp, vp],
         "ha_qapply_steps_counts": [vp, i64, i64, f32, i64, i64, vp, vp, vp, vp, vp, vp, vp, vp, vp, vp, vp, vp, vp],
         "ha_qapply_sync": [vp, i64, i64, vp, i64, vp, f32, vp, i64, vp, vp, i64, i64, c.c_uint32, vp, vp, vp],
+        "ha_qqueue_batch_chains": [i64, i64, vp, vp, vp, vp, vp, i64, i64, vp, vp, vp, vp],
+        "ha_qchain_destroy": [vp],
+        "ha_qapply_steps_chains": [vp, vp, i64, i64, f32, i64, i64, vp, vp, vp, vp, vp, vp, vp, vp, vp, vp, vp, vp, vp, vp, vp,
+                                   vp],
         "ha_xchg_available": [],
         "ha_xchg_unique_id": [vp],
         "ha_xchg_destroy": [vp],
diff --git a/herald_amd/csrc/qstep.hip b/herald_amd/csrc/qstep.hip
--- a/herald_amd/csrc/qstep.hip
+++ b/herald_amd/csrc/qstep.hip
@@ -1,4 +1,7 @@
 #include <hip/hip_ext.h>
+#include <condition_variable>
+#include <new>
+#include <thread>
 
 #include "plan_dev.h"
 #include "gather_dev.h"
@@ -29,7 +32,10 @@
     uint32_t overflow_wave, overflow_copy;
     uint32_t epoch_wave, epoch_copy, done;
     uint32_t verdict;
-    uint32_t reserved[50];
+    uint32_t n_wave0, n_coop0, n_copy0;
+    uint32_t n_long0, n_medium0, n_small0, n_copy_medium0, n_copy_small0;
+    uint32_t verdict1;
+    uint32_t reserved[41];
 };
 static_assert(sizeof(QHeader) == 256, "queue header is one 256-byte line");
 struct QEntry {
@@ -112,6 +118,7 @@
     float *out;
     int ncoop, nworker;
     uint32_t epoch;
+    uint32_t sel;
     uint32_t *err;
     unsigned long long *dbg;
 };
@@ -495,7 +502,33 @@
     uint32_t st_base, fs_base;
     uint32_t tid, nt;
     int tbits;
+    uint32_t two;
 };
+__device__ __forceinline__ uint32_t q_class(uint32_t key) {
+    return ((key * 0x85EBCA6Bu) >> 12) & 1u;
+}
+struct QCount2 {
+    QCount a, b;
+};
+__device__ __forceinline__ QCount q_pick(const QCount2 &t, uint32_t cl) {
+    QCount r;
+    r.g = cl ? t.b.g : t.a.g;
+    r.l = cl ? t.b.l : t.a.l;
+    r.m = cl ? t.b.m : t.a.m;
+    r.s = cl ? t.b.s : t.a.s;
+    return r;
+}
+__device__ __forceinline__ QCount2 q_put(QCount2 t, uint32_t cl, QCount v) {
+    t.a.g = cl ? t.a.g : v.g;
+    t.a.l = cl ? t.a.l : v.l;
+    t.a.m = cl ? t.a.m : v.m;
+    t.a.s = cl ? t.a.s : v.s;
+    t.b.g = cl ? v.g : t.b.g;
+    t.b.l = cl ? v.l : t.b.l;
+    t.b.m = cl ? v.m : t.b.m;
+    t.b.s = cl ? v.s : t.b.s;
+    return t;
+}
 
 __device__ __forceinline__ uint32_t qjoin_probe(const QJoin &j, uint32_t key) {
     uint32_t h = q_hash(key, j.tbits);
@@ -527,7 +560,7 @@
 }
 
 template <int R0, int R1>
-__device__ __forceinline__ QCount qjoin_count_groups(const QJoin &j, QCount t) {
+__device__ __forceinline__ QCount2 qjoin_count_groups(const QJoin &j, QCount2 t) {
     const uint32_t tid = j.tid, last = static_cast<uint32_t>(max(j.Ua, 1) - 1);
     uint32_t ka[R1 - R0], c[R1 - R0];
 #pragma unroll
@@ -539,14 +572,15 @@
 #pragma unroll
     for (int r = R0; r < R1; ++r) {
         if (static_cast<int>(static_cast<uint32_t>(r) * j.nt + tid) < j.Ua) {
-            const uint32_t mf = qjoin_dest(j, qjoin_probe(j, ka[r - R0]));
-            t = q_count(t, q_kind(c[r - R0], mf & 0xFFFFu, ka[r - R0] < j.rows), j.per512, j.per128, j.per32, c[r - R0]);
+            const uint32_t mf = qjoin_dest(j, qjoin_probe(j, ka[r - R0])), cl = q_class(ka[r - R0]) & j.two;
+            t = q_put(t, cl, q_count(q_pick(t, cl), q_kind(c[r - R0], mf & 0xFFFFu, ka[r - R0] < j.rows), j.per512, j.per128,
+                                     j.per32, c[r - R0]));
         }
     }
     return t;
 }
 template <int R0, int R1>
-__device__ __forceinline__ QCount qjoin_emit_groups(const QJoin &j, QCount b) {
+__device__ __forceinline__ QCount2 qjoin_emit_groups(const QJoin &j, QCount2 b) {
     const uint32_t tid = j.tid, last = static_cast<uint32_t>(max(j.Ua, 1) - 1);
     uint32_t ka[R1 - R0], cst[R1 - R0], o01[R1 - R0], o2[R1 - R0];
 #pragma unroll
@@ -561,16 +595,16 @@
 #pragma unroll
     for (int r = R0; r < R1; ++r) {
         if (static_cast<int>(static_cast<uint32_t>(r) * j.nt + tid) < j.Ua) {
-            const uint32_t mf = qjoin_dest(j, qjoin_probe(j, ka[r - R0]));
-            b = qjoin_emit_one(j, b, j.bwave, j.bcap_wave, ka[r - R0], cst[r - R0] & 0xFFFFu, cst[r - R0] >> 16,
-                               mf & 0xFFFFu, mf >> 16, o01[r - R0], o2[r - R0]);
+            const uint32_t mf = qjoin_dest(j, qjoin_probe(j, ka[r - R0])), cl = q_class(ka[r - R0]) & j.two;
+            b = q_put(b, cl, qjoin_emit_one(j, q_pick(b, cl), j.bwave, j.bcap_wave, ka[r - R0], cst[r - R0] & 0xFFFFu,
+                                            cst[r - R0] >> 16, mf & 0xFFFFu, mf >> 16, o01[r - R0], o2[r - R0]));
         }
     }
     return b;
 }
 
 template <int R0, int R1>
-__device__ __forceinline__ QCount qjoin_count_copies(const QJoin &j, QCount t) {
+__device__ __forceinline__ QCount2 qjoin_count_copies(const QJoin &j, QCount2 t) {
     const uint32_t tid = j.tid, last = static_cast<uint32_t>(max(j.Ug, 1) - 1);
     uint32_t kg[R1 - R0], m[R1 - R0];
 #pragma unroll
@@ -581,12 +615,14 @@
     }
 #pragma unroll
     for (int r = R0; r < R1; ++r)
-        if (static_cast<int>(static_cast<uint32_t>(r) * j.nt + tid) < j.Ug && qjoin_probe(j, kg[r - R0]) == kQTabEmpty)
-            t = q_count(t, q_kind(0u, m[r - R0], kg[r - R0] < j.rows), j.per512, j.per128, j.per32, 0u);
+        if (static_cast<int>(static_cast<uint32_t>(r) * j.nt + tid) < j.Ug && qjoin_probe(j, kg[r - R0]) == kQTabEmpty) {
+            const uint32_t cl = q_class(kg[r - R0]) & j.two;
+            t = q_put(t, cl, q_count(q_pick(t, cl), q_kind(0u, m[r - R0], kg[r - R0] < j.rows), j.per512, j.per128, j.per32, 0u));
+        }
     return t;
 }
 template <int R0, int R1>
-__device__ __forceinline__ QCount qjoin_emit_copies(const QJoin &j, QCount b) {
+__device__ __forceinline__ QCount2 qjoin_emit_copies(const QJoin &j, QCount2 b) {
     const uint32_t tid = j.tid, last = static_cast<uint32_t>(max(j.Ug, 1) - 1);
     uint32_t kg[R1 - R0], mfs[R1 - R0];
 #pragma unroll
@@ -597,9 +633,11 @@
     }
 #pragma unroll
     for (int r = R0; r < R1; ++r)
-        if (static_cast<int>(static_cast<uint32_t>(r) * j.nt + tid) < j.Ug && qjoin_probe(j, kg[r - R0]) == kQTabEmpty)
-            b = qjoin_emit_one(j, b, j.bcopy, j.bcap_copy, kg[r - R0], 0u, 0u, mfs[r - R0] & 0xFFFFu, mfs[r - R0] >> 16,
-                               0u, 0u);
+        if (static_cast<int>(static_cast<uint32_t>(r) * j.nt + tid) < j.Ug && qjoin_probe(j, kg[r - R0]) == kQTabEmpty) {
+            const uint32_t cl = q_class(kg[r - R0]) & j.two;
+            b = q_put(b, cl, qjoin_emit_one(j, q_pick(b, cl), j.bcopy, j.bcap_copy, kg[r - R0], 0u, 0u, mfs[r - R0] & 0xFFFFu,
+                                            mfs[r - R0] >> 16, 0u, 0u));
+        }
     return b;
 }
 
@@ -610,7 +648,8 @@
                                            uint32_t *lds, uint32_t lds_bytes, const int part,
                                            unsigned long long *ph = nullptr, uint32_t *mirror = nullptr,
                                            const uint32_t st_base = 0, const uint32_t fs_base = 0,
-                                           const uint32_t epoch = 0, const uint32_t wide_parts = 0, const bool signal = true) {
+                                           const uint32_t epoch = 0, const uint32_t wide_parts = 0, const bool signal = true,
+                                           const uint32_t two = 0, uint32_t *mirror1 = nullptr) {
     constexpr int TS = 1 << TBITS;
     const int tid = static_cast<int>(threadIdx.x) & (NT - 1), w = tid >> 6;
     q_phase(ph, 0);
@@ -618,6 +657,7 @@
     j.tid = static_cast<uint32_t>(tid);
     j.nt = NT;
     j.tbits = TBITS;
+    j.two = WIDE ? 0u : two;
     j.pa = pa;
     j.pg = pg;
     j.st_base = st_base;
@@ -666,7 +706,7 @@
     }
     __syncthreads();
     q_phase(ph, 2);
-    QCount t{0u, 0u, 0u, 0u};
+    QCount2 t{{0u, 0u, 0u, 0u}, {0u, 0u, 0u, 0u}};
     if (part == 0) {
         if (j.Ua > 0)
             t = qjoin_count_groups<0, 4>(j, t);
@@ -674,11 +714,24 @@
             t = qjoin_count_groups<4, 8>(j, t);
         q_phase(ph, 3);
         uint32_t nL, nM, nS, nG;
-        QCount b;
-        b.l = qscan_n<NT / 64>(t.l, j.s_w, &nL, w);
-        b.m = qscan_n<NT / 64>(t.m, j.s_w, &nM, w) + nL;
-        b.s = qscan_n<NT / 64>(t.s, j.s_w, &nS, w) + nL + nM;
-        b.g = qscan_n<NT / 64>(t.g, j.s_w, &nG, w);
+        QCount2 b{{0u, 0u, 0u, 0u}, {0u, 0u, 0u, 0u}};
+        b.a.l = qscan_n<NT / 64>(t.a.l, j.s_w, &nL, w);
+        b.a.m = qscan_n<NT / 64>(t.a.m, j.s_w, &nM, w) + nL;
+        b.a.s = qscan_n<NT / 64>(t.a.s, j.s_w, &nS, w) + nL + nM;
+        b.a.g = qscan_n<NT / 64>(t.a.g, j.s_w, &nG, w);
+        const uint32_t nL0 = nL, nM0 = nM, nS0 = nS, nG0 = nG;
+        if (j.two) {
+            uint32_t nL1, nM1, nS1, nG1;
+            const uint32_t w0 = nL + nM + nS;
+            b.b.l = qscan_n<NT / 64>(t.b.l, j.s_w, &nL1, w) + w0;
+            b.b.m = qscan_n<NT / 64>(t.b.m, j.s_w, &nM1, w) + w0 + nL1;
+            b.b.s = qscan_n<NT / 64>(t.b.s, j.s_w, &nS1, w) + w0 + nL1 + nM1;
+            b.b.g = qscan_n<NT / 64>(t.b.g, j.s_w, &nG1, w) + nG;
+            nL += nL1;
+            nM += nM1;
+            nS += nS1;
+            nG += nG1;
+        }
         if (WIDE) {
             __syncthreads();
             if (tid == 0) {
@@ -701,10 +754,10 @@
             }
             __syncthreads();
             const uint32_t bw = j.s_w[20], bc = j.s_w[21];
-            b.l += bw;
-            b.m += bw;
-            b.s += bw;
-            b.g += bc;
+            b.a.l += bw;
+            b.a.m += bw;
+            b.a.s += bw;
+            b.a.g += bc;
         }
         if (!WIDE && tid == 0) {
             bqh->n_wave = min(nL + nM + nS, bcap_wave);
@@ -712,6 +765,11 @@
             bqh->n_long = nL;
             bqh->n_medium = nM;
             bqh->n_small = nS;
+            bqh->n_wave0 = min(nL0 + nM0 + nS0, bcap_wave);
+            bqh->n_coop0 = min(nG0, bcap_coop);
+            bqh->n_long0 = nL0;
+            bqh->n_medium0 = nM0;
+            bqh->n_small0 = nS0;
             uint32_t over = (nL + nM + nS > bcap_wave || nG > bcap_coop) ? 1u : 0u;
             if ((pa.n > 0 && pa.hdr->reserved[kOrderFlagWord] != 0) || (pg.n > 0 && pg.hdr->reserved[kOrderFlagWord] != 0))
                 over |= 2u;
@@ -721,6 +779,10 @@
                 mirror[1] = min(nG, bcap_coop) + 1u;
                 if (over)
                     mirror[3] = over;
+            }
+            if (mirror1) {
+                mirror1[0] = min(nL + nM + nS, bcap_wave) - min(nL0 + nM0 + nS0, bcap_wave) + 1u;
+                mirror1[1] = min(nG, bcap_coop) - min(nG0, bcap_coop) + 1u;
             }
         }
         q_phase(ph, 4);
@@ -737,9 +799,17 @@
             t = qjoin_count_copies<4, 8>(j, t);
         q_phase(ph, 3);
         uint32_t nM, nS;
-        QCount b{0u, 0u, 0u, 0u};
-        b.m = qscan_n<NT / 64>(t.m, j.s_w, &nM, w);
-        b.s = qscan_n<NT / 64>(t.s, j.s_w, &nS, w) + nM;
+        QCount2 b{{0u, 0u, 0u, 0u}, {0u, 0u, 0u, 0u}};
+        b.a.m = qscan_n<NT / 64>(t.a.m, j.s_w, &nM, w);
+        b.a.s = qscan_n<NT / 64>(t.a.s, j.s_w, &nS, w) + nM;
+        const uint32_t nM0 = nM, nS0 = nS;
+        if (j.two) {
+            uint32_t nM1, nS1;
+            b.b.m = qscan_n<NT / 64>(t.b.m, j.s_w, &nM1, w) + nM + nS;
+            b.b.s = qscan_n<NT / 64>(t.b.s, j.s_w, &nS1, w) + nM + nS + nM1;
+            nM += nM1;
+            nS += nS1;
+        }
         if (WIDE) {
             __syncthreads();
             if (tid == 0) {
@@ -756,19 +826,24 @@
             }
             __syncthreads();
             const uint32_t bw = j.s_w[20];
-            b.m += bw;
-            b.s += bw;
+            b.a.m += bw;
+            b.a.s += bw;
         }
         if (!WIDE && tid == 0) {
             bqh->n_copy = min(nM + nS, bcap_copy);
             bqh->n_copy_medium = nM;
             bqh->n_copy_small = nS;
+            bqh->n_copy0 = min(nM0 + nS0, bcap_copy);
+            bqh->n_copy_medium0 = nM0;
+            bqh->n_copy_small0 = nS0;
             bqh->overflow_copy = nM + nS > bcap_copy ? 1u : 0u;
             if (mirror) {
                 mirror[2] = min(nM + nS, bcap_copy) + 1u;
                 if (nM + nS > bcap_copy)
                     mirror[3] = 1u;
             }
+            if (mirror1)
+                mirror1[2] = min(nM + nS, bcap_copy) - min(nM0 + nS0, bcap_copy) + 1u;
         }
         q_phase(ph, 4);
         if (j.Ug > 0)
@@ -784,8 +859,11 @@
             if (part == 0) {
                 __hip_atomic_store(&bqh->n_wave, bqh->n_wave, __ATOMIC_RELAXED, __HIP_MEMORY_SCOPE_AGENT);
                 __hip_atomic_store(&bqh->n_coop, bqh->n_coop, __ATOMIC_RELAXED, __HIP_MEMORY_SCOPE_AGENT);
+                __hip_atomic_store(&bqh->n_wave0, bqh->n_wave0, __ATOMIC_RELAXED, __HIP_MEMORY_SCOPE_AGENT);
+                __hip_atomic_store(&bqh->n_coop0, bqh->n_coop0, __ATOMIC_RELAXED, __HIP_MEMORY_SCOPE_AGENT);
             } else {
                 __hip_atomic_store(&bqh->n_copy, bqh->n_copy, __ATOMIC_RELAXED, __HIP_MEMORY_SCOPE_AGENT);
+                __hip_atomic_store(&bqh->n_copy0, bqh->n_copy0, __ATOMIC_RELAXED, __HIP_MEMORY_SCOPE_AGENT);
             }
             asm volatile("s_waitcnt vmcnt(0) lgkmcnt(0)" ::: "memory");
             __hip_atomic_store(part == 0 ? &bqh->epoch_wave : &bqh->epoch_copy, epoch, __ATOMIC_RELAXED, __HIP_MEMORY_SCOPE_AGENT);
@@ -1256,8 +1334,9 @@
     int b = blockIdx.x;
     if (a.epoch != 0u) {
         const uint32_t fail = ~a.epoch;
+        uint32_t *const verdict = const_cast<uint32_t *>(a.sel == 2u ? &a.qh->verdict1 : &a.qh->verdict);
         bool ready = a.qh->epoch_wave == a.epoch && a.qh->epoch_copy == a.epoch &&
-                     a.qh->verdict != fail;
+                     *verdict != fail;
         if (blockIdx.x == 0) {
             const unsigned long long t_poll = __builtin_amdgcn_s_memrealtime();
             for (int spin = 0; !ready && spin < (1 << 22); ++spin) {
@@ -1269,7 +1348,7 @@
                 __builtin_amdgcn_s_sleep(64);
             }
             if (threadIdx.x == 0) {
-                __hip_atomic_store(const_cast<uint32_t *>(&a.qh->verdict), ready ? a.epoch : fail, __ATOMIC_RELAXED,
+                __hip_atomic_store(verdict, ready ? a.epoch : fail, __ATOMIC_RELAXED,
                                    __HIP_MEMORY_SCOPE_AGENT);
                 if (!ready && a.err != nullptr)
                     __hip_atomic_store(a.err, 8u, __ATOMIC_RELAXED, __HIP_MEMORY_SCOPE_SYSTEM);
@@ -1278,7 +1357,7 @@
             const unsigned long long t_poll = __builtin_amdgcn_s_memrealtime();
             uint32_t vd = 0u;
             for (int spin = 0; spin < (1 << 23); ++spin) {
-                vd = uniform(__hip_atomic_load(&a.qh->verdict, __ATOMIC_ACQUIRE, __HIP_MEMORY_SCOPE_AGENT));
+                vd = uniform(__hip_atomic_load(verdict, __ATOMIC_ACQUIRE, __HIP_MEMORY_SCOPE_AGENT));
                 if (vd == a.epoch || vd == fail || __builtin_amdgcn_s_memrealtime() - t_poll > 400000000ull)
                     break;
                 __builtin_amdgcn_s_sleep(64);
@@ -1293,8 +1372,13 @@
     const bool coop = b < a.ncoop;
     if (coop) {
         role = 0;
-        const uint32_t n = min(a.qh->n_coop, a.cap_coop);
-        for (uint32_t e = static_cast<uint32_t>(b); e < n; e += static_cast<uint32_t>(a.ncoop)) {
+        uint32_t g0 = 0u, n = min(a.qh->n_coop, a.cap_coop);
+        if (a.sel != 0u) {
+            const uint32_t gs = min(a.qh->n_coop0, n);
+            g0 = a.sel == 1u ? 0u : gs;
+            n = a.sel == 1u ? gs : n;
+        }
+        for (uint32_t e = g0 + static_cast<uint32_t>(b); e < n; e += static_cast<uint32_t>(a.ncoop)) {
             const QItem it = q_load(a.qcoop + e, a.width);
 #if QV_GOLD
             q_coop_r3(a, it, reinterpret_cast<float *>(s_dyn), e);
@@ -1306,7 +1390,16 @@
     } else {
         b -= a.ncoop;
         role = 3;
-        const uint32_t n0 = min(a.qh->n_wave, a.cap_wave), n = n0 + min(a.qh->n_copy, a.cap_copy);
+        uint32_t w0 = 0u, wn = min(a.qh->n_wave, a.cap_wave), c0 = 0u, cn = min(a.qh->n_copy, a.cap_copy);
+        if (a.sel != 0u) {
+            const uint32_t ws = min(a.qh->n_wave0, wn), cs = min(a.qh->n_copy0, cn);
+            w0 = a.sel == 1u ? 0u : ws;
+            wn = a.sel == 1u ? ws : wn;
+            c0 = a.sel == 1u ? 0u : cs;
+            cn = a.sel == 1u ? cs : cn;
+        }
+        const QEntry *const qwave = a.qwave + w0, *const qcopy = a.qcopy + c0;
+        const uint32_t n0 = wn - w0, n = n0 + (cn - c0);
         const uint32_t stride = static_cast<uint32_t>(a.nworker) * static_cast<uint32_t>(kQWpw);
         const uint32_t wv = uniform(static_cast<uint32_t>(threadIdx.x >> 6));
         if (a.width <= 128) {
@@ -1317,8 +1410,8 @@
                 for (int h = 0; h < 2; ++h) {
                     const uint32_t e = 2u * pe + static_cast<uint32_t>(h);
                     src[h] = e >= n ? nullptr
-                                    : e < both ? ((e & 1u) ? a.qcopy + (e >> 1) : a.qwave + (e >> 1))
-                                               : (n0 > n1 ? a.qwave + (e - n1) : a.qcopy + (e - n0));
+                                    : e < both ? ((e & 1u) ? qcopy + (e >> 1) : qwave + (e >> 1))
+                                               : (n0 > n1 ? qwave + (e - n1) : qcopy + (e - n0));
                 }
                 const uint32_t ka = uniform(src[0]->w[0] & 15u), kb = src[1] ? uniform(src[1]->w[0] & 15u) : 15u;
                 const bool sa = ka == static_cast<uint32_t>(kQS), sb = kb == static_cast<uint32_t>(kQS);
@@ -1347,12 +1440,12 @@
             const uint32_t n1 = n - n0, both = 2u * (n0 < n1 ? n0 : n1);
             const QEntry *src;
             if (e < both)
-                src = (e & 1u) ? a.qcopy + (e >> 1) : a.qwave + (e >> 1);
+                src = (e & 1u) ? qcopy + (e >> 1) : qwave + (e >> 1);
             else
-                src = n0 > n1 ? a.qwave + (e - n1) : a.qcopy + (e - n0);
+                src = n0 > n1 ? qwave + (e - n1) : qcopy + (e - n0);
             const QItem it = q_load(src, a.width);
 #else
-            const QItem it = q_load(e < n0 ? a.qwave + e : a.qcopy + (e - n0), a.width);
+            const QItem it = q_load(e < n0 ? qwave + e : qcopy + (e - n0), a.width);
 #endif
             kind = it.kind;
             if (it.kind == kQL)
@@ -1420,6 +1513,8 @@
     QEntry *coop[kQJoinBatch], *wave[kQJoinBatch], *copy[kQJoinBatch];
     uint32_t *mirror[kQJoinBatch];
     uint32_t epoch[kQJoinBatch];
+    uint32_t *mirror1[kQJoinBatch];
+    uint32_t two;
     unsigned long long *ph;
 };
 __global__ __launch_bounds__(1024, 4) void qqueue_kernel(const QJoinBatch b) {
@@ -1427,7 +1522,7 @@
     const int i = blockIdx.x >> 1, part = blockIdx.x & 1;
     qjoin_body(b.pa[i], b.pg[i], b.rows, b.width, b.qh[i], b.coop[i], b.wave[i], b.copy[i], b.cap_coop, b.cap_wave,
                b.cap_copy, s_dyn, b.lds_bytes, part, (i == 0 && b.ph) ? b.ph + 8 * part : nullptr, b.mirror[i], 0u, 0u,
-               b.epoch[i]);
+               b.epoch[i], 0u, true, b.two, b.mirror1[i]);
 }
 
 __global__ __launch_bounds__(1024) void q_lds_order_check_kernel(uint32_t *bad) {
@@ -1526,7 +1621,7 @@
 static int qqueue_batch(int64_t rows, int64_t width, void *const *plans_a, const int64_t *n_a, void *const *plans_g,
                         const int64_t *n_g, void *const *queues, int64_t queue_n_cap, int64_t count,
                         hipStream_t stream, unsigned long long *ph = nullptr, uint32_t *const *counts_host = nullptr,
-                        const uint32_t *epochs = nullptr) {
+                        const uint32_t *epochs = nullptr, bool two_classes = false, uint32_t *const *counts_host1 = nullptr) {
     HA_REQUIRE(rows >= 0 && rows <= 0xFFFFFFFEll && width >= 4 && width % 4 == 0 && width <= (1 << 20),
                "ha_qqueue_batch: rows of a multiple of 4 floats");
     HA_REQUIRE(count >= 0 && (count == 0 || (plans_a && n_a && plans_g && n_g && queues)), "ha_qqueue_batch: null pointer");
@@ -1543,6 +1638,7 @@
         b.rows = static_cast<uint64_t>(rows);
         b.width = static_cast<int>(width);
         b.ph = k0 == 0 ? ph : nullptr;
+        b.two = two_classes ? 1u : 0u;
         size_t lds = 0;
         for (int64_t k = k0; k < count && b.count < kQJoinBatch; ++k) {
             HA_REQUIRE(n_a[k] >= 0 && n_g[k] >= 0 && n_a[k] <= queue_n_cap && n_g[k] <= queue_n_cap,
@@ -1558,6 +1654,7 @@
             b.qh[i] = q.hdr;
             b.mirror[i] = counts_host ? counts_host[k] : nullptr;
             b.epoch[i] = epochs ? epochs[k] : 0u;
+            b.mirror1[i] = (two_classes && counts_host1) ? counts_host1[k] : nullptr;
             b.coop[i] = q.coop;
             b.wave[i] = q.wave;
             b.copy[i] = q.copy;
@@ -1581,7 +1678,7 @@
                         float lr, const int32_t *perm_next, int64_t n_next, float *next_out, const void *queue_cur,
                         int64_t queue_n_cap, int64_t n_max, hipStream_t stream, unsigned long long *dbg = nullptr,
                         int64_t wave_items = -1, uint32_t epoch = 0, uint32_t *err = nullptr, hipEvent_t done = nullptr,
-                        int64_t coop_items = -1);
+                        int64_t coop_items = -1, uint32_t sel = 0);
 
 static int qapply(float *table, int64_t rows, int64_t width, void *plan_cur, int64_t n_cur, const float *grads, float lr,
                   void *plan_next, int64_t n_next, float *next_out, const void *queue_cur, int64_t queue_n_cap,
@@ -1597,7 +1694,7 @@
 static int qapply_lists(float *table, int64_t rows, int64_t width, const int32_t *perm_cur, int64_t n_cur, const float *grads,
                         float lr, const int32_t *perm_next, int64_t n_next, float *next_out, const void *queue_cur,
                         int64_t queue_n_cap, int64_t n_max, hipStream_t stream, unsigned long long *dbg,
-                        int64_t wave_items, uint32_t epoch, uint32_t *err, hipEvent_t done, int64_t coop_items) {
+                        int64_t wave_items, uint32_t epoch, uint32_t *err, hipEvent_t done, int64_t coop_items, uint32_t sel) {
     HA_REQUIRE(table != nullptr && rows >= 0 && rows <= 0xFFFFFFFEll && width >= 4 && width % 4 == 0 &&
                    width <= (1 << 20) && reinterpret_cast<uintptr_t>(table) % 16 == 0,
                "ha_qapply: the table must be 16-byte aligned with rows of a multiple of 4 floats");
@@ -1617,6 +1714,7 @@
     QArgs a;
     memset(&a, 0, sizeof(a));
     a.epoch = epoch;
+    a.sel = sel;
     a.err = err;
     a.table = table;
     a.rows = static_cast<uint64_t>(rows);
@@ -2192,6 +2290,173 @@
                   as_stream(stream), nullptr, wave_items, epoch, err, static_cast<hipEvent_t>(done_event));
 }
 
+extern "C" int ha_qqueue_batch_chains(int64_t rows, int64_t width, void *const *plans_a, const int64_t *n_a,
+                                      void *const *plans_g, const int64_t *n_g, void *const *queues, int64_t queue_n_cap,
+                                      int64_t count, uint32_t *const *counts_host, uint32_t *const *counts_host1,
+                                      const uint32_t *epochs, ha_stream_t stream) {
+    return qqueue_batch(rows, width, plans_a, n_a, plans_g, n_g, queues, queue_n_cap, count, as_stream(stream), nullptr,
+                        counts_host, epochs, true, counts_host1);
+}
+
+namespace ha {
+struct QChainBlock {
+    float *table;
+    int64_t rows, width, queue_n_cap, count;
+    float lr;
+    void *const *plan_cur;
+    const int64_t *n_cur;
+    const float *const *grads;
+    void *const *plan_next;
+    const int64_t *n_next;
+    float *const *next_out;
+    const void *const *queue_cur;
+    const int64_t *wave_items;
+    const uint32_t *epochs;
+    uint32_t *err;
+    hipEvent_t done, fork;
+    hipStream_t stream;
+};
+constexpr int kQChainForkEvents = 8;
+struct QChain {
+    int device = 0;
+    std::thread th;
+    std::mutex mu;
+    std::condition_variable cv;
+    QChainBlock blk;
+    std::atomic<uint64_t> posted{0}, finished{0};
+    std::atomic<bool> stop{false};
+    int rc = 0;
+    char msg[1024];
+    hipEvent_t fork[kQChainForkEvents];
+    uint64_t nfork = 0;
+};
+static int qchain_enqueue(const QChainBlock &b, uint32_t sel, hipStream_t stream, const int64_t *wave_items, uint32_t *err,
+                          hipEvent_t done) {
+    bool marked = false;
+    for (int64_t k = 0; k < b.count; ++k) {
+        HA_REQUIRE(b.n_cur[k] >= 0 && b.n_next[k] >= 0 && (b.n_cur[k] == 0 || b.plan_cur[k]) && (b.n_next[k] == 0 || b.plan_next[k]),
+                   "ha_qapply_steps_chains: a batch needs its plan");
+        const bool last = k + 1 == b.count;
+        if (qapply_lists(b.table, b.rows, b.width, b.n_cur[k] > 0 ? plan_layout(b.plan_cur[k], b.n_cur[k]).perm : nullptr,
+                         b.n_cur[k], b.grads[k], b.lr, b.n_next[k] > 0 ? plan_layout(b.plan_next[k], b.n_next[k]).perm : nullptr,
+                         b.n_next[k], b.next_out[k], b.queue_cur[k], b.queue_n_cap, kQMax, stream, nullptr,
+                         wave_items ? wave_items[k] : -1, b.epochs ? b.epochs[k] : 0u, err, last ? done : nullptr, -1, sel))
+            return -1;
+        marked = marked || last;
+    }
+    if (!marked && done != nullptr)
+        HA_CHECK_HIP(hipEventRecord(done, stream));
+    return 0;
+}
+static void qchain_feed(QChain *c) {
+    (void)hipSetDevice(c->device);
+    uint64_t seen = 0;
+    for (;;) {
+        bool have = false;
+        for (int spin = 0; spin < 20000 && !have; ++spin) {
+            have = c->posted.load(std::memory_order_acquire) != seen || c->stop.load(std::memory_order_acquire);
+            if (!have)
+                __builtin_ia32_pause();
+        }
+        if (!have) {
+            std::unique_lock<std::mutex> lk(c->mu);
+            c->cv.wait(lk, [&] { return c->posted.load(std::memory_order_acquire) != seen || c->stop.load(std::memory_order_acquire); });
+        }
+        if (c->posted.load(std::memory_order_acquire) == seen)
+            return;
+        seen = c->posted.load(std::memory_order_acquire);
+        const QChainBlock &b = c->blk;
+        int rc = 0;
+        if (hipStreamWaitEvent(b.stream, b.fork, 0) != hipSuccess) {
+            set_error("ha_qapply_steps_chains: hipStreamWaitEvent (fork) failed");
+            rc = -1;
+        }
+        if (rc == 0)
+            rc = qchain_enqueue(b, 2u, b.stream, b.wave_items, b.err, b.done);
+        c->rc = rc;
+        if (rc != 0)
+            snprintf(c->msg, sizeof(c->msg), "%s", ha_last_error());
+        c->finished.store(seen, std::memory_order_release);
+    }
+}
+}
+
+extern "C" void *ha_qchain_create(void) {
+    QChain *c = new (std::nothrow) QChain();
+    if (c == nullptr)
+        return nullptr;
+    if (hipGetDevice(&c->device) != hipSuccess)
+        c->device = 0;
+    for (int i = 0; i < kQChainForkEvents; ++i)
+        c->fork[i] = nullptr;
+    for (int i = 0; i < kQChainForkEvents; ++i)
+        if (hipEventCreateWithFlags(&c->fork[i], hipEventDisableTiming) != hipSuccess) {
+            for (int j = 0; j < i; ++j)
+                (void)hipEventDestroy(c->fork[j]);
+            delete c;
+            set_error("ha_qchain_create: hipEventCreate failed");
+            return nullptr;
+        }
+    c->th = std::thread(qchain_feed, c);
+    return c;
+}
+extern "C" int ha_qchain_destroy(void *chain) {
+    QChain *c = static_cast<QChain *>(chain);
+    if (c == nullptr)
+        return 0;
+    {
+        std::lock_guard<std::mutex> lk(c->mu);
+        c->stop.store(true, std::memory_order_release);
+    }
+    c->cv.notify_all();
+    if (c->th.joinable())
+        c->th.join();
+    for (int i = 0; i < kQChainForkEvents; ++i)
+        (void)hipEventDestroy(c->fork[i]);
+    delete c;
+    return 0;
+}
+extern "C" int ha_qapply_steps_chains(void *chain, float *table, int64_t rows, int64_t width, float lr, int64_t queue_n_cap,
+                                      int64_t count, void *const *plan_cur, const int64_t *n_cur, const float *const *grads,
+                                      void *const *plan_next, const int64_t *n_next, float *const *next_out,
+                                      const void *const *queue_cur, const int64_t *wave_items0, const int64_t *wave_items1,
+                                      const uint32_t *epochs, uint32_t *err0, uint32_t *err1, void *done_event0,
+                                      void *done_event1, ha_stream_t stream, ha_stream_t chain_stream) {
+    QChain *c = static_cast<QChain *>(chain);
+    HA_REQUIRE(c != nullptr && done_event1 != nullptr && chain_stream != nullptr && chain_stream != stream,
+               "ha_qapply_steps_chains: needs a chain, a stream of its own for it and the event of its last launch");
+    HA_REQUIRE(count >= 1 && plan_cur && n_cur && grads && plan_next && n_next && next_out && queue_cur,
+               "ha_qapply_steps_chains: null pointer");
+    HA_REQUIRE(width > 128, "ha_qapply_steps_chains: rows wider than 128 floats");
+    QChainBlock b;
+    b.table = table; b.rows = rows; b.width = width; b.queue_n_cap = queue_n_cap; b.count = count; b.lr = lr;
+    b.plan_cur = plan_cur; b.n_cur = n_cur; b.grads = grads; b.plan_next = plan_next; b.n_next = n_next; b.next_out = next_out;
+    b.queue_cur = queue_cur; b.epochs = epochs;
+    b.wave_items = wave_items1; b.err = err1;
+    b.done = static_cast<hipEvent_t>(done_event1);
+    b.fork = c->fork[c->nfork++ % kQChainForkEvents];
+    b.stream = as_stream(chain_stream);
+    HA_CHECK_HIP(hipEventRecord(b.fork, as_stream(stream)));
+    c->blk = b;
+    const uint64_t ticket = c->posted.load(std::memory_order_relaxed) + 1;
+    {
+        std::lock_guard<std::mutex> lk(c->mu);
+        c->posted.store(ticket, std::memory_order_release);
+    }
+    c->cv.notify_one();
+    const int rc0 = qchain_enqueue(b, 1u, as_stream(stream), wave_items0, err0, static_cast<hipEvent_t>(done_event0));
+    while (c->finished.load(std::memory_order_acquire) != ticket)
+        __builtin_ia32_pause();
+    if (c->rc != 0) {
+        set_error("%s", c->msg);
+        return -1;
+    }
+    if (rc0 != 0)
+        return -1;
+    HA_CHECK_HIP(hipStreamWaitEvent(as_stream(stream), b.done, 0));
+    return 0;
+}
+
 extern "C" int ha_qqueue_batch_counts(int64_t rows, int64_t width, void *const *plans_a, const int64_t *n_a,
                                       void *const *plans_g, const int64_t *n_g, void *const *queues, int64_t queue_n_cap,
                                       int64_t count, uint32_t *const *counts_host, ha_stream_t stream) {
diff --git a/herald_amd/ops.py b/herald_amd/ops.py
--- a/herald_amd/ops.py
+++ b/herald_amd/ops.py
@@ -699,12 +699,32 @@
         self._last_items = 0
         self.fallbacks, self._fb_plan, self._wide_ids = 0, None, {}
         self._enq_last = None
+        self.chains = (table.shape[1] > 128 and not self.wide and self.overlap and self.sync == "flags" and self.block >= 8
+                       and os.environ.get("HA_QCHAINS", "2") != "1")
+        self._chain, self._chain_stream, self._chain_for = None, None, None
+        self._done_ev1 = {}
+        self.counts1 = None
+        if self.chains:
+            self.counts1 = torch.zeros((self.COUNTS, 4), dtype=torch.int32).pin_memory()
+            self._counts1_np = self.counts1.numpy()
+            self._counts1_c = (ctypes.c_int32 * (self.COUNTS * 4)).from_address(self.counts1.data_ptr())
+            self._counts1_base = self.counts1.data_ptr()
+            self._last_items1 = 0
+            with torch.cuda.device(self.device):
+                self._chain = ctypes.c_void_p(L.ha_qchain_create())
+            if not self._chain:
+                check(-1, "ha_qchain_create")
         self.reset()
 
     def close(self):
-        for ev in list(self._done_ev.values()) + self._cev_pool + [e for e, _ in self._cev_busy]:
+        chain, self._chain = getattr(self, "_chain", None), None
+        if chain:
+            self._L.ha_qchain_destroy(chain)
+        self._chain_stream = self._chain_for = None
+        for ev in (list(self._done_ev.values()) + list(getattr(self, "_done_ev1", {}).values()) + self._cev_pool +
+                   [e for e, _ in self._cev_busy]):
             self._L.ha_event_destroy(ev)
-        self._done_ev, self._cev_pool, self._cev_busy = {}, [], []
+        self._done_ev, self._done_ev1, self._cev_pool, self._cev_busy = {}, {}, [], []
 
     def __del__(self):
         try:
@@ -713,14 +733,15 @@
             pass
 
     def reset(self, stream=None):
-        if self._done_ev:
+        live = list(self._done_ev.values()) + list(self._done_ev1.values())
+        if live:
             if self.side is not None:
                 marker = self._event() if hasattr(self, "_ev_pool") else torch.cuda.Event()
                 marker.record(self.side)
-                self._cev_busy.extend((e, marker) for e in self._done_ev.values())
+                self._cev_busy.extend((e, marker) for e in live)
             else:
-                self._cev_pool.extend(self._done_ev.values())
-        self._done_ev = {}
+                self._cev_pool.extend(live)
+        self._done_ev, self._done_ev1 = {}, {}
         self.c, self.n, self.shape, self.ids = None, {}, {}, {}
         self._enq_last, self._covered = None, -(1 << 60)
         self._ev_side = {}
@@ -742,12 +763,17 @@
         return d
 
     def overflowed(self):
+        if self.counts1 is not None and bool(self._counts1_np[:, 3].any()):
+            return True
         return bool((self._counts_np[:, 3] & ~4).any())
 
     def _raise_if_failed(self, steps):
         cc, ring = self._counts_c, self.COUNTS
+        c1 = self._counts1_c if self.counts1 is not None else None
         for j in steps:
             f = cc[4 * (j % ring) + 3]
+            if c1 is not None:
+                f |= c1[4 * (j % ring) + 3]
             if f & ~4:
                 raise RuntimeError("QueueStepPipeline: step %d failed on the device (flags %d: 1 = queue overflow, 2 = an "
                                    "occurrence list out of position order, 8 = an apply launch gave up waiting -- its queue was "
@@ -766,11 +792,18 @@
         self._raise_if_failed(range(max((b - 2) * B, 0), max((b - 1) * B, 0)))
         if self.overlap and flags:
             cev = self._done_ev.pop(b - 1, None)
+            cev1 = self._done_ev1.pop(b - 1, None)
             if cev is not None:
                 check(L.ha_stream_wait_event(sp, cev), "ha_stream_wait_event")
+                if cev1 is not None:
+                    check(L.ha_stream_wait_event(sp, cev1), "ha_stream_wait_event")
                 marker = self._event()
                 marker.record(s)
                 self._cev_busy.append((cev, marker))
+                if cev1 is not None:
+                    marker1 = self._event()
+                    marker1.record(s)
+                    self._cev_busy.append((cev1, marker1))
                 self._covered = b * B - 1
             elif self._enq_last is not None and self._enq_last > self._covered:
                 ev = self._event()
@@ -848,6 +881,15 @@
             if self.wide:
                 check(L.ha_qbig_queue_batch(rows, width, pa, na, pg, ng, qs, self.capacity, cnt, cs, eps, sp),
                       "ha_qbig_queue_batch")
+            elif self.chains:
+                c1, base1 = self._counts1_c, self._counts1_base
+                for j in steps:
+                    at = 4 * (j % ring)
+                    c1[at] = 0
+                    c1[at + 2] = 0
+                cs1 = (vp * cnt)(*[base1 + 16 * (j % ring) for j in steps])
+                check(L.ha_qqueue_batch_chains(rows, width, pa, na, pg, ng, qs, self.capacity, cnt, cs, cs1, eps, sp),
+                      "ha_qqueue_batch_chains")
             else:
                 check(L.ha_qqueue_batch_epochs(rows, width, pa, na, pg, ng, qs, self.capacity, cnt, cs, eps, sp),
                       "ha_qqueue_batch")
@@ -882,6 +924,28 @@
             self._cev_pool.append(old)
         self._done_ev[c // self.block] = ev
         return ev
+
+    def _block_done_event1(self, c):
+        if not self._cev_pool and self._cev_busy and self._cev_busy[0][1].query():
+            old_ev, marker = self._cev_busy.pop(0)
+            self._ev_pool.append(marker)
+            self._cev_pool.append(old_ev)
+        ev = self._cev_pool.pop() if self._cev_pool else ctypes.c_void_p(self._L.ha_event_create())
+        if not ev:
+            raise RuntimeError("ha_event_create failed")
+        old = self._done_ev1.pop(c // self.block, None)
+        if old is not None:
+            self._cev_pool.append(old)
+        self._done_ev1[c // self.block] = ev
+        return ev
+
+    def _pick_chain_stream(self, stream):
+        from . import streams
+        if self._chain_for == stream.cuda_stream:
+            return self._chain_stream
+        self._chain_for = stream.cuda_stream
+        self._chain_stream = streams.pick_chain_stream(stream, self.side)
+        return self._chain_stream
 
     def _err_ptr(self, c):
         return ctypes.c_void_p(self._counts_base + 16 * (c % self.COUNTS) + 12)
@@ -1013,11 +1077,46 @@
         cs = (vp * cnt)()
         base = self._counts_base
         use_counts = os.environ.get("HA_QCOUNTS", "0") != "0"
+        cstream = None
+        if self.chains and flags and sized and self._chain and not torch.cuda.is_current_stream_capturing():
+            cstream = self._pick_chain_stream(stream if stream is not None else torch.cuda.current_stream(self.device))
+        if cstream is not None:
+            csp = _stream_ptr(cstream)
+            hints1 = (i64 * cnt)(*[-1] * cnt)
+            counts1, fn_chains, chain = self._counts1_c, L.ha_qapply_steps_chains, self._chain
+            err1 = lambda c: ctypes.c_void_p(self._counts1_base + 16 * (c % ring) + 12)
+
+        def call_chains(k0):
+            self._enq_last = k0 + cnt - 1 if self._enq_last is None else max(self._enq_last, k0 + cnt - 1)
+            for i in range(cnt):
+                at = 4 * ((k0 + i) % ring)
+                w, cp, w1, cp1 = counts[at], counts[at + 2], counts1[at], counts1[at + 2]
+                if counts[at + 3] or counts1[at + 3]:
+                    raise RuntimeError("ha_qqueue_batch: the work queue of step %d is unusable (flags %d: 1 = overflow, "
+                                       "2 = an occurrence list out of position order)" % (k0 + i, counts[at + 3] | counts1[at + 3]))
+                n1 = w1 + cp1 - 2 if w1 > 0 and cp1 > 0 else -1
+                n0 = w + cp - 2 - n1 if n1 >= 0 and w > 0 and cp > 0 else -1
+                if n0 >= 0:
+                    self._last_items, self._last_items1 = n0 + n1, n1
+                    hints[i], hints1[i] = n0, n1
+                elif self._last_items1 > 0:
+                    hints[i] = ((self._last_items - self._last_items1) * 17) // 16
+                    hints1[i] = (self._last_items1 * 17) // 16
+                else:
+                    hints[i] = hints1[i] = -1
+                eps[i] = epoch(k0 + i)
+            last = k0 + cnt - 1
+            done0, done1 = self._block_done_event(last), self._block_done_event1(last)
+            if fn_chains(chain, *head, pc, ns, gs, pn, ns, os_, qs, hints, hints1, eps, last_err(last), err1(last), done0, done1,
+                         sp, csp) != 0:
+                check(-1, "ha_qapply_steps_chains")
 
         def call(k0):
             if flags and k0 // B != (k0 + cnt - 1) // B:
                 raise RuntimeError("apply_steps_call(sync='flags'): steps %d..%d cross a block boundary (block = %d)"
                                    % (k0, k0 + cnt - 1, B))
+            if cstream is not None and (k0 + cnt) % B == 0:
+                return call_chains(k0)
             self._enq_last = k0 + cnt - 1 if self._enq_last is None else max(self._enq_last, k0 + cnt - 1)
             if sized:
                 for i in range(cnt):
diff --git a/herald_amd/streams.py b/herald_amd/streams.py
--- a/herald_amd/streams.py
+++ b/herald_amd/streams.py
@@ -61,3 +61,43 @@
     del buf, small
     _PICKED[key] = pick
     return pick
+
+
+def _beside(L, a, b, ticks=50000):
+    import ctypes
+    import time
+    torch.cuda.synchronize(a.device)
+    best = None
+    for _ in range(3):
+        t0 = time.perf_counter()
+        L.ha_debug_occupy(1, 64, 4, ticks, ctypes.c_void_p(a.cuda_stream))
+        L.ha_debug_occupy(1, 64, 4, ticks, ctypes.c_void_p(b.cuda_stream))
+        a.synchronize()
+        b.synchronize()
+        dt = time.perf_counter() - t0
+        best = dt if best is None else min(best, dt)
+    return best < 1.6 * ticks * 1e-8
+
+
+def pick_chain_stream(main, side=None, candidates=6):
+    from . import _lib
+    L = _lib.load()
+    dev = main.device
+    sid = side.cuda_stream if side is not None else 0
+    key = ("chain", dev.index, main.cuda_stream, sid)
+    if key in _PICKED:
+        return _PICKED[key]
+    cands = _PICKED.setdefault(("chain candidates", dev.index, main.cuda_stream), [])
+    pick = None
+    with torch.cuda.device(dev):
+        for i in range(candidates):
+            if i == len(cands):
+                cands.append(torch.cuda.Stream(device=dev))
+            cand = cands[i]
+            if cand.cuda_stream in (main.cuda_stream, sid):
+                continue
+            if _beside(L, main, cand) and (side is None or _beside(L, side, cand)):
+                pick = cand
+                break
+    _PICKED[key] = pick
+    return pick
diff --git a/include/herald_amd.h b/include/herald_amd.h
--- a/include/herald_amd.h
+++ b/include/herald_amd.h
@@ -299,6 +299,19 @@
                            const int64_t *n_next, float *const *next_out, const void *const *queue_cur,
                            const int64_t *wave_items, const uint32_t *const *counts_host, const uint32_t *epochs, uint32_t *err,
                            void *done_event, ha_stream_t stream);
+
+int ha_qqueue_batch_chains(int64_t rows, int64_t width, void *const *plans_a, const int64_t *n_a, void *const *plans_g,
+                           const int64_t *n_g, void *const *queues, int64_t queue_n_cap, int64_t count,
+                           uint32_t *const *counts_host, uint32_t *const *counts_host1, const uint32_t *epochs,
+                           ha_stream_t stream);
+void *ha_qchain_create(void);
+int ha_qchain_destroy(void *chain);
+int ha_qapply_steps_chains(void *chain, float *table, int64_t rows, int64_t width, float lr, int64_t queue_n_cap, int64_t count,
+                           void *const *plan_cur, const int64_t *n_cur, const float *const *grads, void *const *plan_next,
+                           const int64_t *n_next, float *const *next_out, const void *const *queue_cur,
+                           const int64_t *wave_items0, const int64_t *wave_items1, const uint32_t *epochs, uint32_t *err0,
+                           uint32_t *err1, void *done_event0, void *done_event1, ha_stream_t stream,
+                           ha_stream_t chain_stream);
 
 int ha_xchg_available(void);
 int ha_xchg_unique_id(void *id128);
```

Result: slower. 520.1 million (-4.1%).
